# yhhshb/biolib

Measured on AMD Instinct MI355X. Metric: Gbp/s minimizer-scanned (k=31,w=11), higher is better.
Workload: dtype u64

## Files before the change

### biolib_amd/csrc/bl_capi.hip

```cpp
#include <hip/hip_runtime.h>
#include <algorithm>
#include <cstdio>
#include <cstdlib>
#include <cstring>
#include <deque>
#include <new>
#include <string>
#include <utility>
#include <vector>

#include "../../include/biolib_amd.h"
#include "bl_launch.hpp"
#include "bl_lookup_launch.hpp"
#include "bl_read_counts_launch.hpp"
#include "bl_scan128_launch.hpp"

namespace {

thread_local std::string g_err;

int fail(int code, const std::string& msg)
{
    g_err = msg;
    return code;
}

}

int bl_set_error(int code, const char* msg) { return fail(code, msg ? msg : ""); }
struct bl_ctx;
hipStream_t bl_ctx_stream(bl_ctx* ctx);
int bl_ctx_device(bl_ctx* ctx);

namespace {

#define BL_HIP(call)                                                                                       \
    do {                                                                                                   \
        hipError_t e_ = (call);                                                                            \
        if (e_ != hipSuccess)                                                                              \
            return fail(e_ == hipErrorOutOfMemory ? BL_ERR_OOM : BL_ERR_HIP,                               \
                        std::string(#call) + ": " + hipGetErrorString(e_));                                \
    } while (0)

constexpr int RESULT_WORDS = 16;
constexpr int RING = 256;
constexpr size_t HDR_BYTES = 256;
constexpr size_t SHARD_BYTES = (size_t)bl::NSHARD * 8 * sizeof(unsigned long long);

struct Pending {
    bl_result* user;
    int slot;
    uint64_t capacity;
    bool has_capacity;
};

}

struct Lane {
    hipStream_t own = nullptr;
    unsigned char* ws = nullptr;
    size_t ws_bytes = 0;
    unsigned char* tile_buf = nullptr;
    size_t tile_buf_bytes = 0;
    uint16_t* slot_buf = nullptr;
    size_t slot_buf_bytes = 0;
    hipEvent_t ev_start = nullptr, ev_stop = nullptr;
    hipEvent_t ev_count_done = nullptr;
    bool count_recorded = false;
    bool scan_recorded = false;

    unsigned long long* shards() const { return reinterpret_cast<unsigned long long*>(ws + HDR_BYTES); }
    unsigned long long* result() const { return reinterpret_cast<unsigned long long*>(ws + HDR_BYTES + SHARD_BYTES); }
};

struct bl_ctx {
    int device = 0;
    Lane lanes[2];
    Lane* cur = nullptr;
    int next_lane = 0;
    int n_lanes = 1;
    uint32_t emit_lds_per_wg = 0;
    hipStream_t user_stream = nullptr;
    bool borrowed = false;
    hipStream_t stream = nullptr;
    unsigned long long* pinned = nullptr;
    hipEvent_t slot_ev[RING] = {};
    int next_slot = 0;
    std::deque<Pending> pending;
    bool timed = false;
    bool exact_windows = false;
    bool position_tiled = false;
    int jaccard128_path = 0;
    bool count128_tables = true;
    int table_prefix_bits = -1;
    bool ktiming = false;
    bl::LaunchLog last_kernels{};
    std::vector<hipEvent_t> ev_pool;
    std::vector<std::pair<hipEvent_t, hipEvent_t>> ev_open;
    double kernel_ms = 0.0;
    uint64_t kernel_launches = 0;
    std::vector<std::pair<hipEvent_t, hipEvent_t>> marks;
    std::vector<bl_batch*> batches;
    void* scratch[8] = {};
    size_t scratch_bytes[8] = {};
    std::vector<std::pair<void*, size_t>> pool_idle;
    std::vector<std::pair<void*, size_t>> pool_live;

    unsigned long long* shards() const { return cur->shards(); }
    unsigned long long* result() const { return cur->result(); }
    static size_t fixed_bytes() { return HDR_BYTES + SHARD_BYTES + RESULT_WORDS * sizeof(unsigned long long); }
};

struct bl_batch {
    bl_ctx* ctx = nullptr;
    uint8_t* bases = nullptr;
    bool owns_bases = false;
    uint32_t* start_bits = nullptr;
    uint64_t n_bases = 0;
    uint64_t n_seqs = 0;
    uint64_t read_len = 0;
    uint64_t origin = 0;
};

namespace {

int grow(bl_ctx* c, void** buf, size_t* have, size_t need)
{
    if (need <= *have) return BL_OK;
    BL_HIP(hipStreamSynchronize(c->stream));
    if (*buf) BL_HIP(hipFree(*buf));
    *buf = nullptr;
    *have = 0;
    const size_t bytes = need + need / 8;
    hipError_t e = hipMalloc(buf, bytes);
    if (e != hipSuccess) return fail(BL_ERR_OOM, std::string("hipMalloc(scan scratch): ") + hipGetErrorString(e));
    *have = bytes;
    return BL_OK;
}

int ensure_workspace(bl_ctx* c)
{
    return grow(c, reinterpret_cast<void**>(&c->cur->ws), &c->cur->ws_bytes, bl_ctx::fixed_bytes());
}

void select_lane(bl_ctx* c)
{
    if (c->borrowed) {
        c->cur = &c->lanes[0];
        c->stream = c->user_stream;
    } else {
        c->cur = &c->lanes[c->next_lane];
        if (c->n_lanes == 2) c->next_lane ^= 1;
        c->stream = c->cur->own;
    }
}

void deliver(bl_ctx* c, const Pending& p)
{
    const unsigned long long* r = c->pinned + (size_t)p.slot * RESULT_WORDS;
    bl_result out;
    std::memset(&out, 0, sizeof(out));
    out.count = r[0];
    out.xor_value = r[1];
    out.xor_hash = r[2];
    out.xor_pos = r[3];
    out.aux = r[4];
    out.redone = (int32_t)(r[5] > 0x7fffffffull ? 0x7fffffffull : r[5]);
    out.status = BL_OK;
    if (p.has_capacity && r[0] > p.capacity) out.status = BL_ERR_CAPACITY;
    if (p.user) *p.user = out;
}

int flush_pending(bl_ctx* c)
{
    for (const Pending& p : c->pending) deliver(c, p);
    c->pending.clear();
    return BL_OK;
}

int flush_kernel_events(bl_ctx* c)
{
    for (auto& pr : c->ev_open) {
        float ms = 0.f;
        BL_HIP(hipEventElapsedTime(&ms, pr.first, pr.second));
        c->kernel_ms += ms;
        c->kernel_launches += 1;
        c->ev_pool.push_back(pr.first);
        c->ev_pool.push_back(pr.second);
    }
    c->ev_open.clear();
    return BL_OK;
}

int sync_ctx(bl_ctx* c)
{
    for (Lane& l : c->lanes) BL_HIP(hipStreamSynchronize(l.own));
    if (c->borrowed) BL_HIP(hipStreamSynchronize(c->user_stream));
    int rc = flush_kernel_events(c);
    if (rc != BL_OK) return rc;
    return flush_pending(c);
}

int kernel_event(bl_ctx* c, bool start)
{
    if (!c->ktiming) return BL_OK;
    if (start) {
        hipEvent_t ev[2];
        for (int i = 0; i < 2; ++i) {
            if (!c->ev_pool.empty()) { ev[i] = c->ev_pool.back(); c->ev_pool.pop_back(); }
            else BL_HIP(hipEventCreate(&ev[i]));
        }
        c->ev_open.emplace_back(ev[0], ev[1]);
        BL_HIP(hipEventRecord(ev[0], c->stream));
    } else {
        BL_HIP(hipEventRecord(c->ev_open.back().second, c->stream));
    }
    return BL_OK;
}

int begin_scan(bl_ctx* c)
{
    BL_HIP(hipSetDevice(c->device));
    select_lane(c);
    int rc = ensure_workspace(c);
    if (rc != BL_OK) return rc;
    BL_HIP(hipEventRecord(c->cur->ev_start, c->stream));
    BL_HIP(hipMemsetAsync(c->cur->ws, 0, bl_ctx::fixed_bytes(), c->stream));
    return BL_OK;
}

int end_scan(bl_ctx* c, uint32_t add_mask, bl_result* user, bool has_capacity, uint64_t capacity, uint32_t flags,
             bool already_folded = false)
{
    if (!already_folded) {
        hipError_t e = bl::launch_reduce_shards(c->shards(), c->result(), add_mask, reinterpret_cast<unsigned long long*>(c->cur->ws) + 1, c->stream);
        if (e != hipSuccess) return fail(BL_ERR_HIP, std::string("reduce_shards: ") + hipGetErrorString(e));
    }
    if ((int)c->pending.size() >= RING) {
        const Pending old = c->pending.front();
        BL_HIP(hipEventSynchronize(c->slot_ev[old.slot]));
        deliver(c, old);
        c->pending.pop_front();
    }
    const int slot = c->next_slot;
    c->next_slot = (c->next_slot + 1) % RING;
    BL_HIP(hipMemcpyAsync(c->pinned + (size_t)slot * RESULT_WORDS, c->result(), RESULT_WORDS * sizeof(unsigned long long),
                          hipMemcpyDeviceToHost, c->stream));
    BL_HIP(hipEventRecord(c->slot_ev[slot], c->stream));
    BL_HIP(hipEventRecord(c->cur->ev_stop, c->stream));
    c->cur->scan_recorded = true;
    c->timed = true;
    c->pending.push_back(Pending{user, slot, capacity, has_capacity});
    if (flags & BL_FLAG_SYNC) {
        int rc = sync_ctx(c);
        if (rc != BL_OK) return rc;
        if (user && user->status != BL_OK)
            return fail(user->status, "output capacity too small for the records found");
    }
    return BL_OK;
}

int zero_result(bl_ctx* c, bl_result* user, uint32_t flags)
{
    if (user) std::memset(user, 0, sizeof(*user));
    (void)c;
    (void)flags;
    return BL_OK;
}

int check_range(const bl_batch* b, uint64_t first, uint64_t n, uint64_t& end)
{
    if (first > b->n_bases) return fail(BL_ERR_INVALID, "range starts beyond the batch");
    end = (n == 0 || n > b->n_bases - first) ? b->n_bases : first + n;
    if (end - first > (1ull << 31)) return fail(BL_ERR_INVALID, "a scan range may hold at most 2^31 positions; split it");
    return BL_OK;
}

int make_start_bits(bl_ctx* c, bl_batch* b, const uint64_t* offsets, uint64_t n_seqs, uint64_t read_len)
{
    const uint64_t n_words = (b->n_bases + 31) / 32 + 4;
    if (!offsets && (read_len == 0 || read_len >= b->n_bases)) {
        b->start_bits = nullptr;
        b->n_seqs = b->n_bases ? 1 : 0;
        return BL_OK;
    }
    BL_HIP(hipMalloc(&b->start_bits, n_words * sizeof(uint32_t)));
    BL_HIP(hipMemsetAsync(b->start_bits, 0, n_words * sizeof(uint32_t), c->stream));
    if (offsets) {
        for (uint64_t q = 0; q < n_seqs; ++q)
            if (offsets[q] > offsets[q + 1]) return fail(BL_ERR_INVALID, "offsets must be non-decreasing");
        if (offsets[0] != 0 || offsets[n_seqs] != b->n_bases) return fail(BL_ERR_INVALID, "offsets must span [0, n_bases]");
        uint64_t* d_off = nullptr;
        BL_HIP(hipMalloc(&d_off, (n_seqs + 1) * sizeof(uint64_t)));
        hipError_t e = hipMemcpyAsync(d_off, offsets, (n_seqs + 1) * sizeof(uint64_t), hipMemcpyHostToDevice, c->stream);
        if (e == hipSuccess) e = bl::launch_start_bits_offsets(b->start_bits, d_off, n_seqs, b->n_bases, c->stream);
        if (e == hipSuccess) e = hipStreamSynchronize(c->stream);
        (void)hipFree(d_off);
        if (e != hipSuccess) return fail(BL_ERR_HIP, std::string("start_bits_offsets: ") + hipGetErrorString(e));
        b->n_seqs = n_seqs;
    } else {
        hipError_t e = bl::launch_start_bits_fixed(b->start_bits, n_words, b->n_bases, read_len, c->stream);
        if (e != hipSuccess) return fail(BL_ERR_HIP, std::string("start_bits_fixed: ") + hipGetErrorString(e));
        b->n_seqs = (b->n_bases + read_len - 1) / read_len;
        BL_HIP(hipStreamSynchronize(c->stream));
    }
    return BL_OK;
}

int ensure_start_bits(bl_ctx* c, const bl_batch* cb)
{
    bl_batch* b = const_cast<bl_batch*>(cb);
    if (b->start_bits || b->read_len == 0 || b->read_len >= b->n_bases) return BL_OK;
    int rc = sync_ctx(c);
    if (rc != BL_OK) return rc;
    return make_start_bits(c, b, nullptr, 0, b->read_len);
}

}

hipStream_t bl_ctx_stream(bl_ctx* c)
{
    if (c->borrowed) return c->user_stream;
    if (c->n_lanes == 2 && c->lanes[1].scan_recorded) (void)hipStreamWaitEvent(c->lanes[0].own, c->lanes[1].ev_stop, 0);
    return c->lanes[0].own;
}
int bl_batch_adopt_device(bl_ctx* ctx, void* d_bases, uint64_t n_bases, uint64_t* d_offsets, uint64_t n_seqs, uint64_t fixed_len, bl_batch** out);
int bl_ctx_device(bl_ctx* c) { return c->device; }
int bl_ctx_count128_tables(bl_ctx* c) { return c->count128_tables ? 1 : 0; }
int bl_ctx_jaccard128_path(bl_ctx* c) { return c->jaccard128_path; }
int bl_ctx_table_prefix_bits(bl_ctx* c) { return c->table_prefix_bits; }
int bl_batch_describe(const bl_batch* b, bl_ctx** ctx, uint64_t* n_bases, uint64_t* n_seqs, uint64_t* read_len)
{
    *ctx = b->ctx;
    *n_bases = b->n_bases;
    *n_seqs = b->n_seqs;
    *read_len = b->read_len;
    return BL_OK;
}

int bl_batch_scan_view(bl_ctx* c, const bl_batch* b, int ensure, const uint32_t** start_bits)
{
    if (ensure) {
        int rc = ensure_start_bits(c, b);
        if (rc != BL_OK) return rc;
    }
    *start_bits = b->start_bits;
    return BL_OK;
}

void* bl_ctx_scratch(bl_ctx* c, int slot, size_t bytes)
{
    if (!c || slot < 0 || slot >= 8) return nullptr;
    if (bytes <= c->scratch_bytes[slot]) return c->scratch[slot];
    (void)hipSetDevice(c->device);
    if (c->scratch[slot]) {
        (void)hipDeviceSynchronize();
        (void)hipFree(c->scratch[slot]);
        c->scratch[slot] = nullptr;
        c->scratch_bytes[slot] = 0;
    }
    const size_t want = bytes + bytes / 8;
    if (hipMalloc(&c->scratch[slot], want) != hipSuccess) {
        c->scratch[slot] = nullptr;
        return nullptr;
    }
    c->scratch_bytes[slot] = want;
    return c->scratch[slot];
}

void* bl_ctx_pool_alloc(bl_ctx* c, size_t bytes)
{
    if (!c) return nullptr;
    if (bytes < 256) bytes = 256;
    size_t best = c->pool_idle.size();
    for (size_t i = 0; i < c->pool_idle.size(); ++i) {
        const size_t have = c->pool_idle[i].second;
        if (have >= bytes && have <= 2 * bytes + 65536 && (best == c->pool_idle.size() || have < c->pool_idle[best].second)) best = i;
    }
    if (best < c->pool_idle.size()) {
        const auto entry = c->pool_idle[best];
        c->pool_idle[best] = c->pool_idle.back();
        c->pool_idle.pop_back();
        c->pool_live.push_back(entry);
        return entry.first;
    }
    void* p = nullptr;
    const size_t want = bytes + bytes / 8;
    if (hipMalloc(&p, want) != hipSuccess) return nullptr;
    c->pool_live.emplace_back(p, want);
    return p;
}

void bl_ctx_pool_free(bl_ctx* c, void* p)
{
    if (!p) return;
    if (c)
        for (size_t i = 0; i < c->pool_live.size(); ++i)
            if (c->pool_live[i].first == p) {
                const auto entry = c->pool_live[i];
                c->pool_live[i] = c->pool_live.back();
                c->pool_live.pop_back();
                size_t total = 0;
                for (const auto& e : c->pool_idle) total += e.second;
                if (c->pool_idle.size() < 16 && entry.second <= ((size_t)1 << 30) && total + entry.second <= ((size_t)4 << 30)) c->pool_idle.push_back(entry);
                else (void)hipFree(p);
                return;
            }
    (void)hipFree(p);
}

extern "C" {

const char* bl_last_error(void) { return g_err.c_str(); }
int bl_version(void) { return BL_VERSION; }

int bl_device_count(int* n)
{
    if (!n) return fail(BL_ERR_INVALID, "n is NULL");
    int c = 0;
    hipError_t e = hipGetDeviceCount(&c);
    if (e != hipSuccess) { *n = 0; return fail(BL_ERR_NO_DEVICE, std::string("hipGetDeviceCount: ") + hipGetErrorString(e)); }
    *n = c;
    return BL_OK;
}

int bl_ctx_create(int device, bl_ctx** out)
{
    if (!out) return fail(BL_ERR_INVALID, "out is NULL");
    *out = nullptr;
    int n = 0;
    if (hipGetDeviceCount(&n) != hipSuccess || n == 0) return fail(BL_ERR_NO_DEVICE, "no HIP device visible: this library has no CPU fallback");
    if (device < 0 || device >= n) return fail(BL_ERR_INVALID, "device index out of range");
    hipDeviceProp_t prop;
    BL_HIP(hipGetDeviceProperties(&prop, device));
    if (std::strncmp(prop.gcnArchName, "gfx950", 6) != 0)
        return fail(BL_ERR_NO_DEVICE, std::string("device is ") + prop.gcnArchName + ", kernels are built for gfx950 (MI355X) only");
    BL_HIP(hipSetDevice(device));
    bl_ctx* c = new (std::nothrow) bl_ctx();
    if (!c) return fail(BL_ERR_OOM, "host allocation failed");
    c->device = device;
    hipError_t e = hipSuccess;
    for (Lane& l : c->lanes) {
        if (e == hipSuccess) e = hipStreamCreateWithFlags(&l.own, hipStreamNonBlocking);
        if (e == hipSuccess) e = hipEventCreate(&l.ev_start);
        if (e == hipSuccess) e = hipEventCreateWithFlags(&l.ev_count_done, hipEventDisableTiming);
        if (e == hipSuccess) e = hipEventCreate(&l.ev_stop);
    }
    if (e == hipSuccess) e = hipHostMalloc(reinterpret_cast<void**>(&c->pinned), (size_t)RING * RESULT_WORDS * sizeof(unsigned long long), hipHostMallocDefault);
    for (int i = 0; i < RING && e == hipSuccess; ++i) e = hipEventCreateWithFlags(&c->slot_ev[i], hipEventDisableTiming);
    if (e != hipSuccess) {
        bl_ctx_destroy(c);
        return fail(BL_ERR_HIP, std::string("context setup: ") + hipGetErrorString(e));
    }
    for (int i = 0; i < 2; ++i) {
        c->cur = &c->lanes[i];
        c->stream = c->cur->own;
        int rc = ensure_workspace(c);
        if (rc != BL_OK) { bl_ctx_destroy(c); return rc; }
    }
    c->cur = &c->lanes[0];
    c->stream = c->lanes[0].own;
    *out = c;
    return BL_OK;
}

int bl_ctx_set_lanes(bl_ctx* c, int n)
{
    if (!c || (n != 1 && n != 2)) return fail(BL_ERR_INVALID, "bl_ctx_set_lanes: need a context and n = 1 or 2");
    int rc = sync_ctx(c);
    if (rc != BL_OK) return rc;
    c->n_lanes = n;
    c->next_lane = 0;
    c->lanes[0].count_recorded = c->lanes[1].count_recorded = false;
    return BL_OK;
}

int bl_ctx_destroy(bl_ctx* c)
{
    if (!c) return BL_OK;
    (void)hipSetDevice(c->device);
    for (Lane& l : c->lanes)
        if (l.own) (void)hipStreamSynchronize(l.own);
    if (c->borrowed) (void)hipStreamSynchronize(c->user_stream);
    while (!c->batches.empty()) bl_batch_destroy(c->batches.back());
    for (Lane& l : c->lanes) {
        if (l.ws) (void)hipFree(l.ws);
        if (l.tile_buf) (void)hipFree(l.tile_buf);
        if (l.slot_buf) (void)hipFree(l.slot_buf);
        if (l.ev_start) (void)hipEventDestroy(l.ev_start);
        if (l.ev_count_done) (void)hipEventDestroy(l.ev_count_done);
        if (l.ev_stop) (void)hipEventDestroy(l.ev_stop);
        if (l.own) (void)hipStreamDestroy(l.own);
    }
    for (void* p : c->scratch)
        if (p) (void)hipFree(p);
    for (const auto& e : c->pool_idle) (void)hipFree(e.first);
    for (const auto& e : c->pool_live) (void)hipFree(e.first);
    if (c->pinned) (void)hipHostFree(c->pinned);
    for (hipEvent_t ev : c->slot_ev)
        if (ev) (void)hipEventDestroy(ev);
    for (auto& pr : c->ev_open) { (void)hipEventDestroy(pr.first); (void)hipEventDestroy(pr.second); }
    for (hipEvent_t ev : c->ev_pool) (void)hipEventDestroy(ev);
    for (auto& pr : c->marks) { (void)hipEventDestroy(pr.first); if (pr.second) (void)hipEventDestroy(pr.second); }
    delete c;
    return BL_OK;
}

int bl_ctx_set_stream(bl_ctx* c, void* hip_stream)
{
    if (!c) return fail(BL_ERR_INVALID, "ctx is NULL");
    int rc = sync_ctx(c);
    if (rc != BL_OK) return rc;
    c->borrowed = true;
    c->user_stream = static_cast<hipStream_t>(hip_stream);
    c->cur = &c->lanes[0];
    c->stream = c->user_stream;
    return BL_OK;
}

int bl_ctx_use_own_streams(bl_ctx* c)
{
    if (!c) return fail(BL_ERR_INVALID, "ctx is NULL");
    int rc = sync_ctx(c);
    if (rc != BL_OK) return rc;
    c->borrowed = false;
    c->user_stream = nullptr;
    c->cur = &c->lanes[0];
    c->stream = c->lanes[0].own;
    return BL_OK;
}

int bl_ctx_sync(bl_ctx* c)
{
    if (!c) return fail(BL_ERR_INVALID, "ctx is NULL");
    return sync_ctx(c);
}

int bl_ctx_last_scan_ms(bl_ctx* c, float* ms)
{
    if (!c || !ms) return fail(BL_ERR_INVALID, "NULL argument");
    if (!c->timed) return fail(BL_ERR_INVALID, "no scan has been issued on this context");
    BL_HIP(hipEventSynchronize(c->cur->ev_stop));
    BL_HIP(hipEventElapsedTime(ms, c->cur->ev_start, c->cur->ev_stop));
    return BL_OK;
}

int bl_ctx_set_exact_windows(bl_ctx* c, int on)
{
    if (!c) return fail(BL_ERR_INVALID, "ctx is NULL");
    c->exact_windows = on != 0;
    return BL_OK;
}

int bl_ctx_set_option(bl_ctx* c, const char* name, int64_t value)
{
    if (!c || !name) return fail(BL_ERR_INVALID, "bl_ctx_set_option: NULL argument");
    const std::string n(name);
    if (n == "exact_windows" && (value == 0 || value == 1)) return bl_ctx_set_exact_windows(c, (int)value);
    if (n == "lanes") return bl_ctx_set_lanes(c, (int)value);
    if (n == "position_tiled" && (value == 0 || value == 1)) {
        c->position_tiled = value != 0;
        return BL_OK;
    }
    if (n == "count128_tables" && (value == 0 || value == 1)) {
        c->count128_tables = value != 0;
        return BL_OK;
    }
    if (n == "jaccard128_path" && value >= 0 && value <= 2) {
        c->jaccard128_path = (int)value;
        return BL_OK;
    }
    if (n == "table_prefix_bits" && value >= -1 && value <= bllk::MAX_PREFIX_BITS) {
        c->table_prefix_bits = (int)value;
        return BL_OK;
    }
    if (n == "emit_lds_bytes" && value >= 0 && value <= 160 * 1024) {
        c->emit_lds_per_wg = (uint32_t)value;
        return BL_OK;
    }
    return fail(BL_ERR_INVALID, "bl_ctx_set_option: unknown name or value out of range: " + n);
}

int bl_ctx_kernel_timing(bl_ctx* c, int enable)
{
    if (!c) return fail(BL_ERR_INVALID, "ctx is NULL");
    int rc = sync_ctx(c);
    if (rc != BL_OK) return rc;
    c->ktiming = enable != 0;
    c->kernel_ms = 0.0;
    c->kernel_launches = 0;
    return BL_OK;
}

int bl_ctx_kernel_time(bl_ctx* c, double* total_ms, uint64_t* launches)
{
    if (!c || !total_ms || !launches) return fail(BL_ERR_INVALID, "NULL argument");
    int rc = sync_ctx(c);
    if (rc != BL_OK) return rc;
    *total_ms = c->kernel_ms;
    *launches = c->kernel_launches;
    return BL_OK;
}

static constexpr size_t MAX_MARKS = 4096;

int bl_ctx_mark(bl_ctx* c)
{
    if (!c) return fail(BL_ERR_INVALID, "ctx is NULL");
    if (c->marks.size() >= MAX_MARKS) return fail(BL_ERR_CAPACITY, "bl_ctx_mark: 4096 markers outstanding: collect them with bl_ctx_mark_times");
    BL_HIP(hipSetDevice(c->device));
    std::pair<hipEvent_t, hipEvent_t> m{nullptr, nullptr};
    const bool two = !c->borrowed && c->n_lanes == 2 && c->lanes[1].own;
    hipError_t e = hipEventCreate(&m.first);
    if (e == hipSuccess && two) e = hipEventCreate(&m.second);
    if (e == hipSuccess) e = hipEventRecord(m.first, c->borrowed ? c->user_stream : c->lanes[0].own);
    if (e == hipSuccess && two) e = hipEventRecord(m.second, c->lanes[1].own);
    if (e != hipSuccess) {
        if (m.first) (void)hipEventDestroy(m.first);
        if (m.second) (void)hipEventDestroy(m.second);
        return fail(BL_ERR_HIP, std::string("bl_ctx_mark: ") + hipGetErrorString(e));
    }
    c->marks.push_back(m);
    return BL_OK;
}

int bl_ctx_mark_times(bl_ctx* c, double* ms, uint32_t capacity, uint32_t* n)
{
    if (!c || !n || (!ms && capacity)) return fail(BL_ERR_INVALID, "NULL argument");
    int rc = sync_ctx(c);
    if (rc != BL_OK) return rc;
    *n = (uint32_t)c->marks.size();
    if (capacity < c->marks.size()) {
        if (capacity == 0) return BL_OK;
        return fail(BL_ERR_CAPACITY, "bl_ctx_mark_times: more markers than the buffer holds (*n says how many)");
    }
    hipError_t e = hipSuccess;
    for (size_t i = 0; i < c->marks.size(); ++i) {
        float a = 0.f, b = 0.f;
        if (e == hipSuccess) e = hipEventSynchronize(c->marks[i].first);
        if (e == hipSuccess) e = hipEventElapsedTime(&a, c->marks[0].first, c->marks[i].first);
        if (e == hipSuccess && c->marks[i].second) {
            e = hipEventSynchronize(c->marks[i].second);
            if (e == hipSuccess) e = hipEventElapsedTime(&b, c->marks[0].first, c->marks[i].second);
        }
        if (i < capacity) ms[i] = a > b ? a : b;
    }
    for (auto& pr : c->marks) { (void)hipEventDestroy(pr.first); if (pr.second) (void)hipEventDestroy(pr.second); }
    c->marks.clear();
    if (e != hipSuccess) return fail(BL_ERR_HIP, std::string("bl_ctx_mark_times: ") + hipGetErrorString(e));
    return BL_OK;
}


static int new_batch(bl_ctx* c, uint64_t n_bases, bl_batch** out, bl_batch*& b)
{
    if (!c || !out) return fail(BL_ERR_INVALID, "NULL argument");
    *out = nullptr;
    BL_HIP(hipSetDevice(c->device));
    b = new (std::nothrow) bl_batch();
    if (!b) return fail(BL_ERR_OOM, "host allocation failed");
    b->ctx = c;
    b->n_bases = n_bases;
    c->batches.push_back(b);
    return BL_OK;
}

static int upload_batch(bl_ctx* c, const char* bases, uint64_t n_bases, const uint64_t* offsets, uint64_t n_seqs, uint64_t read_len, bl_batch** out)
{
    bl_batch* b = nullptr;
    int rc = new_batch(c, n_bases, out, b);
    if (rc != BL_OK) return rc;
    if (n_bases && !bases) { bl_batch_destroy(b); return fail(BL_ERR_INVALID, "bases is NULL"); }
    b->bases = static_cast<uint8_t*>(bl_ctx_pool_alloc(c, n_bases + 64));
    if (!b->bases) { bl_batch_destroy(b); return fail(BL_ERR_OOM, "device allocation of the batch's bases failed"); }
    b->owns_bases = true;
    hipError_t e = hipMemsetAsync(b->bases + (n_bases & ~15ull), 0, 64 + (n_bases & 15ull), c->stream);
    if (e == hipSuccess && n_bases) e = hipMemcpyAsync(b->bases, bases, n_bases, hipMemcpyHostToDevice, c->stream);
    if (e != hipSuccess) { bl_batch_destroy(b); return fail(BL_ERR_HIP, std::string("upload: ") + hipGetErrorString(e)); }
    uint64_t fixed = 0;
    if (read_len) {
        if (read_len < n_bases) {
            fixed = read_len;
            n_seqs = (n_bases + read_len - 1) / read_len;
        } else {
            offsets = nullptr;
            n_seqs = 0;
        }
    } else if (offsets && n_seqs > 1 && offsets[0] == 0 && offsets[n_seqs] == n_bases && offsets[1] > 0 && offsets[1] < n_bases) {
        fixed = offsets[1];
        for (uint64_t q = 1; q < n_seqs && fixed; ++q)
            if (offsets[q] != q * fixed) fixed = 0;
        if (fixed && (n_bases - offsets[n_seqs - 1] > fixed || n_bases == offsets[n_seqs - 1])) fixed = 0;
    }
    if (fixed) {
        b->read_len = fixed;
        b->n_seqs = n_seqs;
    } else {
        rc = make_start_bits(c, b, offsets, n_seqs, 0);
    }
    if (rc == BL_OK) {
        e = hipStreamSynchronize(c->stream);
        if (e != hipSuccess) rc = fail(BL_ERR_HIP, std::string("upload sync: ") + hipGetErrorString(e));
    }
    if (rc != BL_OK) { bl_batch_destroy(b); return rc; }
    *out = b;
    return BL_OK;
}

int bl_batch_upload(bl_ctx* c, const char* bases, uint64_t n_bases, const uint64_t* offsets, uint64_t n_seqs, bl_batch** out)
{
    return upload_batch(c, bases, n_bases, offsets, n_seqs, 0, out);
}

int bl_batch_upload_reads(bl_ctx* c, const char* bases, uint64_t n_bases, uint64_t read_len, bl_batch** out)
{
    if (read_len == 0) return fail(BL_ERR_INVALID, "read_len must not be 0");
    return upload_batch(c, bases, n_bases, nullptr, 0, read_len, out);
}

int bl_batch_from_device(bl_ctx* c, const void* d_bases, uint64_t n_bases, const uint64_t* offsets, uint64_t n_seqs, uint64_t read_len,
                         bl_batch** out)
{
    bl_batch* b = nullptr;
    int rc = new_batch(c, n_bases, out, b);
    if (rc != BL_OK) return rc;
    if ((n_bases && !d_bases) || (reinterpret_cast<uintptr_t>(d_bases) & 15)) {
        bl_batch_destroy(b);
        return fail(BL_ERR_INVALID, "d_bases must be a non-NULL, 16-byte aligned device pointer");
    }
    b->bases = const_cast<uint8_t*>(static_cast<const uint8_t*>(d_bases));
    b->owns_bases = false;
    if (!offsets && read_len > 0 && read_len < n_bases) {
        b->read_len = read_len;
        b->n_seqs = (n_bases + read_len - 1) / read_len;
    } else {
        rc = make_start_bits(c, b, offsets, n_seqs, read_len);
        if (rc != BL_OK) { bl_batch_destroy(b); return rc; }
    }
    *out = b;
    return BL_OK;
}

int bl_batch_set_origin(bl_batch* b, uint64_t origin)
{
    if (!b) return fail(BL_ERR_INVALID, "batch is NULL");
    b->origin = origin;
    return BL_OK;
}

uint64_t bl_batch_origin(const bl_batch* b) { return b ? b->origin : 0; }

int bl_batch_synth(bl_ctx* c, uint64_t seed, uint64_t n_bases, uint64_t read_len, bl_batch** out)
{
    bl_batch* b = nullptr;
    int rc = new_batch(c, n_bases, out, b);
    if (rc != BL_OK) return rc;
    hipError_t e = hipMalloc(&b->bases, n_bases + 64);
    if (e != hipSuccess) { bl_batch_destroy(b); return fail(BL_ERR_OOM, std::string("hipMalloc(bases): ") + hipGetErrorString(e)); }
    b->owns_bases = true;
    e = hipMemsetAsync(b->bases + (n_bases & ~15ull), 0, 64 + (n_bases & 15ull), c->stream);
    if (e == hipSuccess) e = bl::launch_synth(b->bases, 0, n_bases, seed, c->stream);
    if (e != hipSuccess) { bl_batch_destroy(b); return fail(BL_ERR_HIP, std::string("synth: ") + hipGetErrorString(e)); }
    if (read_len > 0 && read_len < n_bases) {
        b->read_len = read_len;
        b->n_seqs = (n_bases + read_len - 1) / read_len;
    } else {
        rc = make_start_bits(c, b, nullptr, 0, read_len);
    }
    if (rc == BL_OK && hipStreamSynchronize(c->stream) != hipSuccess) rc = fail(BL_ERR_HIP, "synth sync failed");
    if (rc != BL_OK) { bl_batch_destroy(b); return rc; }
    *out = b;
    return BL_OK;
}

}

int bl_batch_adopt_device(bl_ctx* c, void* d_bases, uint64_t n_bases, uint64_t* d_offsets, uint64_t n_seqs, uint64_t fixed_len, bl_batch** out)
{
    bl_batch* b = nullptr;
    int rc = new_batch(c, n_bases, out, b);
    if (rc != BL_OK) { bl_ctx_pool_free(c, d_bases); bl_ctx_pool_free(c, d_offsets); return rc; }
    b->bases = static_cast<uint8_t*>(d_bases);
    b->owns_bases = true;
    b->n_seqs = n_seqs;
    if (fixed_len && n_seqs > 1 && fixed_len < n_bases) {
        b->read_len = fixed_len;
        bl_ctx_pool_free(c, d_offsets);
        *out = b;
        return BL_OK;
    }
    hipStream_t s = bl_ctx_stream(c);
    const uint64_t n_words = (n_bases + 31) / 32 + 4;
    b->start_bits = static_cast<uint32_t*>(bl_ctx_pool_alloc(c, n_words * sizeof(uint32_t)));
    hipError_t e = b->start_bits ? hipSuccess : hipErrorOutOfMemory;
    if (e == hipSuccess) e = hipMemsetAsync(b->start_bits, 0, n_words * sizeof(uint32_t), s);
    if (e == hipSuccess) e = bl::launch_start_bits_offsets(b->start_bits, d_offsets, n_seqs, n_bases, s);
    if (e == hipSuccess) e = hipStreamSynchronize(s);
    bl_ctx_pool_free(c, d_offsets);
    if (e != hipSuccess) { bl_batch_destroy(b); return fail(BL_ERR_HIP, std::string("adopt: ") + hipGetErrorString(e)); }
    *out = b;
    return BL_OK;
}

int bl_batch_adopt_like(bl_ctx* c, const bl_batch* like, void* d_bases, uint32_t* d_start_bits, bl_batch** out)
{
    bl_batch* b = nullptr;
    int rc = new_batch(c, like->n_bases, out, b);
    if (rc != BL_OK) { bl_ctx_pool_free(c, d_bases); bl_ctx_pool_free(c, d_start_bits); return rc; }
    b->bases = static_cast<uint8_t*>(d_bases);
    b->owns_bases = true;
    b->start_bits = d_start_bits;
    b->n_seqs = like->n_seqs;
    b->read_len = like->read_len;
    b->origin = like->origin;
    *out = b;
    return BL_OK;
}

extern "C" {

int bl_batch_destroy(bl_batch* b)
{
    if (!b) return BL_OK;
    if (b->ctx) {
        (void)hipSetDevice(b->ctx->device);
        for (Lane& l : b->ctx->lanes)
            if (l.own) (void)hipStreamSynchronize(l.own);
        if (b->ctx->borrowed) (void)hipStreamSynchronize(b->ctx->user_stream);
        auto& v = b->ctx->batches;
        for (size_t i = 0; i < v.size(); ++i)
            if (v[i] == b) { v[i] = v.back(); v.pop_back(); break; }
    }
    if (b->owns_bases && b->bases) bl_ctx_pool_free(b->ctx, b->bases);
    if (b->start_bits) bl_ctx_pool_free(b->ctx, b->start_bits);
    delete b;
    return BL_OK;
}

uint64_t bl_batch_n_bases(const bl_batch* b) { return b ? b->n_bases : 0; }
uint64_t bl_batch_n_seqs(const bl_batch* b) { return b ? b->n_seqs : 0; }
const void* bl_batch_device_bases(const bl_batch* b) { return b ? b->bases : nullptr; }

int bl_batch_download(bl_batch* b, uint64_t first, uint64_t n, char* out)
{
    if (!b || (!out && n)) return fail(BL_ERR_INVALID, "NULL argument");
    if (first > b->n_bases || n > b->n_bases - first) return fail(BL_ERR_INVALID, "range beyond the batch");
    BL_HIP(hipSetDevice(b->ctx->device));
    int rc = sync_ctx(b->ctx);
    if (rc != BL_OK) return rc;
    if (n) BL_HIP(hipMemcpy(out, b->bases + first, n, hipMemcpyDeviceToHost));
    return BL_OK;
}


int bl_scan_kmers(bl_ctx* c, const bl_batch* b, uint64_t first, uint64_t n, uint32_t k, uint64_t seed, uint32_t flags,
                  uint64_t* d_values, uint64_t* d_hashes, uint8_t* d_valid, bl_result* result)
{
    if (!c || !b || b->ctx != c) return fail(BL_ERR_INVALID, "ctx/batch is NULL or the batch belongs to another context");
    if (k < 1 || k > bl::MAX_UNIT) return fail(BL_ERR_INVALID, "k must be in [1, 32] (KmerType = uint64_t)");
    uint64_t end;
    int rc = check_range(b, first, n, end);
    if (rc != BL_OK) return rc;
    if (end <= first) return zero_result(c, result, flags);
    rc = ensure_start_bits(c, b);
    if (rc != BL_OK) return rc;
    bl::KmerParams p{};
    p.bases = b->bases;
    p.n_bases = (int64_t)b->n_bases;
    p.start_bits = b->start_bits;
    p.first = (int64_t)first;
    p.end = (int64_t)end;
    p.origin = bl::align_down16((int64_t)first);
    p.n_tiles = (int32_t)(((int64_t)end - 1 - p.origin) / bl::H + 1);
    p.unit = (int32_t)k;
    p.seed = (uint32_t)seed;
    p.canonical = (flags & BL_FLAG_CANONICAL) ? 1 : 0;
    p.drop_last = (flags & BL_FLAG_DROP_LAST) ? 1 : 0;
    p.out_value = d_values;
    p.out_hash = d_hashes;
    p.out_valid = d_valid;
    rc = begin_scan(c);
    if (rc != BL_OK) return rc;
    p.shards = c->shards();
    const int n_blocks = p.n_tiles < 256 * 8 ? p.n_tiles : 256 * 8;
    rc = kernel_event(c, true);
    if (rc != BL_OK) return rc;
    hipError_t e = bl::launch_kmers(p, n_blocks, c->stream);
    if (e != hipSuccess) return fail(BL_ERR_HIP, std::string("kmer_kernel: ") + hipGetErrorString(e));
    rc = kernel_event(c, false);
    if (rc != BL_OK) return rc;
    return end_scan(c,  (1u << 0) | (1u << 3), result, false, 0, flags);
}


static int prepare_kmers128(bl_ctx* c, const bl_batch* b, uint64_t first, uint64_t n, uint32_t k, uint64_t seed, uint32_t flags, const uint64_t* d_values,
                            bl::Kmer128Params& p, bl_result* result, bool& empty)
{
    empty = false;
    if (!c || !b || b->ctx != c) return fail(BL_ERR_INVALID, "ctx/batch is NULL or the batch belongs to another context");
    if (k < 1 || k > bl::MAX_UNIT128) return fail(BL_ERR_INVALID, "k must be in [1, 64] (KmerType = __uint128_t)");
    if (reinterpret_cast<uintptr_t>(d_values) % 16 != 0) return fail(BL_ERR_INVALID, "d_values must be 16-byte aligned (one __uint128_t per record)");
    uint64_t end;
    int rc = check_range(b, first, n, end);
    if (rc != BL_OK) return rc;
    if (end <= first) {
        empty = true;
        return zero_result(c, result, flags);
    }
    rc = ensure_start_bits(c, b);
    if (rc != BL_OK) return rc;
    p.bases = b->bases;
    p.n_bases = (int64_t)b->n_bases;
    p.start_bits = b->start_bits;
    p.pos_base = (int64_t)b->origin;
    bl::plan_kmers128((int64_t)first, (int64_t)end, p);
    p.unit = (int32_t)k;
    p.seed = (uint32_t)seed;
    p.canonical = (flags & BL_FLAG_CANONICAL) ? 1 : 0;
    p.drop_last = (flags & BL_FLAG_DROP_LAST) ? 1 : 0;
    return BL_OK;
}

extern "C++" {
template <typename P>
static int scan_two_pass128(bl_ctx* c, P& p, bl::Kmer128Params& km, size_t lane_bytes, uint32_t** lane_rest, bool wants, uint64_t capacity, uint32_t flags,
                            bl_result* result, hipError_t (*count)(const P&, hipStream_t), hipError_t (*emit)(const P&, hipStream_t), const char* family)
{
    km.capacity = wants ? capacity : 0;
    int rc = begin_scan(c);
    if (rc != BL_OK) return rc;
    const size_t nt = (size_t)km.n_tiles, nb = (nt + bl::SCAN_BLK - 1) / bl::SCAN_BLK;
    rc = grow(c, reinterpret_cast<void**>(&c->cur->tile_buf), &c->cur->tile_buf_bytes, (2 * nt + 2 * nb + 8) * sizeof(unsigned long long));
    if (rc != BL_OK) return rc;
    unsigned long long* tb = reinterpret_cast<unsigned long long*>(c->cur->tile_buf);
    km.tile_counts = tb;
    km.tile_base = tb + nt;
    unsigned long long* block_tot = tb + 2 * nt;
    km.block_base = block_tot + nb;
    if (lane_bytes) {
        rc = grow(c, reinterpret_cast<void**>(&c->cur->slot_buf), &c->cur->slot_buf_bytes, nt * bl::TPB * lane_bytes);
        if (rc != BL_OK) return rc;
        km.lane_masks = c->cur->slot_buf;
        if (lane_rest) *lane_rest = reinterpret_cast<uint32_t*>(c->cur->slot_buf + nt * bl::TPB);
    }
    km.shards = c->shards();
    rc = kernel_event(c, true);
    if (rc != BL_OK) return rc;
    hipError_t e = count(p, c->stream);
    if (e != hipSuccess) return fail(BL_ERR_HIP, std::string(family) + "_count_kernel: " + hipGetErrorString(e));
    rc = kernel_event(c, false);
    if (rc != BL_OK) return rc;
    bl::ScanParams sp{};
    sp.tile_counts = km.tile_counts;
    sp.tile_base = km.tile_base;
    sp.block_base = km.block_base;
    sp.shards = km.shards;
    unsigned long long* carry = reinterpret_cast<unsigned long long*>(c->cur->ws);
    e = bl::launch_tile_scan(sp, bl::GroupRange{0, (uint32_t)km.n_tiles}, block_tot, carry, c->stream);
    if (e != hipSuccess) return fail(BL_ERR_HIP, std::string("tile_scan: ") + hipGetErrorString(e));
    if (wants) {
        e = emit(p, c->stream);
        if (e != hipSuccess) return fail(BL_ERR_HIP, std::string(family) + "_emit_kernel: " + hipGetErrorString(e));
    }
    return end_scan(c, 1u << 0, result, wants, capacity, flags);
}
}

int bl_scan_kmers128(bl_ctx* c, const bl_batch* b, uint64_t first, uint64_t n, uint32_t k, uint64_t seed, uint32_t flags,
                     uint64_t* d_values, uint64_t* d_hashes, uint8_t* d_valid, bl_result* result)
{
    bl::Kmer128Params p{};
    bool empty;
    int rc = prepare_kmers128(c, b, first, n, k, seed, flags, d_values, p, result, empty);
    if (rc != BL_OK || empty) return rc;
    p.out_value = d_values;
    p.out_hash = d_hashes;
    p.out_valid = d_valid;
    rc = begin_scan(c);
    if (rc != BL_OK) return rc;
    p.shards = c->shards();
    rc = kernel_event(c, true);
    if (rc != BL_OK) return rc;
    hipError_t e = bl::launch_kmers128(p, c->stream);
    if (e != hipSuccess) return fail(BL_ERR_HIP, std::string("kmer128_kernel: ") + hipGetErrorString(e));
    rc = kernel_event(c, false);
    if (rc != BL_OK) return rc;
    return end_scan(c,  (1u << 0) | (1u << 3), result, false, 0, flags);
}

int bl_scan_kmer_counts(bl_ctx* c, const bl_batch* b, uint64_t first, uint64_t n, uint32_t k, uint32_t flags, const bl_table* table, uint32_t* d_counts,
                        uint8_t* d_valid, bl_result* result)
{
    if (!table) return fail(BL_ERR_INVALID, "table is NULL");
    if (c && table->ctx != c) return fail(BL_ERR_INVALID, "the table belongs to another context");
    if (table->view.key_words == 1 && k > 32) return fail(BL_ERR_INVALID, "a table of one-word keys takes k <= 32");
    if (k >= 1 && 2 * k > table->view.key_bits)
        return fail(BL_ERR_INVALID, "2k = " + std::to_string(2 * k) + " exceeds the table's key_bits = " + std::to_string(table->view.key_bits));
    bllk::ScanCountParams p{};
    bool empty;
    int rc = prepare_kmers128(c, b, first, n, k, 0, flags, nullptr, p.km, result, empty);
    if (rc != BL_OK || empty) return rc;
    p.table = table->view;
    p.out_counts = d_counts;
    p.out_valid = d_valid;
    rc = begin_scan(c);
    if (rc != BL_OK) return rc;
    p.km.shards = c->shards();
    rc = kernel_event(c, true);
    if (rc != BL_OK) return rc;
    hipError_t e = bllk::launch_scan_counts(p, c->stream);
    if (e != hipSuccess) return fail(BL_ERR_HIP, std::string("scan_counts_kernel: ") + hipGetErrorString(e));
    rc = kernel_event(c, false);
    if (rc != BL_OK) return rc;
    return end_scan(c,  (1u << 0) | (1u << 2) | (1u << 3), result, false, 0, flags);
}

int bl_scan_read_counts(bl_ctx* c, const bl_batch* b, uint64_t first, uint64_t n, uint32_t k, uint32_t flags, const bl_table* table, uint32_t min_count,
                        const uint64_t* d_offsets, uint32_t mode, bl_read_counts* d_records, bl_result* result)
{
    static_assert(sizeof(bl_read_counts) == sizeof(blrc::Record) && alignof(blrc::Record) == 16, "the kernel's record is the header's");
    if (!table) return fail(BL_ERR_INVALID, "table is NULL");
    if (c && table->ctx != c) return fail(BL_ERR_INVALID, "the table belongs to another context");
    if (table->view.key_words == 1 && k > 32) return fail(BL_ERR_INVALID, "a table of one-word keys takes k <= 32");
    if (k >= 1 && 2 * k > table->view.key_bits)
        return fail(BL_ERR_INVALID, "2k = " + std::to_string(2 * k) + " exceeds the table's key_bits = " + std::to_string(table->view.key_bits));
    if (min_count == 0) return fail(BL_ERR_INVALID, "min_count must be at least 1");
    if (mode != BL_READ_COUNTS_INIT && mode != BL_READ_COUNTS_ACCUMULATE) return fail(BL_ERR_INVALID, "mode is BL_READ_COUNTS_INIT or BL_READ_COUNTS_ACCUMULATE");
    if (!d_records) return fail(BL_ERR_INVALID, "d_records is NULL");
    if (reinterpret_cast<uintptr_t>(d_records) % 16 != 0) return fail(BL_ERR_INVALID, "d_records must be 16-byte aligned");
    if (b && !d_offsets && b->n_seqs > 1 && b->read_len == 0)
        return fail(BL_ERR_INVALID, "d_offsets is NULL: only a single-sequence or a fixed-read-length batch finds its sequences without the offsets");
    blrc::ReadCountParams p{};
    bool empty;
    int rc = prepare_kmers128(c, b, first, n, k, 0, flags, nullptr, p.km, result, empty);
    if (rc != BL_OK || empty) return rc;
    p.table = table->view;
    p.min_count = min_count;
    p.offsets = d_offsets;
    p.n_seqs = b->n_seqs;
    p.read_len = d_offsets ? 0 : b->read_len;
    p.records = reinterpret_cast<blrc::Record*>(d_records);
    rc = begin_scan(c);
    if (rc != BL_OK) return rc;
    p.km.shards = c->shards();
    rc = kernel_event(c, true);
    if (rc != BL_OK) return rc;
    hipError_t e = mode == BL_READ_COUNTS_INIT ? blrc::launch_read_counts_init(p, c->stream) : hipSuccess;
    if (e != hipSuccess) return fail(BL_ERR_HIP, std::string("read_counts_init_kernel: ") + hipGetErrorString(e));
    e = blrc::launch_read_counts(p, c->stream);
    if (e != hipSuccess) return fail(BL_ERR_HIP, std::string("read_counts_kernel: ") + hipGetErrorString(e));
    rc = kernel_event(c, false);
    if (rc != BL_OK) return rc;
    return end_scan(c,  (1u << 0) | (1u << 2) | (1u << 3), result, false, 0, flags);
}

int bl_scan_hash_sample128(bl_ctx* c, const bl_batch* b, uint64_t first, uint64_t n, uint32_t k, uint64_t seed, uint64_t threshold, uint32_t flags,
                           uint64_t* d_values, uint64_t* d_positions, uint64_t* d_hashes, uint64_t capacity, bl_result* result)
{
    bl::Kmer128Params p{};
    bool empty;
    int rc = prepare_kmers128(c, b, first, n, k, seed, flags, d_values, p, result, empty);
    if (rc != BL_OK || empty) return rc;
    p.hash_below = threshold;
    p.rec_value = d_values;
    p.rec_pos = d_positions;
    p.rec_hash = d_hashes;
    return scan_two_pass128(c, p, p, sizeof(uint16_t), nullptr, d_values || d_positions || d_hashes, capacity, flags, result, bl::launch_kmers128_count,
                            bl::launch_kmers128_emit, "kmer128");
}


int bl_scan_syncmers128(bl_ctx* c, const bl_batch* b, uint64_t first, uint64_t n, uint32_t k, uint32_t s, uint32_t start_offset,
                        uint32_t end_offset, uint64_t seed, uint32_t flags, uint64_t* d_positions, uint64_t capacity, bl_result* result)
{
    if (!c || !b || b->ctx != c) return fail(BL_ERR_INVALID, "ctx/batch is NULL or the batch belongs to another context");
    if (s < 1 || s > bl::MAX_SMER128 || k < s || k > bl::MAX_UNIT128)
        return fail(BL_ERR_INVALID, "need 1 <= s <= 32 and s <= k <= 64 (KmerType = __uint128_t, 16-byte s-mer keys)");
    bl::Sync128Params p{};
    bool empty;
    int rc = prepare_kmers128(c, b, first, n, k, seed, flags, nullptr, p.km, result, empty);
    if (rc != BL_OK || empty) return rc;
    bl::plan_syncmers128((int)k, (int)s, start_offset, end_offset, p);
    p.km.rec_pos = d_positions;
    return scan_two_pass128(c, p, p.km, sizeof(uint16_t), nullptr, d_positions != nullptr, capacity, flags, result, bl::launch_syncmers128_count,
                            bl::launch_syncmers128_emit, "sync128");
}


int bl_scan_minimizers128(bl_ctx* c, const bl_batch* b, uint64_t first, uint64_t n, uint32_t unit, uint32_t w, uint64_t seed, uint32_t flags,
                          uint64_t* d_values, uint64_t* d_positions, uint64_t* d_hashes, uint64_t capacity, bl_result* result)
{
    if (!c || !b || b->ctx != c) return fail(BL_ERR_INVALID, "ctx/batch is NULL or the batch belongs to another context");
    if (unit < 1 || unit > bl::MAX_UNIT128 || w < 1 || w > bl::MAX_W)
        return fail(BL_ERR_INVALID, "need 1 <= unit <= 64 and 1 <= w <= 64 (KmerType = __uint128_t, 16-byte unit keys)");
    bl::Min128Params p{};
    bool empty;
    int rc = prepare_kmers128(c, b, first, n, unit, seed, flags, d_values, p.km, result, empty);
    if (rc != BL_OK || empty) return rc;
    const bool wants = d_values || d_positions || d_hashes;
    p.w = (int32_t)w;
    p.km.rec_value = d_values;
    p.km.rec_pos = d_positions;
    p.km.rec_hash = d_hashes;
    return scan_two_pass128(c, p, p.km, wants ? sizeof(uint16_t) + 3 * sizeof(uint32_t) : 0, &p.lane_offs, wants, capacity, flags, result,
                            bl::launch_minimizers128_count, bl::launch_minimizers128_emit, "min128");
}

uint64_t bl_hash64_u128(uint64_t lo, uint64_t hi, uint64_t seed) { return bl::murmur64_u128(lo, hi, (uint32_t)seed); }

static int scan_windows(int mode, bl_ctx* c, const bl_batch* b, uint64_t first, uint64_t n, uint32_t unit, uint32_t w, uint64_t seed,
                        uint32_t flags, bl::ScanParams& p, uint64_t capacity, bl_result* result)
{
    if (!c || !b || b->ctx != c) return fail(BL_ERR_INVALID, "ctx/batch is NULL or the batch belongs to another context");
    c->last_kernels.n = 0;
    if (unit < 1 || unit > bl::MAX_UNIT) return fail(BL_ERR_INVALID, "hashed unit length must be in [1, 32]");
    if (w < 1 || w > bl::MAX_W) return fail(BL_ERR_INVALID, "window must be in [1, 64]");
    uint64_t end;
    int rc = check_range(b, first, n, end);
    if (rc != BL_OK) return rc;
    if (end <= first) return zero_result(c, result, flags);
    p.bases = b->bases;
    p.n_bases = (int64_t)b->n_bases;
    p.pos_base = (int64_t)b->origin;
    p.exact_windows = c->exact_windows ? 1 : 0;
    bl::plan_scan(mode, (int64_t)first, (int64_t)end, (int)w, p);
    if (b->read_len && !c->position_tiled && !p.use_threshold && bl::frl_width_built(mode, (int)w)) {
        bl::plan_scan_frl_for(mode, (int64_t)first, (int64_t)end, (int64_t)b->n_bases, (int64_t)b->read_len, (int)unit, (int)w, (flags & BL_FLAG_CANONICAL) != 0, p);
    }
    if (!p.frl) {
        rc = ensure_start_bits(c, b);
        if (rc != BL_OK) return rc;
    }
    p.start_bits = b->start_bits;
    p.unit = (int32_t)unit;
    p.w = (int32_t)w;
    p.seed = (uint32_t)seed;
    p.canonical = (flags & BL_FLAG_CANONICAL) ? 1 : 0;
    p.drop_last = (flags & BL_FLAG_DROP_LAST) ? 1 : 0;
    p.capacity = capacity;
    rc = begin_scan(c);
    if (rc != BL_OK) return rc;
    const size_t nt = (size_t)p.n_tiles, nb = (nt + bl::SCAN_BLK - 1) / bl::SCAN_BLK;
    rc = grow(c, reinterpret_cast<void**>(&c->cur->tile_buf), &c->cur->tile_buf_bytes, (2 * nt + 2 * nb + 8) * sizeof(unsigned long long) + nt * sizeof(uint32_t));
    if (rc != BL_OK) return rc;
    const size_t n_lists = mode == bl::MODE_SUPERKMER ? 3 : 1;
    const size_t slot_entries = nt * (size_t)p.stride;
    const size_t list_bytes = n_lists * slot_entries * sizeof(uint16_t);
    rc = grow(c, reinterpret_cast<void**>(&c->cur->slot_buf), &c->cur->slot_buf_bytes, list_bytes + nt * (size_t)p.slot_chunks * sizeof(uint32_t));
    if (rc != BL_OK) return rc;
    unsigned long long* tb = reinterpret_cast<unsigned long long*>(c->cur->tile_buf);
    p.tile_counts = tb;
    p.tile_base = tb + nt;
    unsigned long long* block_tot = tb + 2 * nt;
    p.block_base = block_tot + nb;
    p.redo_list = reinterpret_cast<uint32_t*>(tb + 2 * nt + 2 * nb + 8);
    p.redo_count = reinterpret_cast<unsigned long long*>(c->cur->ws) + 1;
    p.slots_a = c->cur->slot_buf;
    p.slots_j = mode == bl::MODE_SUPERKMER ? c->cur->slot_buf + slot_entries : nullptr;
    p.slots_e = mode == bl::MODE_SUPERKMER ? c->cur->slot_buf + 2 * slot_entries : nullptr;
    p.slots_c = reinterpret_cast<uint32_t*>(reinterpret_cast<unsigned char*>(c->cur->slot_buf) + list_bytes);
    p.shards = c->shards();
    const bl::GroupRange all{0, (uint32_t)p.n_tiles};
    unsigned long long* carry = reinterpret_cast<unsigned long long*>(c->cur->ws);
    const bool staggered = c->n_lanes == 2 && !c->borrowed;
    if (staggered) {
        Lane* other = c->cur == &c->lanes[0] ? &c->lanes[1] : &c->lanes[0];
        if (other->count_recorded) BL_HIP(hipStreamWaitEvent(c->stream, other->ev_count_done, 0));
    }
    rc = kernel_event(c, true);
    if (rc != BL_OK) return rc;
    hipError_t e = bl::launch_scan_count(mode, p, all, c->stream, &c->last_kernels);
    if (e != hipSuccess) return fail(BL_ERR_HIP, std::string("scan_count_kernel: ") + hipGetErrorString(e));
    if (staggered) {
        BL_HIP(hipEventRecord(c->cur->ev_count_done, c->stream));
        c->cur->count_recorded = true;
    }
    rc = kernel_event(c, false);
    if (rc != BL_OK) return rc;
    e = bl::launch_tile_scan(p, all, block_tot, carry, c->stream);
    if (e != hipSuccess) return fail(BL_ERR_HIP, std::string("tile_scan: ") + hipGetErrorString(e));
    const uint32_t emit_lds_default = mode == bl::MODE_SUPERKMER ? 8192u : 28672u;
    e = bl::launch_scan_emit(mode, p, all, c->stream, staggered ? (c->emit_lds_per_wg ? c->emit_lds_per_wg : emit_lds_default) : 0, &c->last_kernels);
    if (e != hipSuccess) return fail(BL_ERR_HIP, std::string("scan_emit_kernel: ") + hipGetErrorString(e));
    return BL_OK;
}

int bl_scan_minimizers(bl_ctx* c, const bl_batch* b, uint64_t first, uint64_t n, uint32_t unit, uint32_t w, uint64_t seed, uint32_t flags,
                       uint64_t* d_values, uint64_t* d_positions, uint64_t* d_hashes, uint64_t capacity, bl_result* result)
{
    bl::ScanParams p{};
    p.out_value = d_values;
    p.out_pos = d_positions;
    p.out_hash = d_hashes;
    const bool wants = d_values || d_positions || d_hashes;
    int rc = scan_windows(bl::MODE_MINIMIZER, c, b, first, n, unit, w, seed, flags, p, wants ? capacity : 0, result);
    if (rc != BL_OK || p.n_tiles == 0) return rc;
    return end_scan(c, 1u << 0, result, wants, capacity, flags);
}

int bl_scan_hash_sample(bl_ctx* c, const bl_batch* b, uint64_t first, uint64_t n, uint32_t k, uint64_t seed, uint64_t threshold, uint32_t flags,
                        uint64_t* d_values, uint64_t* d_positions, uint64_t* d_hashes, uint64_t capacity, bl_result* result)
{
    bl::ScanParams p{};
    p.out_value = d_values;
    p.out_pos = d_positions;
    p.out_hash = d_hashes;
    p.use_threshold = 1;
    p.hash_below = threshold;
    const bool wants = d_values || d_positions || d_hashes;
    int rc = scan_windows(bl::MODE_MINIMIZER, c, b, first, n, k, 1, seed, flags, p, wants ? capacity : 0, result);
    if (rc != BL_OK || p.n_tiles == 0) return rc;
    return end_scan(c, 1u << 0, result, wants, capacity, flags);
}

int bl_scan_super_kmers(bl_ctx* c, const bl_batch* b, uint64_t first, uint64_t n, uint32_t k, uint32_t m, uint64_t seed, uint32_t flags,
                        uint64_t* d_minimizers, uint64_t* d_first_pos, uint8_t* d_mm_pos, uint8_t* d_sizes, uint64_t* d_hashes,
                        uint64_t capacity, bl_result* result)
{
    if (m < 1 || k < m) return fail(BL_ERR_INVALID, "need 1 <= m <= k");
    if (!c) return fail(BL_ERR_INVALID, "ctx is NULL");
    bl::ScanParams p{};
    p.out_value = d_minimizers;
    p.out_first = d_first_pos;
    p.out_mmpos = d_mm_pos;
    p.out_hash = d_hashes;
    const bool wants = d_minimizers || d_first_pos || d_mm_pos || d_sizes || d_hashes;
    p.out_size = d_sizes;
    int rc = scan_windows(bl::MODE_SUPERKMER, c, b, first, n, m, k - m + 1, seed, flags, p, wants ? capacity : 0, result);
    if (rc != BL_OK || p.n_tiles == 0) return rc;
    return end_scan(c, (1u << 0) | (1u << 4), result, wants, capacity, flags);
}

int bl_scan_super_kmer_records(bl_ctx* c, const bl_batch* b, uint64_t first, uint64_t n, uint32_t k, uint32_t m, uint64_t seed, uint32_t flags,
                               uint64_t* d_records, uint64_t* d_hashes, uint64_t capacity, bl_result* result)
{
    if (m < 1 || k < m || k > 32 || 2 * k - m > 59) return fail(BL_ERR_INVALID, "need 1 <= m <= k <= 32 and 2k - m <= 59 (bases per packed record)");
    if (!c) return fail(BL_ERR_INVALID, "ctx is NULL");
    bl::ScanParams p{};
    p.out_records = d_records;
    p.out_hash = d_hashes;
    const bool wants = d_records || d_hashes;
    int rc = scan_windows(bl::MODE_SUPERKMER, c, b, first, n, m, k - m + 1, seed, flags, p, wants ? capacity : 0, result);
    if (rc != BL_OK || p.n_tiles == 0) return rc;
    return end_scan(c, (1u << 0) | (1u << 4), result, wants, capacity, flags);
}

int bl_scan_super_kmer_records128(bl_ctx* c, const bl_batch* b, uint64_t first, uint64_t n, uint32_t k, uint32_t m, uint64_t seed, uint32_t flags,
                                  uint64_t* d_records, uint64_t* d_hashes, uint64_t capacity, bl_result* result)
{
    if (m < 1 || m > 32 || k < m || k > 64 || k - m + 1 > 64 || 2 * k - m > 122)
        return fail(BL_ERR_INVALID, "need 1 <= m <= 32, m <= k <= 64, k - m + 1 <= 64 and 2k - m <= 122 (bases per 32-byte record)");
    if ((uintptr_t)d_records & 31u) return fail(BL_ERR_INVALID, "d_records must be 32-byte aligned");
    if (!c) return fail(BL_ERR_INVALID, "ctx is NULL");
    bl::ScanParams p{};
    p.out_records = d_records;
    p.out_hash = d_hashes;
    p.records128 = 1;
    const bool wants = d_records || d_hashes;
    int rc = scan_windows(bl::MODE_SUPERKMER, c, b, first, n, m, k - m + 1, seed, flags, p, wants ? capacity : 0, result);
    if (rc != BL_OK || p.n_tiles == 0) return rc;
    return end_scan(c, (1u << 0) | (1u << 4), result, wants, capacity, flags);
}

int bl_scan_syncmers(bl_ctx* c, const bl_batch* b, uint64_t first, uint64_t n, uint32_t k, uint32_t s, uint32_t start_offset,
                     uint32_t end_offset, uint64_t seed, uint32_t flags, uint64_t* d_positions, uint64_t capacity, bl_result* result)
{
    if (s < 1 || k < s || k > bl::MAX_UNIT) return fail(BL_ERR_INVALID, "need 1 <= s <= k <= 32");
    bl::ScanParams p{};
    p.out_pos = d_positions;
    p.soff = (int32_t)start_offset;
    p.eoff = (int32_t)end_offset;
    int rc = scan_windows(bl::MODE_SYNCMER, c, b, first, n, s, k - s + 1, seed, flags, p, d_positions ? capacity : 0, result);
    if (rc != BL_OK || p.n_tiles == 0) return rc;
    return end_scan(c, 1u << 0, result, d_positions != nullptr, capacity, flags);
}

static int copy_names(const char* const* names, int n, char* buf, uint64_t capacity, uint64_t* needed)
{
    uint64_t bytes = 1;
    for (int i = 0; i < n; ++i) bytes += std::strlen(names[i]) + 1;
    if (needed) *needed = bytes;
    if (!buf || capacity < bytes) return fail(BL_ERR_CAPACITY, "the buffer is too small for the kernel names");
    char* o = buf;
    for (int i = 0; i < n; ++i) {
        const size_t len = std::strlen(names[i]);
        std::memcpy(o, names[i], len);
        o[len] = '\n';
        o += len + 1;
    }
    *o = 0;
    return BL_OK;
}

int bl_ctx_last_scan_kernels(bl_ctx* c, char* buf, uint64_t capacity, uint64_t* needed)
{
    if (!c) return fail(BL_ERR_INVALID, "ctx is NULL");
    return copy_names(c->last_kernels.names, c->last_kernels.n, buf, capacity, needed);
}

int bl_scan_kernel_names(char* buf, uint64_t capacity, uint64_t* needed)
{
    int n = 0;
    const char* const* names = bl::scan_kernel_names(&n);
    return copy_names(names, n, buf, capacity, needed);
}


int bl_device_alloc(bl_ctx* c, uint64_t bytes, void** d_ptr)
{
    if (!c || !d_ptr) return fail(BL_ERR_INVALID, "NULL argument");
    BL_HIP(hipSetDevice(c->device));
    *d_ptr = nullptr;
    hipError_t e = hipMalloc(d_ptr, bytes ? bytes : 16);
    if (e != hipSuccess) return fail(BL_ERR_OOM, std::string("hipMalloc: ") + hipGetErrorString(e));
    return BL_OK;
}

int bl_device_free(bl_ctx* c, void* d_ptr)
{
    if (!c) return fail(BL_ERR_INVALID, "ctx is NULL");
    BL_HIP(hipSetDevice(c->device));
    int rc = sync_ctx(c);
    if (rc != BL_OK) return rc;
    if (d_ptr) BL_HIP(hipFree(d_ptr));
    return BL_OK;
}

int bl_host_alloc(bl_ctx* c, uint64_t bytes, void** ptr)
{
    if (!c || !ptr) return fail(BL_ERR_INVALID, "NULL argument");
    BL_HIP(hipSetDevice(c->device));
    *ptr = nullptr;
    hipError_t e = hipHostMalloc(ptr, bytes ? bytes : 16, hipHostMallocPortable);
    if (e != hipSuccess) return fail(BL_ERR_OOM, std::string("hipHostMalloc: ") + hipGetErrorString(e));
    return BL_OK;
}

int bl_host_free(bl_ctx* c, void* ptr)
{
    if (!c) return fail(BL_ERR_INVALID, "ctx is NULL");
    BL_HIP(hipSetDevice(c->device));
    int rc = sync_ctx(c);
    if (rc != BL_OK) return rc;
    if (ptr) BL_HIP(hipHostFree(ptr));
    return BL_OK;
}

int bl_copy_to_host(bl_ctx* c, void* dst, const void* d_src, uint64_t bytes)
{
    if (!c || (bytes && (!dst || !d_src))) return fail(BL_ERR_INVALID, "NULL argument");
    BL_HIP(hipSetDevice(c->device));
    int rc = sync_ctx(c);
    if (rc != BL_OK) return rc;
    if (bytes) BL_HIP(hipMemcpy(dst, d_src, bytes, hipMemcpyDeviceToHost));
    return BL_OK;
}

int bl_copy_to_device(bl_ctx* c, void* d_dst, const void* src, uint64_t bytes)
{
    if (!c || (bytes && (!d_dst || !src))) return fail(BL_ERR_INVALID, "NULL argument");
    BL_HIP(hipSetDevice(c->device));
    int rc = sync_ctx(c);
    if (rc != BL_OK) return rc;
    if (bytes) BL_HIP(hipMemcpy(d_dst, src, bytes, hipMemcpyHostToDevice));
    return BL_OK;
}

uint64_t bl_hash64_u64(uint64_t value, uint64_t seed) { return bl::murmur64(value, (uint32_t)seed); }

}
```

### biolib_amd/csrc/bl_kernels.hip

```cpp
#include <hip/hip_runtime.h>
#include <cstdlib>
#include "bl_scan_frl.hpp"
#include "bl_launch.hpp"

#ifndef BL_SY0_WAVES
#define BL_SY0_WAVES 2
#endif
#ifndef BL_SY2_WAVES
#define BL_SY2_WAVES 3
#endif
#ifndef BL_CS_WAVES
#define BL_CS_WAVES 3
#endif
#ifndef BL_POSAX_WAVES
#define BL_POSAX_WAVES 4
#endif
#ifndef BL_SKAX_WAVES
#define BL_SKAX_WAVES 4
#endif
#ifndef BL_C4_WAVES
#define BL_C4_WAVES 5
#endif
#ifndef BL_CSRT_WAVES
#define BL_CSRT_WAVES 3
#endif

namespace bl {


__device__ __forceinline__ uint32_t wave_incl_scan_u32(uint32_t v, int lane)
{
    (void)lane;
#ifndef BL_SCAN_BUILTIN_DPP
    asm("s_nop 1\n\t"
        "v_add_u32_dpp %0, %0, %0 row_shr:1 row_mask:0xf bank_mask:0xf bound_ctrl:0\n\t"
        "s_nop 1\n\t"
        "v_add_u32_dpp %0, %0, %0 row_shr:2 row_mask:0xf bank_mask:0xf bound_ctrl:0\n\t"
        "s_nop 1\n\t"
        "v_add_u32_dpp %0, %0, %0 row_shr:4 row_mask:0xf bank_mask:0xf bound_ctrl:0\n\t"
        "s_nop 1\n\t"
        "v_add_u32_dpp %0, %0, %0 row_shr:8 row_mask:0xf bank_mask:0xf bound_ctrl:0\n\t"
        "s_nop 1\n\t"
        "v_add_u32_dpp %0, %0, %0 row_bcast:15 row_mask:0xa bank_mask:0xf\n\t"
        "s_nop 1\n\t"
        "v_add_u32_dpp %0, %0, %0 row_bcast:31 row_mask:0xc bank_mask:0xf"
        : "+v"(v));
    return v;
#else
    v += (uint32_t)__builtin_amdgcn_update_dpp(0, (int)v, 0x111, 0xf, 0xf, false);
    v += (uint32_t)__builtin_amdgcn_update_dpp(0, (int)v, 0x112, 0xf, 0xf, false);
    v += (uint32_t)__builtin_amdgcn_update_dpp(0, (int)v, 0x114, 0xf, 0xf, false);
    v += (uint32_t)__builtin_amdgcn_update_dpp(0, (int)v, 0x118, 0xf, 0xf, false);
    v += (uint32_t)__builtin_amdgcn_update_dpp(0, (int)v, 0x142, 0xa, 0xf, false);
    v += (uint32_t)__builtin_amdgcn_update_dpp(0, (int)v, 0x143, 0xc, 0xf, false);
    return v;
#endif
}

__device__ __forceinline__ uint32_t wave_xor_to_last_u32(uint32_t v)
{
    v ^= (uint32_t)__builtin_amdgcn_update_dpp(0, (int)v, 0x111, 0xf, 0xf, false);
    v ^= (uint32_t)__builtin_amdgcn_update_dpp(0, (int)v, 0x112, 0xf, 0xf, false);
    v ^= (uint32_t)__builtin_amdgcn_update_dpp(0, (int)v, 0x114, 0xf, 0xf, false);
    v ^= (uint32_t)__builtin_amdgcn_update_dpp(0, (int)v, 0x118, 0xf, 0xf, false);
    v ^= (uint32_t)__builtin_amdgcn_update_dpp(0, (int)v, 0x142, 0xa, 0xf, false);
    v ^= (uint32_t)__builtin_amdgcn_update_dpp(0, (int)v, 0x143, 0xc, 0xf, false);
    return v;
}

__device__ __forceinline__ unsigned long long wave_xor_to_last_u64(unsigned long long v)
{
    return ((unsigned long long)wave_xor_to_last_u32((uint32_t)(v >> 32)) << 32) | wave_xor_to_last_u32((uint32_t)v);
}

__device__ __forceinline__ unsigned long long wave_xor_u64(unsigned long long v)
{
#pragma unroll
    for (int d = 32; d >= 1; d >>= 1) v ^= __shfl_xor(v, d, 64);
    return v;
}

__device__ __forceinline__ unsigned long long wave_sum_u64(unsigned long long v)
{
#pragma unroll
    for (int d = 32; d >= 1; d >>= 1) v += __shfl_xor(v, d, 64);
    return v;
}

__device__ __forceinline__ unsigned long long uniform64(unsigned long long v)
{
    const uint32_t lo = __builtin_amdgcn_readfirstlane((uint32_t)v), hi = __builtin_amdgcn_readfirstlane((uint32_t)(v >> 32));
    return ((unsigned long long)hi << 32) | lo;
}

__device__ __forceinline__ uint32_t block_excl_scan(uint32_t v, uint32_t* wave_tot, int tid, uint32_t& total)
{
    const int lane = tid & 63, wv = wave_index(tid);
    const uint32_t incl = wave_incl_scan_u32(v, lane);
    if (lane == 63) wave_tot[wv] = incl;
    __syncthreads();
    uint32_t before = 0, all = 0;
#pragma unroll
    for (int i = 0; i < TPB / 64; ++i) {
        const uint32_t t = wave_tot[i];
        if (i < wv) before += t;
        all += t;
    }
    total = all;
    return before + incl - v;
}

__device__ __forceinline__ void spill_list(uint16_t* dst, const uint16_t* src, uint32_t n, int tid)
{
    uint32_t* d32 = reinterpret_cast<uint32_t*>(dst);
    const uint32_t* s32 = reinterpret_cast<const uint32_t*>(src);
    const uint32_t nd = (n + 1) / 2;
    if ((uint32_t)tid < nd) d32[tid] = s32[tid];
#pragma unroll 1
    for (uint32_t i = TPB + tid; i < nd; i += TPB) d32[i] = s32[i];
}

__device__ __forceinline__ void fill_list(uint16_t* dst, const uint16_t* src, uint32_t n, int tid)
{
    uint32_t* d32 = reinterpret_cast<uint32_t*>(dst);
    const uint32_t* s32 = reinterpret_cast<const uint32_t*>(src);
#pragma unroll 1
    for (uint32_t i = tid; i < (n + 1) / 2; i += TPB) d32[i] = s32[i];
}

template <int MODE, int W, int SY = 0, int U = 0>
__device__ __forceinline__ void count_tile(const ScanParams& p, TileShared<MODE, W>& sh, uint32_t tile, int tid)
{
    const int64_t q0 = p.origin + (int64_t)tile * p.stride;
    phase_load<MODE, W>(p, sh, tid, q0);
    constexpr bool CS = SY == 1;
    if (SY != 0 && tid == 0) sh.redo = 0;
    if (MODE != MODE_SYNCMER) {
        const int needed = staged_chunks(p);
        uint32_t* sc = p.slots_c + (size_t)tile * p.slot_chunks;
        if (tid < needed) sc[tid] = sh.codes[tid];
        if (TPB + tid < needed) sc[TPB + tid] = sh.codes[TPB + tid];
    }
    __syncthreads();

    ThreadState st;
    constexpr bool DIRECT = MODE == MODE_SYNCMER && SY != 0 && U >= 1 && U <= 16 && U + W - 1 >= 16 && U + W - 1 <= 32;
    bool tie = false;
#ifdef BL_CLOSED_ON_HASHES
    constexpr bool AP = false;
#else
    constexpr bool AP = DIRECT && CS;
#endif
    constexpr bool MAX = MODE != MODE_SYNCMER && SY == 2;
    if (DIRECT) phase_hash_closed<MODE, W, (DIRECT ? U : 1), SY == 2, AP>(p, sh, tid, st, &tie);
    else phase_hash<MODE, W, (MODE != MODE_SYNCMER && U >= 1 && U <= 16 ? U : 0), U == 0, MAX>(p, sh, tid, st);

    uint32_t packed;
    if constexpr (MODE == MODE_SYNCMER && CS && W < 0) {
        packed = phase_sync_closed_rt<MODE, (W == -16 ? -16 : -8)>(p, reinterpret_cast<TileShared<MODE, (W == -16 ? -16 : -8)>&>(sh), tid, q0, st, nullptr);
    } else if (MODE == MODE_SYNCMER && CS) {
        bool undecided;
        packed = phase_sync_closed<MODE, (W > 1 ? W : 2), (DIRECT ? U : 0), AP>(p, reinterpret_cast<TileShared<MODE, (W > 1 ? W : 2)>&>(sh), tid, q0, st, nullptr, undecided);
        if (BL_COLD(wave_any(undecided)) && (tid & 63) == 0) sh.redo = 1;
    } else if (MODE == MODE_SYNCMER && SY == 2 && W > 1) {
        uint32_t af[S + 1];
        phase_sync_fwd<MODE, W, true>(p, sh, tid, st, nullptr, af, &tie);
        packed = phase_sync_rev<MODE, W, true>(p, sh, tid, q0, st, nullptr, af, &tie);
        if (BL_COLD(wave_any(tie)) && (tid & 63) == 0) sh.redo = 1;
    } else if (MODE == MODE_SYNCMER) {
        uint32_t af[S + 1];
        phase_sync_fwd<MODE, W>(p, sh, tid, st, nullptr, af);
        packed = phase_sync_rev<MODE, W>(p, sh, tid, q0, st, nullptr, af);
    } else if (MAX) {
        packed = phase_window<MODE, W, MAX>(p, sh, tid, q0, st, nullptr, &tie);
        if (BL_COLD(wave_any(tie)) && (tid & 63) == 0) sh.redo = 1;
    } else {
        packed = phase_window<MODE, W>(p, sh, tid, q0, st, nullptr);
    }

    uint32_t total;
    const uint32_t excl = block_excl_scan(packed, sh.wave_tot, tid, total);
    const uint32_t n_s = total & 0xffffu, n_e = total >> 16;
    phase_list<MODE, W>(sh, tid, st, excl & 0xffffu, excl >> 16);
    if (tid == 0) p.tile_counts[tile] = (unsigned long long)n_s | ((unsigned long long)n_e << 32);
    __syncthreads();
    if (SY != 0 && tid == 0 && BL_COLD(sh.redo != 0)) p.redo_list[atomicAdd(p.redo_count, 1ull)] = tile;

    const size_t slot = (size_t)tile * p.stride;
    spill_list(p.slots_a + slot, sh.list_a, n_s, tid);
    if (MODE == MODE_SUPERKMER) {
        spill_list(p.slots_j + slot, sh.list_j, n_s, tid);
        spill_list(p.slots_e + slot, sh.list_e, n_e, tid);
    }
}

template <int MODE, int W, int NS, int LIM_LAST, bool GENERIC, bool APPROX = false, int U = 0>
__device__ __forceinline__ void count_tile_frl(const ScanParams& p, TileShared<MODE, W>& sh, uint32_t tile, int tid)
{
    const int64_t q0 = tile_q0(p, tile);
    phase_load_frl<MODE, W>(p, sh, tid, q0);
    if (APPROX && tid == 0) sh.redo = 0;
    {
        uint32_t* sc = p.slots_c + (size_t)tile * p.slot_chunks;
        for (int c = tid; c < p.slot_chunks; c += TPB) sc[c] = sh.codes[c];
    }
    __syncthreads();

    ThreadState st;
    bool tie = false;
    phase_hash_frl<MODE, W, NS, GENERIC, APPROX, U>(p, sh, tid, q0, tile, st);
    phase_window_frl_a<MODE, W, NS, LIM_LAST, APPROX>(p, sh, tid, st, nullptr, &tie);
    if (APPROX && BL_COLD(wave_any(tie)) && (tid & 63) == 0) sh.redo = 1;
    const uint32_t packed = phase_window_frl_b<MODE, W, NS>(p, tid, st, nullptr);

    uint32_t total;
    const uint32_t excl = block_excl_scan(packed, sh.wave_tot, tid, total);
    const uint32_t n_s = total & 0xffffu, n_e = total >> 16;
    phase_list_frl<MODE, W, NS>(sh, st, excl & 0xffffu, excl >> 16);
    if (tid == 0) p.tile_counts[tile] = (unsigned long long)n_s | ((unsigned long long)n_e << 32);
    __syncthreads();
    if (APPROX && tid == 0 && BL_COLD(sh.redo != 0)) p.redo_list[atomicAdd(p.redo_count, 1ull)] = tile;
    const size_t slot = (size_t)tile * p.stride;
    spill_list(p.slots_a + slot, sh.list_a, n_s, tid);
    if (MODE == MODE_SUPERKMER) {
        spill_list(p.slots_j + slot, sh.list_j, n_s, tid);
        spill_list(p.slots_e + slot, sh.list_e, n_e, tid);
    }
}

constexpr int C3_RC = NCHUNK + 4;
template <int MODE, bool LOOPED = false, bool C3 = false, bool WIDE = false>
__device__ __forceinline__ void emit_tile(const ScanParams& p, uint32_t* codes, uint32_t tile, int tid, Digest& dg)
{
    const int64_t q0 = tile_q0(p, tile);
    const size_t slot = (size_t)tile * p.stride;
    const unsigned long long cnt = uniform64(p.tile_counts[tile]);
    const unsigned long long base = uniform64(p.tile_base[tile] + p.block_base[tile / SCAN_BLK]);
    const int needed = staged_chunks(p);
    const uint32_t* sc = p.slots_c + (size_t)tile * p.slot_chunks;
    const uint32_t c0 = (MODE != MODE_SYNCMER && tid < needed) ? sc[tid] : 0;
    const uint32_t c1 = (MODE != MODE_SYNCMER && TPB + tid < needed) ? sc[TPB + tid] : 0;
    const uint16_t* la = p.slots_a + slot;
    const uint16_t* lj = MODE == MODE_SUPERKMER ? p.slots_j + slot : nullptr;
    const bool in0 = tid < p.stride, in1 = TPB + tid < p.stride;
    const uint32_t a0 = in0 ? la[tid] : 0, a1 = in1 ? la[TPB + tid] : 0;
    uint32_t j0 = 0, j1 = 0;
    if (MODE == MODE_SUPERKMER) {
        j0 = in0 ? lj[tid] : 0;
        j1 = in1 ? lj[TPB + tid] : 0;
    }
    const uint32_t n_s = (uint32_t)cnt, n_e = (uint32_t)(cnt >> 32);
    if (n_s == 0 && n_e == 0) {
        if (LOOPED && MODE != MODE_SYNCMER) __syncthreads();
        return;
    }
    const uint64_t base_s = base & 0xffffffffull, base_e = base >> 32;
    if (C3) {
        if (tid < needed) {
            codes[1 + tid] = c0;
            codes[C3_RC + needed - tid] = revcomp16(c0);
        }
        if (TPB + tid < needed) {
            codes[1 + TPB + tid] = c1;
            codes[C3_RC + needed - TPB - tid] = revcomp16(c1);
        }
        __syncthreads();
    } else if (MODE != MODE_SYNCMER) {
        if (tid < needed) codes[tid] = c0;
        if (TPB + tid < needed) codes[TPB + tid] = c1;
        __syncthreads();
    }
    const bool fits = !BL_COLD(base_s + n_s > p.capacity);
    TileLists L{codes, la, lj, MODE == MODE_SUPERKMER ? p.slots_e + slot : nullptr, MODE == MODE_SUPERKMER ? p.slots_e + slot + p.stride : nullptr};
    const uint32_t d = (uint32_t)(base_s - base_e);
    auto one = [&](uint32_t r, uint32_t ent, uint32_t ent_j) {
        const Record rec = C3 ? emit_prepare_c3<LOOPED>(p, codes + 1, codes + C3_RC + 1, needed, q0, ent, dg) : emit_prepare<MODE, LOOPED>(p, codes, q0, ent, ent_j, dg);
        if (fits) emit_store<MODE, false>(p, rec, base_s + r);
        else emit_store<MODE, true>(p, rec, base_s + r);
        if (MODE == MODE_SUPERKMER && (p.out_size || p.out_records) && (fits || base_s + r < p.capacity)) {
            const int size = (int)(end_position(p, L, tile, q0, r + d, n_e) - (int64_t)rec.first + 1);
            if (p.out_size) p.out_size[base_s + r] = (uint8_t)size;
            if (WIDE) {
                if (p.out_records) emit_record128(p, codes, needed - 1, q0, rec, size, base_s + r);
            } else if (p.out_records) {
                emit_record(p, codes, needed - 1, q0, rec, size, base_s + r);
            }
        }
    };
    if ((uint32_t)tid < n_s) one(tid, a0, j0);
    if (LOOPED) BL_SCHED_FENCE();
    if ((uint32_t)(TPB + tid) < n_s) one(TPB + tid, a1, j1);
    if (LOOPED) BL_SCHED_FENCE();
#pragma unroll 1
    for (uint32_t r = 2 * TPB + tid; r < n_s; r += TPB) one(r, la[r], MODE == MODE_SUPERKMER ? lj[r] : 0u);
}

template <int MODE, int W, int U, int C, int SY = 0>
__global__ __launch_bounds__(TPB, (MODE == MODE_MINIMIZER && SY == 2 ? BL_POSAX_WAVES : MODE == MODE_SUPERKMER && SY == 2 ? BL_SKAX_WAVES : SY == 1 && W < 0 ? BL_CSRT_WAVES : SY == 1 ? BL_CS_WAVES : SY == 2 ? BL_SY2_WAVES : (MODE == MODE_SYNCMER && W > 0 ? BL_SY0_WAVES : MODE == MODE_SYNCMER || (MODE == MODE_SUPERKMER && W == -32) ? 2 : (W == -32 || (W < 0 && MODE == MODE_SUPERKMER) ? 3 : (W == -16 ? 5 : (W < 0 ? 4 : (W <= 11 ? 5 : (MODE == MODE_SUPERKMER && W == 17 && U == 15 ? BL_C4_WAVES : 4)))))))) void scan_count_kernel(const ScanParams pin, GroupRange g)
{
    __shared__ TileShared<MODE, W> sh;
    ScanParams p = pin;
    if (U != 0) p.unit = U;
    if (W > 0) {
        p.w = W;
        p.stride = NWAVE * (64 * S - 16 * ((W + 15) / 16));
    }
    if (C >= 0) p.canonical = C;
    if (blockIdx.x < g.count) count_tile<MODE, W, SY, U>(p, sh, g.first + blockIdx.x, threadIdx.x);
}

template <int MODE, int W, int U, int C>
__global__ __launch_bounds__(TPB, 2) void scan_redo_kernel(const ScanParams pin)
{
    __shared__ TileShared<MODE, W> sh;
    ScanParams p = pin;
    if (U != 0) p.unit = U;
    if (W > 0) {
        p.w = W;
        p.stride = NWAVE * (64 * S - 16 * ((W + 15) / 16));
    }
    if (C >= 0) p.canonical = C;
    const unsigned long long n = *p.redo_count;
    for (unsigned long long i = blockIdx.x; i < n; i += gridDim.x) {
        count_tile<MODE, W>(p, sh, p.redo_list[i], threadIdx.x);
        __syncthreads();
    }
}

template <int MODE, int W, int NS, int U, int L, int C>
__device__ __forceinline__ ScanParams frl_params(const ScanParams& pin)
{
    ScanParams p = pin;
    p.w = W;
    p.ns = NS;
    if (U != 0) p.unit = U;
    if (C >= 0) p.canonical = C;
    if (L != 0) {
        constexpr int nu = L - U + 1, lpr = (nu + S - 1) / S, rpw = 64 / (lpr > 0 ? lpr : 1);
        p.read_len = L;
        p.lpr = lpr;
        p.rpw = rpw;
        p.nwin = nu - W + 1;
        p.lpr_inv = (65536u + lpr - 1) / lpr;
        p.stride = NWAVE * rpw * L;
        p.slot_chunks = (15 + NWAVE * rpw * L + 15) / 16 + 3;
    }
    return p;
}
template <int W, int NS, int U, int L>
constexpr int frl_lim_last() { return L != 0 ? (L - U + 1 - W + 1) - ((L - U + 1 + S - 1) / S - 1) * NS : 0; }

#ifndef BL_FRL_WAVES
#define BL_FRL_WAVES 5
#endif
template <int MODE, int W, int NS, int U, int L, int C, bool APPROX = false>
__global__ __launch_bounds__(TPB, (W <= 11 ? BL_FRL_WAVES : 4)) void scan_count_frl_kernel(const ScanParams pin, GroupRange g)
{
    __shared__ TileShared<MODE, W> sh;
    const ScanParams p = frl_params<MODE, W, NS, U, L, C>(pin);
    constexpr int LIM_LAST = frl_lim_last<W, NS, U, L>();
    static_assert(L == 0 || (LIM_LAST >= 1 && LIM_LAST <= NS), "read-tiled geometry: the last lane of a read must own 1..NS windows");
    if (blockIdx.x < g.count) count_tile_frl<MODE, W, NS, LIM_LAST, U == 0, APPROX, U>(p, sh, g.first + blockIdx.x, threadIdx.x);
}

template <int MODE, int W, int NS, int U, int L, int C>
__global__ __launch_bounds__(TPB, (W <= 11 ? 5 : 4)) void scan_redo_frl_kernel(const ScanParams pin)
{
    __shared__ TileShared<MODE, W> sh;
    const ScanParams p = frl_params<MODE, W, NS, U, L, C>(pin);
    const unsigned long long n = *p.redo_count;
    for (unsigned long long i = blockIdx.x; i < n; i += gridDim.x) {
        count_tile_frl<MODE, W, NS, frl_lim_last<W, NS, U, L>(), U == 0, false, U>(p, sh, p.redo_list[i], threadIdx.x);
        __syncthreads();
    }
}

#ifndef BL_EMIT_TILES
#define BL_EMIT_TILES 4
#endif
template <int MODE>
constexpr int emit_tiles() { return MODE == MODE_MINIMIZER ? BL_EMIT_TILES : 1; }

template <int MODE, int U, int C, int FRL>
constexpr bool emit_c3() { return MODE == MODE_MINIMIZER && U == 31 && C == 1 && FRL == 1; }
template <int MODE, int U = 0, int C = -1, int FRL = -1, bool WIDE = false>
__global__ __launch_bounds__(TPB) void scan_emit_kernel(const ScanParams pin, GroupRange g)
{
    static_assert(!WIDE || (MODE == MODE_SUPERKMER && U == 0), "32-byte records are super-k-mer groups; the unit length comes from the arguments");
    constexpr int K = emit_tiles<MODE>();
    constexpr bool C3 = emit_c3<MODE, U, C, FRL>();
    __shared__ uint32_t codes[K > 1 ? 2 : 1][C3 ? 2 * C3_RC : NCHUNK];
    const int tid = threadIdx.x;
    ScanParams p = pin;
    if (U != 0) p.unit = U;
    if (C >= 0) p.canonical = C;
    if (FRL >= 0) p.frl = FRL;
    Digest dg{0, 0, 0};
    if constexpr (K > 1) {
        __shared__ uint32_t acc[6][TPB];
#pragma unroll
        for (int i = 0; i < 6; ++i) acc[i][tid] = 0;
        const uint32_t t0 = blockIdx.x * K;
#pragma unroll 1
        for (uint32_t k = 0; k < (uint32_t)K && t0 + k < g.count; ++k) {
            Digest d1{0, 0, 0};
            emit_tile<MODE, true, C3>(p, codes[k & 1], g.first + t0 + k, tid, d1);
            acc[0][tid] ^= (uint32_t)d1.xv; acc[1][tid] ^= (uint32_t)(d1.xv >> 32);
            acc[2][tid] ^= (uint32_t)d1.xh; acc[3][tid] ^= (uint32_t)(d1.xh >> 32);
            acc[4][tid] ^= (uint32_t)d1.xp; acc[5][tid] ^= (uint32_t)(d1.xp >> 32);
        }
        dg.xv = ((unsigned long long)acc[1][tid] << 32) | acc[0][tid];
        dg.xh = ((unsigned long long)acc[3][tid] << 32) | acc[2][tid];
        dg.xp = ((unsigned long long)acc[5][tid] << 32) | acc[4][tid];
    } else {
        if (blockIdx.x >= g.count) return;
        emit_tile<MODE, false, C3, WIDE>(p, codes[0], g.first + blockIdx.x, tid, dg);
    }

    const unsigned long long xv = MODE == MODE_SYNCMER ? 0ull : wave_xor_to_last_u64(dg.xv), xh = MODE == MODE_SYNCMER ? 0ull : wave_xor_to_last_u64(dg.xh);
    const unsigned long long xp = wave_xor_to_last_u64(dg.xp);
    if ((tid & 63) == 63 && (xv | xh | xp)) {
        unsigned long long* shard = p.shards + 8 * ((blockIdx.x * NWAVE + (tid >> 6)) % NSHARD);
        if (MODE != MODE_SYNCMER) {
            atomicXor(&shard[1], xv);
            atomicXor(&shard[2], xh);
        }
        atomicXor(&shard[3], xp);
    }
}

__global__ __launch_bounds__(512) void tile_scan_local_kernel(const unsigned long long* counts, unsigned long long* tile_base,
                                                              unsigned long long* block_tot, uint32_t first_tile, uint32_t n_group)
{
    __shared__ unsigned long long wtot[8];
    const int tid = threadIdx.x, lane = tid & 63, wv = tid >> 6;
    const uint32_t rel = blockIdx.x * SCAN_BLK + tid * 4;
    unsigned long long c[4], run = 0;
#pragma unroll
    for (int i = 0; i < 4; ++i) {
        c[i] = rel + i < n_group ? counts[first_tile + rel + i] : 0;
        run += c[i];
    }
    unsigned long long incl = run;
#pragma unroll
    for (int d = 1; d < 64; d <<= 1) {
        const unsigned long long o = __shfl_up(incl, d, 64);
        if (lane >= d) incl += o;
    }
    if (lane == 63) wtot[wv] = incl;
    __syncthreads();
    unsigned long long before = 0, all = 0;
#pragma unroll
    for (int i = 0; i < 8; ++i) {
        if (i < wv) before += wtot[i];
        all += wtot[i];
    }
    unsigned long long ex = before + incl - run;
#pragma unroll
    for (int i = 0; i < 4; ++i) {
        if (rel + i < n_group) tile_base[first_tile + rel + i] = ex;
        ex += c[i];
    }
    if (tid == 0) block_tot[first_tile / SCAN_BLK + blockIdx.x] = all;
}

__global__ void tile_scan_top_kernel(const unsigned long long* block_tot, unsigned long long* block_base, uint32_t first_block,
                                     uint32_t n_blocks, unsigned long long* carry, unsigned long long* shards)
{
    if (blockIdx.x != 0 || threadIdx.x >= 64) return;
    const uint32_t lane = threadIdx.x, per = (n_blocks + 63) / 64;
    const uint32_t lo = lane * per, hi = lo + per < n_blocks ? lo + per : n_blocks;
    unsigned long long sum = 0;
    for (uint32_t i = lo; i < hi; ++i) sum += block_tot[first_block + i];
    unsigned long long incl = sum;
#pragma unroll
    for (int d = 1; d < 64; d <<= 1) {
        const unsigned long long o = __shfl_up(incl, d, 64);
        if ((int)lane >= d) incl += o;
    }
    const unsigned long long before = *carry;
    unsigned long long run = before + incl - sum;
    for (uint32_t i = lo; i < hi; ++i) {
        block_base[first_block + i] = run;
        run += block_tot[first_block + i];
    }
    const unsigned long long total = __shfl(incl, 63, 64);
    if (lane == 0) {
        *carry = before + total;
        shards[0] += total & 0xffffffffull;
        shards[4] += total >> 32;
    }
}

struct KmerShared {
    uint32_t codes[NCHUNK_POS];
    uint32_t flags[NCHUNK_POS];
    unsigned long long dig[4];
};

__global__ __launch_bounds__(TPB) void kmer_kernel(const KmerParams p)
{
    __shared__ KmerShared sh;
    const int tid = threadIdx.x;
    KmerAcc acc{0, 0, 0, 0};
    if (tid < 4) sh.dig[tid] = 0;
    ScanParams lp{};
    lp.bases = p.bases;
    lp.n_bases = p.n_bases;
    lp.start_bits = p.start_bits;
    for (int tile = blockIdx.x; tile < p.n_tiles; tile += gridDim.x) {
        const int64_t q0 = p.origin + (int64_t)tile * H;
        __syncthreads();
        stage_chunk(lp, sh.codes, sh.flags, tid, q0);
        if (tid < NCHUNK_POS - TPB) stage_chunk(lp, sh.codes, sh.flags, TPB + tid, q0);
        __syncthreads();
        kmer_thread(p, sh.codes, sh.flags, tid, q0, acc);
    }
    __syncthreads();
    const unsigned long long c = wave_sum_u64(acc.cnt), xv = wave_xor_u64(acc.xv), xh = wave_xor_u64(acc.xh), s = wave_sum_u64(acc.sh);
    if ((tid & 63) == 0) {
        atomicAdd(&sh.dig[0], c);
        atomicXor(&sh.dig[1], xv);
        atomicXor(&sh.dig[2], xh);
        atomicAdd(&sh.dig[3], s);
    }
    __syncthreads();
    if (tid < 4) {
        unsigned long long* shard = p.shards + 8 * (blockIdx.x % NSHARD);
        if (tid == 0 || tid == 3) atomicAdd(&shard[tid], sh.dig[tid]);
        else atomicXor(&shard[tid], sh.dig[tid]);
    }
}


__global__ void reduce_shards_kernel(const unsigned long long* shards, unsigned long long* result, uint32_t add_mask, const unsigned long long* redone)
{
    const int slot = threadIdx.x;
    if (slot == 8) result[8] = 0;
    if (slot == 9) result[5] = *redone;
    if (slot >= 8) return;
    if (slot == 5) return;
    unsigned long long acc = 0;
    for (int i = 0; i < NSHARD; ++i) {
        const unsigned long long v = shards[8 * i + slot];
        if ((add_mask >> slot) & 1) acc += v;
        else acc ^= v;
    }
    result[slot] = acc;
}

__global__ void synth_kernel(uint8_t* bases, uint64_t first, uint64_t n, uint64_t seed)
{
    const uint64_t wordi = (uint64_t)blockIdx.x * blockDim.x + threadIdx.x;
    const uint64_t i0 = wordi * 32;
    if (i0 >= n) return;
    uint64_t x = seed + ((first + i0) >> 5);
    x += 0x9E3779B97F4A7C15ULL;
    x = (x ^ (x >> 30)) * 0xBF58476D1CE4E5B9ULL;
    x = (x ^ (x >> 27)) * 0x94D049BB133111EBULL;
    x ^= x >> 31;
    const uint32_t lut = 0x54474341u;
    uint32_t out[8];
#pragma unroll
    for (int q = 0; q < 8; ++q) {
        const uint32_t c4 = (uint32_t)(x >> (8 * q)) & 0xffu;
        const uint32_t sel = (c4 & 3u) | (((c4 >> 2) & 3u) << 8) | (((c4 >> 4) & 3u) << 16) | (((c4 >> 6) & 3u) << 24);
        out[q] = __builtin_amdgcn_perm(lut, lut, sel);
    }
    if (i0 + 32 <= n) {
        uint4* dst = reinterpret_cast<uint4*>(bases + i0);
        dst[0] = make_uint4(out[0], out[1], out[2], out[3]);
        dst[1] = make_uint4(out[4], out[5], out[6], out[7]);
    } else {
        for (uint64_t b = 0; i0 + b < n; ++b) bases[i0 + b] = (uint8_t)(out[b >> 2] >> (8 * (b & 3)));
    }
}

__global__ void start_bits_fixed_kernel(uint32_t* bits, uint64_t n_words, uint64_t n_bases, uint64_t read_len)
{
    const uint64_t wi = (uint64_t)blockIdx.x * blockDim.x + threadIdx.x;
    if (wi >= n_words) return;
    const uint64_t p0 = wi * 32;
    uint64_t r = p0 % read_len;
    uint64_t nxt = r == 0 ? p0 : p0 + (read_len - r);
    uint32_t w = 0;
    while (nxt < p0 + 32 && nxt < n_bases) {
        w |= 1u << (nxt - p0);
        nxt += read_len;
    }
    bits[wi] = w;
}

__global__ void start_bits_offsets_kernel(uint32_t* bits, const uint64_t* offsets, uint64_t n_seqs, uint64_t n_bases)
{
    const uint64_t q = (uint64_t)blockIdx.x * blockDim.x + threadIdx.x;
    if (q >= n_seqs) return;
    const uint64_t p = offsets[q];
    if (p < n_bases && offsets[q + 1] > p) atomicOr(&bits[p >> 5], 1u << (p & 31));
}


#define BL_LAUNCH(NAME, KERNEL, GRID, BLOCK, LDS, ...)                          \
    do {                                                                       \
        if (log) log->add(NAME);                                               \
        hipLaunchKernelGGL(KERNEL, GRID, BLOCK, LDS, stream, __VA_ARGS__);     \
    } while (0)
#define BL_MODE_NAME(HEAD, TAIL) (MODE == MODE_MINIMIZER ? HEAD "MM" TAIL : MODE == MODE_SUPERKMER ? HEAD "SK" TAIL : HEAD "SY" TAIL)

#define BL_W_ALL(X)                                                                                                                      \
    X(2) X(3) X(4) X(5) X(6) X(7) X(8) X(9) X(10) X(11) X(12) X(13) X(14) X(15) X(16) X(17) X(18) X(19) X(20) X(21) X(22) X(23) X(24)    \
    X(25) X(26) X(27) X(28) X(29) X(30) X(31) X(32)

static const char* const SCAN_KERNEL_NAMES[] = {
    "frl<MM,W=11,NS=15,U=31,L=150,approx>", "frl_redo<MM,W=11,NS=15,U=31,L=150>", "frl<MM,W=11,NS=15,U=31,L=150>",
    "frl<MM,W=11,NS=14,U=31,approx>", "frl_redo<MM,W=11,NS=14,U=31>", "frl<MM,W=11,NS=14,U=31>",
    "frl<MM,W=11,NS=15,U=31,approx>", "frl_redo<MM,W=11,NS=15,U=31>", "frl<MM,W=11,NS=15,U=31>",
    "frl<MM,W=11,NS=16,U=31,approx>", "frl_redo<MM,W=11,NS=16,U=31>", "frl<MM,W=11,NS=16,U=31>",
    "frl<MM,W=5>", "frl<MM,W=10>", "frl<MM,W=11>", "frl<MM,W=19>", "frl<SK,W=17>",
#ifndef BL_NO_POSAX
    "count<MM,W=11,U=31,C=1,approx>", "redo<MM,W=11,U=31,C=1>",
#endif
    "count<MM,W=11,U=31,C=1>",
#ifdef BL_SKAX
    "count<SK,W=17,U=15,C=1,approx>", "redo<SK,W=17,U=15,C=1>",
#endif
    "count<SK,W=17,U=15,C=1>",
    "count<SY,W=21,U=11,C=1,closed>", "redo<SY,W=21,U=11,C=1>",
#ifndef BL_NO_SY2
    "count<SY,W=21,U=11,C=1,deferred>",
#else
    "count<SY,W=21,U=11,C=1>",
#endif
    "count<SY,closed,W<=17>", "count<SY,closed,W<=32>",
#define BL_W(WV) "count<MM,W=" #WV ">", "count<SK,W=" #WV ">",
    BL_W_ALL(BL_W)
#undef BL_W
    "count<MM,W=1>", "count<SK,W=1>", "count<SY,W=1>", "count<SY,W=11>", "count<SY,W=17>", "count<SY,W=21>",
    "count<SY,W<=16>", "count<SY,W<=32>", "count<MM,W>32>", "count<SK,W>32>",
    "emit<MM>", "emit<SK>", "emit<SY>", "emit<MM,C3>", "emit<SK,wide>",
};

const char* const* scan_kernel_names(int* count)
{
    *count = (int)(sizeof(SCAN_KERNEL_NAMES) / sizeof(SCAN_KERNEL_NAMES[0]));
    return SCAN_KERNEL_NAMES;
}

static hipError_t launch_count_frl(int mode, const ScanParams& p, GroupRange g, hipStream_t stream, LaunchLog* log)
{
    const dim3 grid(g.count), block(TPB);
    if (mode == MODE_MINIMIZER && p.w == 11 && p.unit == 31 && p.canonical && p.read_len == 150 && p.ns == 15 && p.rpw == 8) {
        if (p.redo_list && g.first == 0 && !p.exact_windows) {
            BL_LAUNCH("frl<MM,W=11,NS=15,U=31,L=150,approx>", (scan_count_frl_kernel<MODE_MINIMIZER, 11, 15, 31, 150, 1, true>), grid, block, 0, p, g);
            BL_LAUNCH("frl_redo<MM,W=11,NS=15,U=31,L=150>", (scan_redo_frl_kernel<MODE_MINIMIZER, 11, 15, 31, 150, 1>), dim3(g.count < 512u ? g.count : 512u), block, 0, p);
        } else {
            BL_LAUNCH("frl<MM,W=11,NS=15,U=31,L=150>", (scan_count_frl_kernel<MODE_MINIMIZER, 11, 15, 31, 150, 1>), grid, block, 0, p, g);
        }
        return hipGetLastError();
    }
    if (mode == MODE_MINIMIZER && p.w == 11 && p.unit == 31 && p.canonical && p.ns >= 14 && p.ns <= 16) {
        const bool approx = p.redo_list && g.first == 0 && !p.exact_windows;
        const dim3 redo_grid(g.count < 512u ? g.count : 512u);
#define BL_FRL_SHAPE(NSV)                                                                                                                                    \
    if (approx) {                                                                                                                                            \
        BL_LAUNCH("frl<MM,W=11,NS=" #NSV ",U=31,approx>", (scan_count_frl_kernel<MODE_MINIMIZER, 11, NSV, 31, 0, 1, true>), grid, block, 0, p, g);            \
        BL_LAUNCH("frl_redo<MM,W=11,NS=" #NSV ",U=31>", (scan_redo_frl_kernel<MODE_MINIMIZER, 11, NSV, 31, 0, 1>), redo_grid, block, 0, p);                   \
    } else {                                                                                                                                                 \
        BL_LAUNCH("frl<MM,W=11,NS=" #NSV ",U=31>", (scan_count_frl_kernel<MODE_MINIMIZER, 11, NSV, 31, 0, 1>), grid, block, 0, p, g);                         \
    }
        if (p.ns == 14) { BL_FRL_SHAPE(14) } else if (p.ns == 15) { BL_FRL_SHAPE(15) } else { BL_FRL_SHAPE(16) }
#undef BL_FRL_SHAPE
        return hipGetLastError();
    }
    if (p.ns != S) return hipErrorInvalidValue;
    if (mode == MODE_MINIMIZER) {
        switch (p.w) {
            case 5: BL_LAUNCH("frl<MM,W=5>", (scan_count_frl_kernel<MODE_MINIMIZER, 5, S, 0, 0, -1>), grid, block, 0, p, g); break;
            case 10: BL_LAUNCH("frl<MM,W=10>", (scan_count_frl_kernel<MODE_MINIMIZER, 10, S, 0, 0, -1>), grid, block, 0, p, g); break;
            case 11: BL_LAUNCH("frl<MM,W=11>", (scan_count_frl_kernel<MODE_MINIMIZER, 11, S, 0, 0, -1>), grid, block, 0, p, g); break;
            case 19: BL_LAUNCH("frl<MM,W=19>", (scan_count_frl_kernel<MODE_MINIMIZER, 19, S, 0, 0, -1>), grid, block, 0, p, g); break;
            default: return hipErrorInvalidValue;
        }
    } else if (mode == MODE_SUPERKMER && p.w == 17) {
        BL_LAUNCH("frl<SK,W=17>", (scan_count_frl_kernel<MODE_SUPERKMER, 17, S, 0, 0, -1>), grid, block, 0, p, g);
    } else {
        return hipErrorInvalidValue;
    }
    return hipGetLastError();
}

template <int MODE>
static hipError_t launch_count_mode(const ScanParams& p, GroupRange g, hipStream_t stream, LaunchLog* log)
{
    const dim3 grid(g.count), block(TPB);
    if (MODE == MODE_MINIMIZER && p.w == 11 && p.unit == 31 && p.canonical) {
#ifndef BL_NO_POSAX
        if (p.redo_list && g.first == 0 && !p.exact_windows) {
            BL_LAUNCH("count<MM,W=11,U=31,C=1,approx>", (scan_count_kernel<MODE_MINIMIZER, 11, 31, 1, 2>), grid, block, 0, p, g);
            BL_LAUNCH("redo<MM,W=11,U=31,C=1>", (scan_redo_kernel<MODE_MINIMIZER, 11, 31, 1>), dim3(g.count < 512u ? g.count : 512u), block, 0, p);
            return hipGetLastError();
        }
#endif
        BL_LAUNCH("count<MM,W=11,U=31,C=1>", (scan_count_kernel<MODE, 11, 31, 1>), grid, block, 0, p, g);
        return hipGetLastError();
    }
    if (MODE == MODE_SUPERKMER && p.w == 17 && p.unit == 15 && p.canonical) {
#ifdef BL_SKAX
        if (p.redo_list && g.first == 0 && !p.exact_windows) {
            BL_LAUNCH("count<SK,W=17,U=15,C=1,approx>", (scan_count_kernel<MODE_SUPERKMER, 17, 15, 1, 2>), grid, block, 0, p, g);
            BL_LAUNCH("redo<SK,W=17,U=15,C=1>", (scan_redo_kernel<MODE_SUPERKMER, 17, 15, 1>), dim3(g.count < 512u ? g.count : 512u), block, 0, p);
            return hipGetLastError();
        }
#endif
        BL_LAUNCH("count<SK,W=17,U=15,C=1>", (scan_count_kernel<MODE, 17, 15, 1>), grid, block, 0, p, g);
        return hipGetLastError();
    }
    if (MODE == MODE_SYNCMER && p.w == 21 && p.unit == 11 && p.canonical) {
        const bool closed = (p.soff == 0 && p.eoff == 20) || (p.soff == 20 && p.eoff == 0);
        const unsigned redo_grid = g.count < 512u ? g.count : 512u;
        if (closed && !p.exact_windows && p.redo_list && g.first == 0) {
            BL_LAUNCH("count<SY,W=21,U=11,C=1,closed>", (scan_count_kernel<MODE_SYNCMER, 21, 11, 1, 1>), grid, block, 0, p, g);
            BL_LAUNCH("redo<SY,W=21,U=11,C=1>", (scan_redo_kernel<MODE_SYNCMER, 21, 11, 1>), dim3(redo_grid), block, 0, p);
#ifndef BL_NO_SY2
        } else if (p.redo_list && g.first == 0) {
            BL_LAUNCH("count<SY,W=21,U=11,C=1,deferred>", (scan_count_kernel<MODE_SYNCMER, 21, 11, 1, 2>), grid, block, 0, p, g);
            BL_LAUNCH("redo<SY,W=21,U=11,C=1>", (scan_redo_kernel<MODE_SYNCMER, 21, 11, 1>), dim3(redo_grid), block, 0, p);
#endif
        } else {
            BL_LAUNCH("count<SY,W=21,U=11,C=1>", (scan_count_kernel<MODE, 21, 11, 1>), grid, block, 0, p, g);
        }
        return hipGetLastError();
    }
    if (MODE == MODE_SYNCMER && p.w <= 32 && !p.exact_windows && ((p.soff == 0 && p.eoff == p.w - 1) || (p.soff == p.w - 1 && p.eoff == 0))) {
        if (p.w <= 17) BL_LAUNCH("count<SY,closed,W<=17>", (scan_count_kernel<MODE_SYNCMER, -8, 0, -1, 1>), grid, block, 0, p, g);
        else BL_LAUNCH("count<SY,closed,W<=32>", (scan_count_kernel<MODE_SYNCMER, -16, 0, -1, 1>), grid, block, 0, p, g);
        return hipGetLastError();
    }
    if (MODE != MODE_SYNCMER && p.w >= 2 && p.w <= 32) {
        constexpr int MM = MODE == MODE_SYNCMER ? MODE_MINIMIZER : MODE;
        switch (p.w) {
#define BL_W(WV) case WV: BL_LAUNCH(BL_MODE_NAME("count<", ",W=" #WV ">"), (scan_count_kernel<MM, WV, 0, -1>), grid, block, 0, p, g); return hipGetLastError();
            BL_W_ALL(BL_W)
#undef BL_W
        }
    }
    switch (p.w) {
        case 1: BL_LAUNCH(BL_MODE_NAME("count<", ",W=1>"), (scan_count_kernel<MODE, 1, 0, -1>), grid, block, 0, p, g); break;
        case 11: BL_LAUNCH(BL_MODE_NAME("count<", ",W=11>"), (scan_count_kernel<MODE, 11, 0, -1>), grid, block, 0, p, g); break;
        case 17: BL_LAUNCH(BL_MODE_NAME("count<", ",W=17>"), (scan_count_kernel<MODE, 17, 0, -1>), grid, block, 0, p, g); break;
        case 21: BL_LAUNCH(BL_MODE_NAME("count<", ",W=21>"), (scan_count_kernel<MODE, 21, 0, -1>), grid, block, 0, p, g); break;
        default:
            if constexpr (MODE == MODE_SYNCMER) {
                if (p.w <= 16) { BL_LAUNCH("count<SY,W<=16>", (scan_count_kernel<MODE, -8, 0, -1>), grid, block, 0, p, g); break; }
                if (p.w <= 32) { BL_LAUNCH("count<SY,W<=32>", (scan_count_kernel<MODE, -16, 0, -1>), grid, block, 0, p, g); break; }
            }
            BL_LAUNCH(BL_MODE_NAME("count<", ",W>32>"), (scan_count_kernel<MODE, -32, 0, -1>), grid, block, 0, p, g);
            break;
    }
    return hipGetLastError();
}

hipError_t launch_scan_count(int mode, const ScanParams& p, GroupRange g, hipStream_t stream, LaunchLog* log)
{
    if (g.count == 0) return hipSuccess;
    if (p.frl) return launch_count_frl(mode, p, g, stream, log);
    switch (mode) {
        case MODE_MINIMIZER: return launch_count_mode<MODE_MINIMIZER>(p, g, stream, log);
        case MODE_SUPERKMER: return launch_count_mode<MODE_SUPERKMER>(p, g, stream, log);
        case MODE_SYNCMER: return launch_count_mode<MODE_SYNCMER>(p, g, stream, log);
    }
    return hipErrorInvalidValue;
}

template <int MODE>
static void launch_emit_mode(const ScanParams& p, GroupRange g, hipStream_t stream, uint32_t lds_per_wg, LaunchLog* log)
{
    constexpr int K = emit_tiles<MODE>();
    const uint32_t have = (uint32_t)(((K > 1 ? 2 : 1) * NCHUNK + (K > 1 ? 6 * TPB : 0)) * sizeof(uint32_t));
    const uint32_t pad = lds_per_wg > have ? lds_per_wg - have : 0;
    const dim3 grid((g.count + K - 1) / K), block(TPB);
    if (MODE == MODE_MINIMIZER && p.frl && p.unit == 31 && p.canonical) {
        const uint32_t have_c3 = (uint32_t)(((K > 1 ? 2 : 1) * 2 * C3_RC + (K > 1 ? 6 * TPB : 0)) * sizeof(uint32_t));
        BL_LAUNCH("emit<MM,C3>", (scan_emit_kernel<MODE_MINIMIZER, 31, 1, 1>), grid, block, lds_per_wg > have_c3 ? lds_per_wg - have_c3 : 0, p, g);
        return;
    }
    if (MODE == MODE_SUPERKMER && p.records128) {
        BL_LAUNCH("emit<SK,wide>", (scan_emit_kernel<MODE_SUPERKMER, 0, -1, -1, true>), grid, block, pad, p, g);
        return;
    }
    BL_LAUNCH(BL_MODE_NAME("emit<", ">"), (scan_emit_kernel<MODE>), grid, block, pad, p, g);
}

hipError_t launch_scan_emit(int mode, const ScanParams& p, GroupRange g, hipStream_t stream, uint32_t lds_per_wg, LaunchLog* log)
{
    if (g.count == 0) return hipSuccess;
    switch (mode) {
        case MODE_MINIMIZER: launch_emit_mode<MODE_MINIMIZER>(p, g, stream, lds_per_wg, log); break;
        case MODE_SUPERKMER: launch_emit_mode<MODE_SUPERKMER>(p, g, stream, lds_per_wg, log); break;
        case MODE_SYNCMER: launch_emit_mode<MODE_SYNCMER>(p, g, stream, lds_per_wg, log); break;
        default: return hipErrorInvalidValue;
    }
    return hipGetLastError();
}
#undef BL_LAUNCH
#undef BL_MODE_NAME
#undef BL_W_ALL

hipError_t launch_tile_scan(const ScanParams& p, GroupRange g, unsigned long long* block_tot, unsigned long long* carry, hipStream_t stream)
{
    if (g.count == 0) return hipSuccess;
    const uint32_t n_blocks = (g.count + SCAN_BLK - 1) / SCAN_BLK;
    hipLaunchKernelGGL(tile_scan_local_kernel, dim3(n_blocks), dim3(512), 0, stream, p.tile_counts, p.tile_base, block_tot, g.first, g.count);
    hipLaunchKernelGGL(tile_scan_top_kernel, dim3(1), dim3(64), 0, stream, block_tot, p.block_base, g.first / SCAN_BLK, n_blocks, carry,
                       p.shards);
    return hipGetLastError();
}

hipError_t launch_kmers(const KmerParams& p, int n_blocks, hipStream_t stream)
{
    if (p.n_tiles <= 0) return hipSuccess;
    hipLaunchKernelGGL(kmer_kernel, dim3(n_blocks), dim3(TPB), 0, stream, p);
    return hipGetLastError();
}

hipError_t launch_reduce_shards(const unsigned long long* shards, unsigned long long* result, uint32_t add_mask, const unsigned long long* redone, hipStream_t stream)
{
    hipLaunchKernelGGL(reduce_shards_kernel, dim3(1), dim3(64), 0, stream, shards, result, add_mask, redone);
    return hipGetLastError();
}

hipError_t launch_synth(uint8_t* bases, uint64_t first, uint64_t n, uint64_t seed, hipStream_t stream)
{
    if (n == 0) return hipSuccess;
    const uint64_t words = (n + 31) / 32;
    hipLaunchKernelGGL(synth_kernel, dim3((unsigned)((words + 255) / 256)), dim3(256), 0, stream, bases, first, n, seed);
    return hipGetLastError();
}

hipError_t launch_start_bits_fixed(uint32_t* bits, uint64_t n_words, uint64_t n_bases, uint64_t read_len, hipStream_t stream)
{
    if (n_words == 0) return hipSuccess;
    hipLaunchKernelGGL(start_bits_fixed_kernel, dim3((unsigned)((n_words + 255) / 256)), dim3(256), 0, stream, bits, n_words, n_bases, read_len);
    return hipGetLastError();
}

hipError_t launch_start_bits_offsets(uint32_t* bits, const uint64_t* offsets, uint64_t n_seqs, uint64_t n_bases, hipStream_t stream)
{
    if (n_seqs == 0) return hipSuccess;
    hipLaunchKernelGGL(start_bits_offsets_kernel, dim3((unsigned)((n_seqs + 255) / 256)), dim3(256), 0, stream, bits, offsets, n_seqs, n_bases);
    return hipGetLastError();
}

}

#ifdef BL_EXPERIMENT_COUNT_FALLBACK
extern "C" unsigned long long bl_dbg_read_fallbacks()
{
    unsigned long long v = 0;
    (void)hipDeviceSynchronize();
    (void)hipMemcpyFromSymbol(&v, HIP_SYMBOL(bl::bl_dbg_fallbacks), sizeof(v));
    return v;
}
#endif
```

### biolib_amd/csrc/bl_launch.hpp

```cpp
#pragma once
#include <hip/hip_runtime.h>
#include "bl_scan_phases.hpp"

namespace bl {
struct LaunchLog {
    static constexpr int MAX = 8;
    const char* names[MAX];
    int n;
    void add(const char* name) { if (n < MAX) names[n++] = name; }
};
const char* const* scan_kernel_names(int* count);
hipError_t launch_scan_count(int mode, const ScanParams& p, GroupRange g, hipStream_t stream, LaunchLog* log);
hipError_t launch_scan_emit(int mode, const ScanParams& p, GroupRange g, hipStream_t stream, uint32_t lds_per_wg, LaunchLog* log);
hipError_t launch_tile_scan(const ScanParams& p, GroupRange g, unsigned long long* block_tot, unsigned long long* carry, hipStream_t stream);
hipError_t launch_kmers(const KmerParams& p, int n_blocks, hipStream_t stream);
hipError_t launch_reduce_shards(const unsigned long long* shards, unsigned long long* result, uint32_t add_mask, const unsigned long long* redone, hipStream_t stream);
hipError_t launch_synth(uint8_t* bases, uint64_t first, uint64_t n, uint64_t seed, hipStream_t stream);
hipError_t launch_start_bits_fixed(uint32_t* bits, uint64_t n_words, uint64_t n_bases, uint64_t read_len, hipStream_t stream);
hipError_t launch_start_bits_offsets(uint32_t* bits, const uint64_t* offsets, uint64_t n_seqs, uint64_t n_bases, hipStream_t stream);
}
```

### biolib_amd/csrc/bl_scan_core.hpp

```cpp
#pragma once
#include <stdint.h>

#if defined(__HIPCC__) && !defined(BL_CPU_EMU)
#define BL_DEV __host__ __device__ __forceinline__
#define BL_UNROLL _Pragma("unroll")
#else
#define BL_DEV static inline
#define BL_UNROLL
#endif

#ifdef BL_CENSUS_HOT
#define BL_COLD(c) (false)
#else
#define BL_COLD(c) (c)
#endif

#if defined(__HIP_DEVICE_COMPILE__) && !defined(BL_CPU_EMU) && !defined(BL_NO_SCHED_FENCE)
#define BL_SCHED_FENCE() __builtin_amdgcn_sched_barrier(0)
#else
#define BL_SCHED_FENCE() do {} while (0)
#endif

namespace bl {

constexpr int TPB = 256;
constexpr int S = 16;
constexpr int H = TPB * S;
constexpr int NCHUNK = 512;
constexpr int NCHUNK_POS = H / 16 + 8;
constexpr int MAX_UNIT = 32;
constexpr int MAX_W = 64;
constexpr int NSHARD = 256;
constexpr int SCAN_BLK = 2048;
constexpr int NWAVE_CORE = TPB / 64;

enum ScanMode { MODE_MINIMIZER = 0, MODE_SUPERKMER = 1, MODE_SYNCMER = 2 };

struct ScanParams {
    const uint8_t* bases;
    int64_t n_bases;
    const uint32_t* start_bits;
    int64_t win_first, win_end;
    int64_t origin;
    int64_t pos_base;
    int32_t n_tiles;
    int32_t stride;
    int32_t unit, w;
    uint32_t seed;
    int32_t canonical;
    int32_t soff, eoff;
    int32_t drop_last;
    int32_t use_threshold;
    uint64_t hash_below;
    uint64_t* out_value;
    uint64_t* out_pos;
    uint64_t* out_hash;
    uint64_t* out_first;
    uint8_t* out_mmpos;
    uint8_t* out_size;
    uint64_t* out_records;
    uint64_t capacity;
    unsigned long long* tile_counts;
    unsigned long long* tile_base;
    unsigned long long* block_base;
    uint16_t* slots_a;
    uint16_t* slots_j;
    uint16_t* slots_e;
    uint32_t* slots_c;
    int32_t slot_chunks;
    unsigned long long* shards;
    int32_t exact_windows;
    uint32_t* redo_list;
    unsigned long long* redo_count;
    int32_t frl;
    int32_t read_len;
    int32_t lpr, rpw, ns;
    int32_t nwin;
    uint32_t lpr_inv;
    int64_t n_reads;
    int32_t records128;
};

BL_DEV bool frl_width_built(int mode, int w)
{
    return (mode == MODE_MINIMIZER && (w == 11 || w == 5 || w == 10 || w == 19)) || (mode == MODE_SUPERKMER && w == 17);
}

BL_DEV bool plan_scan_frl(int64_t first, int64_t end, int64_t n_bases, int64_t read_len, int unit, int w, int ns_fixed, ScanParams& p)
{
    if (read_len <= 0 || read_len > 4096 || first % read_len != 0) return false;
    if (end % read_len != 0 || end > n_bases || end <= first) return false;
    const int L = (int)read_len;
    const int nu = L - unit + 1, nwin = nu - w + 1;
    if (nwin < 1 || w < 2) return false;
    const int lpr = (nu + S - 1) / S;
    if (lpr > 64) return false;
    const int ns = ns_fixed ? ns_fixed : (nu + lpr - 1) / lpr;
    if (ns * lpr < nu || ns > S || w - 1 > 3 * ns) return false;
    int rpw = 64 / lpr;
    const int cap = (NCHUNK * 16 - 64 - 32) / NWAVE_CORE / L;
    if (rpw > cap) rpw = cap;
    if (rpw < 1) return false;
    const double frl_eff = (double)(rpw * nwin) / (64.0 * ns);
    const double pos_eff = (double)nwin / L * (double)(64 * S - 16 * ((w + 15) / 16)) / (64.0 * S);
    if (frl_eff <= pos_eff) return false;
    p.frl = 1;
    p.read_len = L;
    p.lpr = lpr;
    p.rpw = rpw;
    p.ns = ns;
    p.nwin = nwin;
    p.lpr_inv = (65536u + (uint32_t)lpr - 1) / (uint32_t)lpr;
    p.n_reads = (end - first) / L;
    p.win_first = first;
    p.win_end = end;
    p.origin = first;
    p.stride = NWAVE_CORE * rpw * L;
    p.n_tiles = (int32_t)((p.n_reads + NWAVE_CORE * rpw - 1) / (NWAVE_CORE * rpw));
    p.slot_chunks = (15 + p.stride + 15) / 16 + 3;
    return true;
}

BL_DEV bool plan_scan_frl_for(int mode, int64_t first, int64_t end, int64_t n_bases, int64_t read_len, int unit, int w, bool canonical, ScanParams& p)
{
    if (mode == MODE_MINIMIZER && w == 11 && unit == 31 && canonical) {
        ScanParams q = p;
        if (plan_scan_frl(first, end, n_bases, read_len, unit, w, 0, q) && q.ns >= 14 && q.ns <= 16) {
            p = q;
            return true;
        }
    }
    return plan_scan_frl(first, end, n_bases, read_len, unit, w, S, p);
}

struct GroupRange {
    uint32_t first, count;
};

BL_DEV int64_t align_down16(int64_t x) { return x >= 0 ? (x & ~15LL) : -(((-x) + 15) & ~15LL); }

BL_DEV void plan_scan(int mode, int64_t first, int64_t end, int w, ScanParams& p)
{
    p.win_first = first;
    p.win_end = end;
    p.stride = (TPB / 64) * (64 * S - 16 * ((w + 15) / 16));
    p.origin = align_down16(mode == MODE_SYNCMER ? first : first - 1);
    p.n_tiles = end > first ? (int32_t)((end - 1 - p.origin) / p.stride + 1) : 0;
    p.frl = 0;
    p.slot_chunks = NCHUNK_POS;
}

BL_DEV uint64_t rotl64(uint64_t x, int r) { return (x << r) | (x >> (64 - r)); }

BL_DEV uint64_t rotl64_31(uint64_t x)
{
#if defined(__HIP_DEVICE_COMPILE__) && !defined(BL_CPU_EMU)
    const uint32_t lo = (uint32_t)x, hi = (uint32_t)(x >> 32);
    const uint32_t nh = __builtin_amdgcn_alignbit(hi, lo, 1), nl = __builtin_amdgcn_alignbit(lo, hi, 1);
    return ((uint64_t)nh << 32) | nl;
#else
    return rotl64(x, 31);
#endif
}

template <bool SPELLED = false>
BL_DEV uint64_t mul64c_as(uint64_t a, uint64_t c)
{
    const uint32_t alo = (uint32_t)a, ahi = (uint32_t)(a >> 32);
    const uint32_t clo = (uint32_t)c, chi = (uint32_t)(c >> 32);
    uint32_t cross = alo * chi + ahi * clo;
#if defined(__HIP_DEVICE_COMPILE__) && !defined(BL_CPU_EMU)
    asm("" : "+v"(cross));
    if (SPELLED) {
        uint64_t d, carry;
        asm("v_mad_u64_u32 %0, %1, %2, %3, %4" : "=v"(d), "=s"(carry) : "v"(alo), "s"(clo), "v"((uint64_t)cross << 32));
        return d;
    }
#endif
    return (uint64_t)alo * clo + ((uint64_t)cross << 32);
}
BL_DEV uint64_t mul64c(uint64_t a, uint64_t c) { return mul64c_as<false>(a, c); }

BL_DEV uint64_t fmix64(uint64_t k)
{
    k ^= k >> 33;
    k = mul64c(k, 0xff51afd7ed558ccdULL);
    k ^= k >> 33;
    k = mul64c(k, 0xc4ceb9fe1a85ec53ULL);
    k ^= k >> 33;
    return k;
}

BL_DEV uint64_t murmur64(uint64_t key, uint32_t seed)
{
    uint64_t k1 = mul64c(key, 0x87c37b91114253d5ULL);
    k1 = rotl64_31(k1);
    k1 = mul64c(k1, 0x4cf5ad432745937fULL);
    uint64_t h1 = (uint64_t)seed ^ k1;
    uint64_t h2 = (uint64_t)seed;
    h1 ^= 8; h2 ^= 8;
    h1 += h2; h2 += h1;
    h1 = fmix64(h1); h2 = fmix64(h2);
    return h1 + h2;
}

BL_DEV uint64_t mad_lo(uint32_t a, uint32_t b, uint64_t c)
{
#if defined(__HIP_DEVICE_COMPILE__) && !defined(BL_CPU_EMU)
    uint64_t d, carry;
    asm("v_mad_u64_u32 %0, %1, %2, %3, %4" : "=v"(d), "=s"(carry) : "v"(a), "s"(b), "v"(c));
    return d;
#else
    return (uint64_t)(uint32_t)(a * b + (uint32_t)c);
#endif
}
template <bool PLUS_ONE = false>
BL_DEV uint64_t mad_lo0(uint32_t a, uint32_t b)
{
#if defined(__HIP_DEVICE_COMPILE__) && !defined(BL_CPU_EMU)
    uint64_t d, carry;
    if (PLUS_ONE) asm("v_mad_u64_u32 %0, %1, %2, %3, 1" : "=v"(d), "=s"(carry) : "v"(a), "s"(b));
    else asm("v_mad_u64_u32 %0, %1, %2, %3, 0" : "=v"(d), "=s"(carry) : "v"(a), "s"(b));
    return d;
#else
    return (uint64_t)(uint32_t)(a * b + (PLUS_ONE ? 1u : 0u));
#endif
}
template <bool PLUS_ONE = false>
BL_DEV uint32_t murmur64_top(uint64_t key, uint32_t seed)
{
    uint64_t k1 = mul64c(key, 0x87c37b91114253d5ULL);
    k1 = rotl64_31(k1);
    k1 = mul64c(k1, 0x4cf5ad432745937fULL);
    uint64_t h1 = (uint64_t)seed ^ k1;
    uint64_t h2 = (uint64_t)seed;
    h1 ^= 8; h2 ^= 8;
    h1 += h2; h2 += h1;
    h1 ^= h1 >> 33;
    h1 = mul64c_as<true>(h1, 0xff51afd7ed558ccdULL);
    h1 ^= h1 >> 33;
    h2 ^= h2 >> 33;
    h2 = mul64c_as<true>(h2, 0xff51afd7ed558ccdULL);
    h2 ^= h2 >> 33;
    const uint32_t clo = 0x1a85ec53u, chi = 0xc4ceb9feu;
    const uint32_t a1 = (uint32_t)h1, b1 = (uint32_t)(h1 >> 32), a2 = (uint32_t)h2, b2 = (uint32_t)(h2 >> 32);
    const uint32_t cross = (uint32_t)mad_lo(b1 + b2, clo, mad_lo0<PLUS_ONE>(a1 + a2, chi));
#if defined(__HIP_DEVICE_COMPILE__) && !defined(BL_CPU_EMU)
    uint32_t top;
    asm("v_add3_u32 %0, %1, %2, %3" : "=v"(top) : "v"(__umulhi(a1, clo)), "v"(__umulhi(a2, clo)), "v"(cross));
    return top;
#else
    return (uint32_t)(((uint64_t)a1 * clo) >> 32) + (uint32_t)(((uint64_t)a2 * clo) >> 32) + cross;
#endif
}

BL_DEV uint64_t fmix64_plain(uint64_t k)
{
    k ^= k >> 33;
    k *= 0xff51afd7ed558ccdULL;
    k ^= k >> 33;
    k *= 0xc4ceb9fe1a85ec53ULL;
    k ^= k >> 33;
    return k;
}
BL_DEV uint64_t murmur64_plain(uint64_t key, uint32_t seed)
{
    uint64_t k1 = key * 0x87c37b91114253d5ULL;
    k1 = rotl64_31(k1);
    k1 *= 0x4cf5ad432745937fULL;
    uint64_t h1 = (uint64_t)seed ^ k1;
    uint64_t h2 = (uint64_t)seed;
    h1 ^= 8; h2 ^= 8;
    h1 += h2; h2 += h1;
    h1 = fmix64_plain(h1); h2 = fmix64_plain(h2);
    return h1 + h2;
}

BL_DEV uint32_t byte_perm(uint32_t hi, uint32_t lo, uint32_t sel)
{
#if defined(__HIP_DEVICE_COMPILE__) && !defined(BL_CPU_EMU)
    return __builtin_amdgcn_perm(hi, lo, sel);
#else
    uint64_t both = ((uint64_t)hi << 32) | lo;
    uint32_t r = 0;
    for (int i = 0; i < 4; ++i) {
        uint32_t s = (sel >> (8 * i)) & 0xff;
        uint32_t byte = s < 8 ? (uint32_t)((both >> (8 * s)) & 0xff) : 0;
        r |= byte << (8 * i);
    }
    return r;
#endif
}

BL_DEV bool wave_any(bool pred)
{
#if defined(__HIP_DEVICE_COMPILE__) && !defined(BL_CPU_EMU)
    return __builtin_amdgcn_ballot_w64(pred) != 0;
#else
    return pred;
#endif
}

BL_DEV void encode4(uint32_t d, uint32_t& code8, uint32_t& diff)
{
    uint32_t x = (d >> 1) & 0x03030303u;
    x ^= (x >> 1) & 0x01010101u;
    const uint32_t lut = 0x74676361u;
    const uint32_t expect = byte_perm(lut, lut, x);
    diff = ((d | 0x20202020u) ^ expect) & ~((x & (x >> 1)) & 0x01010101u);
    code8 = (x * 0x40100401u) >> 24;
}

BL_DEV uint32_t bad_bits4(uint32_t diff)
{
    const uint32_t nz = (((diff & 0x7f7f7f7fu) + 0x7f7f7f7fu) | diff) & 0x80808080u;
    return ((nz >> 7) * 0x00204081u >> 21) & 0xfu;
}

BL_DEV void encode16(const uint32_t d[4], uint32_t& code, uint32_t& bad)
{
    uint32_t c0, c1, c2, c3, f0, f1, f2, f3;
    encode4(d[0], c0, f0);
    encode4(d[1], c1, f1);
    encode4(d[2], c2, f2);
    encode4(d[3], c3, f3);
    code = (c0 << 24) | (c1 << 16) | (c2 << 8) | c3;
    bad = 0;
    if (BL_COLD(wave_any((f0 | f1 | f2 | f3) != 0))) bad = bad_bits4(f0) | (bad_bits4(f1) << 4) | (bad_bits4(f2) << 8) | (bad_bits4(f3) << 12);
}

BL_DEV uint64_t pairrev64(uint64_t x)
{
    uint64_t r = __builtin_bitreverse64(x);
    return ((r >> 1) & 0x5555555555555555ULL) | ((r & 0x5555555555555555ULL) << 1);
}

struct Roller {
    uint32_t flo, fhi;
    uint32_t rlo, rhi;
    uint32_t next16;
    int unit;
};
BL_DEV uint64_t roller_fwd(const Roller& r) { return ((uint64_t)r.fhi << 32) | r.flo; }
BL_DEV uint64_t roller_rc(const Roller& r) { return ((uint64_t)r.rhi << 32) | r.rlo; }

BL_DEV uint32_t funnel_shr(uint32_t hi, uint32_t lo, int n)
{
#if defined(__HIP_DEVICE_COMPILE__) && !defined(BL_CPU_EMU)
    return __builtin_amdgcn_alignbit(hi, lo, n);
#else
    return (uint32_t)((((uint64_t)hi << 32) | lo) >> n);
#endif
}

BL_DEV void roller_start(Roller& r, uint32_t c0, uint32_t c1, uint32_t c2, int unit)
{
    const uint64_t A = ((uint64_t)c0 << 32) | c1;
    const uint64_t B = ((uint64_t)c1 << 32) | c2;
    const int pre = unit - 1;
    uint64_t fwd = 0, rc = 0;
    if (pre != 0) {
        fwd = A >> (64 - 2 * pre);
        uint64_t little = pairrev64(fwd) >> (64 - 2 * pre);
        little ^= (pre == 32) ? ~0ULL : ((1ULL << (2 * pre)) - 1);
        rc = little << 2;
    }
    r.flo = (uint32_t)fwd;
    r.fhi = (uint32_t)(fwd >> 32);
    r.rlo = (uint32_t)rc;
    r.rhi = (uint32_t)(rc >> 32);
    r.next16 = pre < 16 ? (uint32_t)((A << (2 * pre)) >> 32) : (uint32_t)((B << (2 * (pre - 16))) >> 32);
    r.unit = unit;
}

BL_DEV void roller_step(Roller& r, int s)
{
    const int at = 30 - 2 * s;
    const uint32_t c = (r.next16 >> at) & 3u;
    const int top = 2 * (r.unit - 1);
    if (r.unit > 16) {
        const uint32_t nhi = funnel_shr(r.fhi, r.flo, 30);
        r.flo = (r.flo << 2) | c;
        r.fhi = r.unit == 32 ? nhi : (nhi & ((1u << (2 * r.unit - 32)) - 1u));
        r.rlo = funnel_shr(r.rhi, r.rlo, 2);
// ... 291 lines not shown
```

### biolib_amd/csrc/bl_scan_frl.hpp

```cpp
#pragma once
#include "bl_scan_phases.hpp"

namespace bl {

BL_DEV int64_t tile_q0(const ScanParams& p, uint32_t tile)
{
    const int64_t g = p.origin + (int64_t)tile * p.stride;
    return p.frl ? (g & ~15LL) : g;
}

BL_DEV bool stage_chunk_frl(const ScanParams& p, uint32_t* codes, uint32_t* flags, int c, int64_t q0)
{
    const int64_t g = q0 + 16 * (int64_t)c;
    uint32_t d[4] = {0, 0, 0, 0};
    if (g + 16 <= p.n_bases) {
        const Vec16 v = *reinterpret_cast<const Vec16*>(p.bases + g);
        d[0] = v.x; d[1] = v.y; d[2] = v.z; d[3] = v.w;
    } else if (BL_COLD(g < p.n_bases)) {
        for (int b = 0; b < 16; ++b) {
            const int64_t q = g + b;
            if (q < p.n_bases) d[b >> 2] |= (uint32_t)p.bases[q] << (8 * (b & 3));
        }
    }
    uint32_t code, bad;
    encode16(d, code, bad);
    codes[c] = code;
    flags[c] = ~bad & 0xffffu;
    return bad != 0;
}

template <int MODE, int W>
BL_DEV void phase_load_frl(const ScanParams& p, TileShared<MODE, W>& sh, int tid, int64_t q0)
{
    bool bad = false;
    for (int c = tid; c < p.slot_chunks; c += TPB) bad |= stage_chunk_frl(p, sh.codes, sh.flags, c, q0);
    const int wv = wave_index(tid);
#if defined(__HIP_DEVICE_COMPILE__) && !defined(BL_CPU_EMU)
    const bool any = wave_any(bad);
    if ((tid & 63) == 0) sh.wave_bad[wv] = any ? 1u : 0u;
#else
    if ((tid & 63) == 0) sh.wave_bad[wv] = 0;
    if (bad) sh.wave_bad[wv] = 1;
#endif
}


BL_DEV uint64_t bases_ending_at(uint32_t a0, uint32_t a1, uint32_t a2, int e)
{
    const int q = e >> 4, sh = 30 - 2 * (e & 15);
    const uint32_t w[3] = {a0, a1, a2};
    const uint32_t lo = sh == 0 ? w[q] : (q == 0 ? w[0] >> sh : funnel_shr(w[q - 1], w[q], sh));
    const uint32_t hi = q == 0 ? 0u : (sh == 0 ? w[q - 1] : (q == 1 ? w[0] >> sh : funnel_shr(w[q - 2], w[q - 1], sh)));
    return ((uint64_t)hi << 32) | lo;
}

template <int U>
BL_DEV void units_direct(uint32_t a0, uint32_t a1, uint32_t a2, uint32_t r0, uint32_t r1, uint32_t r2, int s, uint64_t& fw, uint64_t& rv)
{
    static_assert(U > 16 && U <= 32, "direct extraction: 16 < U <= 32");
    constexpr uint64_t M = U == 32 ? ~0ull : (1ull << (2 * U)) - 1;
    fw = bases_ending_at(a0, a1, a2, s + U - 1) & M;
    rv = bases_ending_at(r0, r1, r2, 47 - s) & M;
}

template <int MODE, int W, int NS, bool GENERIC = false, bool APPROX = false, int U = 0>
BL_DEV void phase_hash_frl(const ScanParams& p, TileShared<MODE, W>& sh, int tid, int64_t q0, uint32_t tile, ThreadState& st)
{
    const int wv = wave_index(tid), lane = tid & 63;
    const int r = (int)(((uint32_t)lane * p.lpr_inv) >> 16);
    const int j = lane - r * p.lpr;
    const int64_t read_idx = ((int64_t)tile * NWAVE + wv) * p.rpw + r;
    const bool active = r < p.rpw && read_idx < p.n_reads;
    const int off0 = (int)(p.origin + (int64_t)tile * p.stride - q0);
    const int base = active ? off0 + (wv * p.rpw + r) * p.read_len + j * NS : off0;
    st.lane_base = base;
    st.jlane = active ? j : -1;
    const uint32_t* cp = sh.codes + (base >> 4);
    const uint32_t c0 = cp[0], c1 = cp[1], c2 = cp[2], c3 = cp[3];
    const int sh2 = 2 * (base & 15);
    const uint32_t a0 = (uint32_t)(((((uint64_t)c0 << 32) | c1) << sh2) >> 32);
    const uint32_t a1 = (uint32_t)(((((uint64_t)c1 << 32) | c2) << sh2) >> 32);
    const uint32_t a2 = (uint32_t)(((((uint64_t)c2 << 32) | c3) << sh2) >> 32);
    constexpr bool DIRECT_OK = !GENERIC && (U == 0 || U == 31) && NS + 31 - 1 <= 47;
    if (DIRECT_OK && (U == 31 || p.unit == 31)) {
        const uint32_t r0 = revcomp16(a2), r1 = revcomp16(a1), r2 = revcomp16(a0);
        BL_UNROLL
        for (int s = 0; s < NS; ++s) {
            uint64_t fw, rv;
            units_direct<31>(a0, a1, a2, r0, r1, r2, s, fw, rv);
            const uint64_t v = (p.canonical && rv < fw) ? rv : fw;
            st.h[s] = APPROX ? (uint64_t)murmur64_top<true>(v, p.seed) << 32 : murmur64(v, p.seed);
        }
        return;
    }
    Roller rr;
    roller_start(rr, a0, a1, a2, p.unit);
    BL_UNROLL
    for (int s = 0; s < NS; ++s) {
        roller_step(rr, s);
        const uint64_t fw = roller_fwd(rr), rv = roller_rc(rr);
        const uint64_t v = (p.canonical && rv < fw) ? rv : fw;
        if (APPROX) st.h[s] = (uint64_t)murmur64_top<true>(v, p.seed) << 32;
        else st.h[s] = GENERIC ? murmur64_plain(v, p.seed) : murmur64(v, p.seed);
    }
}

#if defined(__HIP_DEVICE_COMPILE__) && !defined(BL_CPU_EMU)
BL_DEV uint32_t dpp_next32(uint32_t v) { return (uint32_t)__builtin_amdgcn_update_dpp(0, (int)v, 0x130, 0xf, 0xf, true); }
BL_DEV uint32_t dpp_next32_rot(uint32_t v) { return (uint32_t)__builtin_amdgcn_update_dpp(0, (int)v, 0x134, 0xf, 0xf, true); }
BL_DEV uint32_t dpp_prev32(uint32_t v) { return (uint32_t)__builtin_amdgcn_update_dpp(0, (int)v, 0x138, 0xf, 0xf, true); }
BL_DEV uint32_t dpp_next32_rot_add(uint32_t v, uint32_t k)
{
    uint32_t d;
    asm("s_nop 1\n\tv_add_u32_dpp %0, %1, %2 wave_rol:1 row_mask:0xf bank_mask:0xf" : "=v"(d) : "v"(v), "v"(k));
    return d;
}
#endif

template <int NS, int W, bool APPROX = false>
BL_DEV void lane_window_argmin_frl(const ThreadState* all, int tid, const ThreadState& st, bool owns, uint32_t* a, bool* tie = nullptr)
{
    constexpr int NE = W - 1, NK = NS + NE;
    uint32_t key[NK];
    BL_UNROLL
    for (int s = 0; s < NS; ++s) key[s] = packed_key((uint32_t)(st.h[s] >> 32), s, true);
#if defined(__HIP_DEVICE_COMPILE__) && !defined(BL_CPU_EMU)
    (void)all;
    (void)tid;
    if constexpr (APPROX && NE <= NS) {
        const uint32_t ns = (uint32_t)NS;
        BL_UNROLL
        for (int x = 0; x < NE; ++x) key[NS + x] = dpp_next32_rot_add(key[x], ns);
    } else {
        uint32_t cur[NS];
        BL_UNROLL
        for (int x = 0; x < NS; ++x) cur[x] = key[x];
        BL_UNROLL
        for (int hop = 0; hop * NS < NE; ++hop) {
            BL_UNROLL
            for (int x = 0; x < NS; ++x) {
                if (hop * NS + x < NE || (hop + 1) * NS + x < NE || (hop + 2) * NS + x < NE)
                    cur[x] = dpp_next32_rot(cur[x]) + (uint32_t)NS;
                if (hop * NS + x < NE) key[(hop + 1) * NS + x] = cur[x];
            }
        }
    }
#else
    {
        const int lane = tid & 63;
        for (int x = 0; x < NE; ++x) {
            const int nb = lane + 1 + x / NS;
            const uint32_t hi = nb < 64 ? (uint32_t)(all[tid + 1 + x / NS].h[x % NS] >> 32) : (0x03fffff0u - 4u * (uint32_t)x) << 6;
            key[NS + x] = packed_key(hi, NS + x, true);
        }
    }
#endif
    const uint32_t dmin = window_argmin_packed<NS, W, true, true, APPROX>(key, a);
    if (APPROX) {
        uint32_t amin = a[NS - 1];
        BL_UNROLL
        for (int s = 0; s < NS - 1; s += W) amin = a[s] < amin ? a[s] : amin;
        if (owns && (dmin < 128u || amin < 64u)) *tie = true;
        return;
    }
    if (BL_COLD(wave_any(owns && dmin < 64u))) {
        uint64_t e[NK];
        BL_UNROLL
        for (int s = 0; s < NS; ++s) e[s] = st.h[s];
#if defined(__HIP_DEVICE_COMPILE__) && !defined(BL_CPU_EMU)
        uint64_t cur[NS];
        BL_UNROLL
        for (int x = 0; x < NS; ++x) cur[x] = st.h[x];
        BL_UNROLL
        for (int hop = 0; hop * NS < NE; ++hop) {
            BL_UNROLL
            for (int x = 0; x < NS; ++x) {
                if (hop * NS + x < NE || (hop + 1) * NS + x < NE || (hop + 2) * NS + x < NE) cur[x] = lane_next(cur[x]);
                if (hop * NS + x < NE) e[(hop + 1) * NS + x] = cur[x];
            }
        }
#else
        const int lane = tid & 63;
        for (int x = 0; x < NE; ++x) {
            const int nb = lane + 1 + x / NS;
            e[NS + x] = nb < 64 ? all[tid + 1 + x / NS].h[x % NS] : 0xDEADBEEFDEADBEEFull;
        }
#endif
        window_argmin<NS, W, true>(e, a);
    }
}

template <int NS>
BL_DEV uint32_t frl_good_mask(const ScanParams& p, const uint32_t* flags, int base, int span)
{
    const int ch = base >> 4, off = base & 15;
    uint64_t g[3] = {0, 0, 0};
    for (int c = 0; c < 9; ++c) {
        int idx = ch + c;
        idx = idx < p.slot_chunks ? idx : p.slot_chunks - 1;
        g[c >> 2] |= (uint64_t)(flags[idx] & 0xffffu) << (16 * (c & 3));
    }
    Bits128 good;
    good.lo = off ? (g[0] >> off) | (g[1] << (64 - off)) : g[0];
    good.hi = off ? (g[1] >> off) | (g[2] << (64 - off)) : g[1];
    return (uint32_t)and_run(good, span).lo & ((1u << NS) - 1);
}

template <int MODE, int W, int NS>
constexpr bool frl_occ_form() { return MODE == MODE_MINIMIZER && W > 1 && W - 1 <= NS && NS + W - 1 <= 32; }

template <int MODE, int W, int NS, int LIM_LAST = 0, bool APPROX = false>
BL_DEV void phase_window_frl_a(const ScanParams& p, TileShared<MODE, W>& sh, int tid, ThreadState& st, const ThreadState* all, bool* tie = nullptr)
{
    uint32_t a[S];
    lane_window_argmin_frl<NS, (W > 1 ? W : 2), APPROX>(all, tid, st, st.jlane >= 0, a, tie);
    uint32_t vmask = 0;
    if (st.jlane >= 0) {
        int lim = p.nwin - st.jlane * NS;
        lim = lim < 0 ? 0 : (lim > NS ? NS : lim);
        vmask = (1u << lim) - 1u;
    }
    const uint32_t tile_bad = sh.wave_bad[0] | sh.wave_bad[1] | sh.wave_bad[2] | sh.wave_bad[3];
    if (BL_COLD(tile_bad)) vmask &= frl_good_mask<NS>(p, sh.flags, st.lane_base, p.unit + (W > 0 ? W : p.w) - 1);
    st.vmask = vmask;
    if (frl_occ_form<MODE, W, NS>()) {
        uint32_t occ = 0;
        if (LIM_LAST == 0 || BL_COLD(tile_bad)) {
            BL_UNROLL
            for (int s = 0; s < NS; ++s) occ |= ((vmask >> s) & 1u) << (a[s] & 31u);
        } else {
            BL_UNROLL
            for (int s = 0; s < NS; ++s) occ |= 1u << (a[s] & 31u);
            const uint32_t a_sel = st.jlane == p.lpr - 1 ? a[LIM_LAST > 0 ? LIM_LAST - 1 : 0] : a[NS - 1];
            occ &= (2u << (a_sel & 31u)) - 1u;
            if (st.jlane < 0) occ = 0;
        }
        st.occ = occ;
        return;
    }
    BL_UNROLL
    for (int s = NS; s < S; ++s) a[s] = 0;
    uint32_t apk[4];
    BL_UNROLL
    for (int q = 0; q < 4; ++q) {
        const uint32_t lo2 = byte_perm(a[4 * q + 1], a[4 * q], 0x0c0c0400u);
        const uint32_t hi2 = byte_perm(a[4 * q + 3], a[4 * q + 2], 0x04000c0cu);
        apk[q] = (lo2 | hi2) & 0x3f3f3f3fu;
    }
    st.apk0 = ((uint64_t)apk[1] << 32) | apk[0];
    st.apk1 = ((uint64_t)apk[3] << 32) | apk[2];
    st.a_first = a[0] & 63u;
    st.a_last = a[NS - 1] & 63u;
}

template <int MODE, int W, int NS>
BL_DEV uint32_t phase_window_frl_b(const ScanParams& p, int tid, ThreadState& st, const ThreadState* all)
{
    if (frl_occ_form<MODE, W, NS>()) {
#if defined(__HIP_DEVICE_COMPILE__) && !defined(BL_CPU_EMU)
        (void)all;
        (void)tid;
        const uint32_t prev = dpp_prev32(st.occ);
#else
        const uint32_t prev = (tid & 63) > 0 ? all[tid - 1].occ : 0u;
#endif
        st.endm = 0;
        st.emit = (st.occ | (prev >> NS)) & ((1u << NS) - 1u);
        return (uint32_t)__builtin_popcount(st.emit);
    }
#if defined(__HIP_DEVICE_COMPILE__) && !defined(BL_CPU_EMU)
    (void)all;
    (void)tid;
    const uint32_t prev_last = dpp_prev32(st.a_last), prev_vm = dpp_prev32(st.vmask);
    const uint32_t next_first = dpp_next32(st.a_first), next_vm = dpp_next32(st.vmask);
#else
    const int lane = tid & 63;
    const uint32_t prev_last = lane > 0 ? all[tid - 1].a_last : 0xAAu, prev_vm = lane > 0 ? all[tid - 1].vmask : 0xAAAAu;
    const uint32_t next_first = lane < 63 ? all[tid + 1].a_first : 0x55u, next_vm = lane < 63 ? all[tid + 1].vmask : 0x5555u;
#endif
    const int j = st.jlane;
    const uint32_t apk[4] = {(uint32_t)st.apk0, (uint32_t)(st.apk0 >> 32), (uint32_t)st.apk1, (uint32_t)(st.apk1 >> 32)};
    const uint32_t p0 = (prev_last - (uint32_t)NS) & 0x7fu;
    uint32_t differ = 0;
    BL_UNROLL
    for (int q = 0; q < 4; ++q) {
        const uint32_t prv = q ? funnel_shr(apk[q], apk[q - 1], 24) : ((apk[0] << 8) | p0);
        const uint32_t x = apk[q] ^ prv;
        const uint32_t nz = ((x + 0x7f7f7f7fu) >> 7) & 0x01010101u;
        differ |= ((nz * 0x01020408u) >> 24) << (4 * q);
    }
    const uint32_t vm = st.vmask;
    const uint32_t pv = (j > 0) ? ((prev_vm >> (NS - 1)) & 1u) : 0u;
    const uint32_t vprev = (vm << 1) | pv;
    st.emit = vm & (~vprev | differ);
    st.endm = 0;
    if (MODE == MODE_SUPERKMER) {
        const uint32_t nv = (j >= 0 && j < p.lpr - 1) ? (next_vm & 1u) : 0u;
        const uint32_t dn = ((next_first + (uint32_t)NS) != st.a_last) ? 1u : 0u;
        const uint32_t vnext = (vm >> 1) | (nv << (NS - 1));
        const uint32_t dnext = (differ >> 1) | (dn << (NS - 1));
        st.endm = vm & (~vnext | dnext);
    }
    return (uint32_t)__builtin_popcount(st.emit) | ((uint32_t)__builtin_popcount(st.endm) << 16);
}

template <int MODE, int W, int NS = 0>
BL_DEV void phase_list_frl(TileShared<MODE, W>& sh, const ThreadState& st, uint32_t excl_s, uint32_t excl_e)
{
    uint32_t m = st.emit;
    uint32_t r = excl_s;
    if (NS != 0 && frl_occ_form<MODE, W, (NS ? NS : 1)>()) {
        while (m) {
            const int s = __builtin_ctz(m);
            m &= m - 1;
            sh.list_a[r] = (uint16_t)(st.lane_base + s);
            ++r;
        }
        return;
    }
    while (m) {
        const int s = __builtin_ctz(m);
        m &= m - 1;
        const uint32_t arel = (uint32_t)((s < 8 ? st.apk0 : st.apk1) >> (8 * (s & 7))) & 0xffu;
        sh.list_a[r] = (uint16_t)((uint32_t)st.lane_base + arel);
        if (MODE == MODE_SUPERKMER) sh.list_j[r] = (uint16_t)(st.lane_base + s);
        ++r;
    }
    if (MODE == MODE_SUPERKMER) {
        m = st.endm;
        r = excl_e;
        while (m) {
            const int s = __builtin_ctz(m);
            m &= m - 1;
            sh.list_e[r] = (uint16_t)(st.lane_base + s);
            ++r;
        }
    }
}
// ... 3 lines not shown
```

### biolib_amd/csrc/bl_scan_phases.hpp

```cpp
#pragma once
#include <type_traits>

#include "bl_scan_core.hpp"

namespace bl {

constexpr int NWAVE = TPB / 64;
constexpr int WH = 64 * S;
constexpr int WCHUNK = 64 + 8;

template <int MODE, int W>
struct TileShared {
    uint32_t codes[NCHUNK];
    uint32_t flags[NCHUNK];
    typename std::conditional<(MODE == MODE_SYNCMER || W == -32), uint64_t, uint32_t>::type half[W < 0 ? S : 1][W < 0 ? TPB : 1];
    alignas(4) uint16_t list_a[H];
    alignas(4) uint16_t list_j[MODE == MODE_SUPERKMER ? H : 2];
    alignas(4) uint16_t list_e[MODE == MODE_SUPERKMER ? H : 2];
    uint32_t wave_tot[NWAVE];
    uint32_t redo;
    uint32_t wave_bad[NWAVE];
    unsigned long long dig[4];
};

struct ThreadState {
    uint64_t h[S];
    uint64_t h2[S];
    uint32_t emit;
    uint32_t endm;
    uint32_t strand;
    uint64_t apk0, apk1;
    int32_t lane_base;
    int32_t jlane;
    uint32_t a_first, a_last;
    uint32_t vmask;
    uint32_t cw[3], rw[3];
    uint32_t hmax;
    uint32_t hlow;
    uint32_t occ;
};

struct alignas(16) Vec16 {
    uint32_t x, y, z, w;
};

BL_DEV void stage_chunk(const ScanParams& p, uint32_t* codes, uint32_t* flags, int c, int64_t q0)
{
    const int64_t g = q0 + 16 * (int64_t)c;
    uint32_t d[4] = {0, 0, 0, 0};
    if (g >= 0 && g + 16 <= p.n_bases) {
        const Vec16 v = *reinterpret_cast<const Vec16*>(p.bases + g);
        d[0] = v.x; d[1] = v.y; d[2] = v.z; d[3] = v.w;
    } else if (BL_COLD(g + 16 > 0 && g < p.n_bases)) {
        for (int b = 0; b < 16; ++b) {
            const int64_t q = g + b;
            if (q >= 0 && q < p.n_bases) d[b >> 2] |= (uint32_t)p.bases[q] << (8 * (b & 3));
        }
    }
    uint32_t code, bad;
    encode16(d, code, bad);
    uint32_t start = 0;
    if (p.start_bits) {
        if (g >= 0 && g < p.n_bases) start = (p.start_bits[g >> 5] >> (g & 31)) & 0xffffu;
    } else if (g == 0) {
        start = 1;
    }
    codes[c] = code;
    flags[c] = (~bad & 0xffffu) | (start << 16);
}

BL_DEV Vec16 load_chunk(const ScanParams& p, int c, int64_t q0)
{
    const int64_t g = q0 + 16 * (int64_t)c;
    Vec16 v{0, 0, 0, 0};
    if (g >= 0 && g + 16 <= p.n_bases) {
        v = *reinterpret_cast<const Vec16*>(p.bases + g);
    } else if (g + 16 > 0 && g < p.n_bases) {
        uint32_t d[4] = {0, 0, 0, 0};
        for (int b = 0; b < 16; ++b) {
            const int64_t q = g + b;
            if (q >= 0 && q < p.n_bases) d[b >> 2] |= (uint32_t)p.bases[q] << (8 * (b & 3));
        }
        v = Vec16{d[0], d[1], d[2], d[3]};
    }
    return v;
}

BL_DEV uint32_t codes_of(const Vec16& v)
{
    const uint32_t d[4] = {v.x, v.y, v.z, v.w};
    uint32_t code = 0;
    BL_UNROLL
    for (int i = 0; i < 4; ++i) {
        uint32_t x = (d[i] >> 1) & 0x03030303u;
        x ^= (x >> 1) & 0x01010101u;
        code = (code << 8) | ((x * 0x40100401u) >> 24);
    }
    return code;
}

BL_DEV int wave_index(int tid)
{
#if defined(__HIP_DEVICE_COMPILE__) && !defined(BL_CPU_EMU)
    return __builtin_amdgcn_readfirstlane(tid >> 6);
#else
    return tid >> 6;
#endif
}

BL_DEV int64_t wave_origin(const ScanParams& p, int64_t q0, int wv) { return q0 + (int64_t)wv * (p.stride / NWAVE); }

BL_DEV int wave_chunk0(const ScanParams& p, int wv) { return wv * (p.stride / NWAVE / 16); }

BL_DEV int staged_chunks(const ScanParams& p)
{
    if (p.frl) return p.slot_chunks;
    const int wchunks = p.stride / NWAVE / 16;
    int per_wave = (wchunks - 1) + (S + p.unit + p.w) / 16 + 1;
    per_wave = per_wave < 66 ? 66 : (per_wave > WCHUNK ? WCHUNK : per_wave);
    if (p.records128) per_wave = WCHUNK;
    return wave_chunk0(p, NWAVE - 1) + per_wave;
}
static_assert(3 * 63 + WCHUNK <= NCHUNK_POS && NCHUNK_POS <= 2 * TPB && NCHUNK_POS <= NCHUNK, "a tile's staged chunks fit its slot, two staging rounds and the LDS array");

template <int MODE, int W>
BL_DEV void phase_load(const ScanParams& p, TileShared<MODE, W>& sh, int tid, int64_t q0)
{
    const int needed = staged_chunks(p);
    if (tid < needed) stage_chunk(p, sh.codes, sh.flags, tid, q0);
    if (TPB + tid < needed) stage_chunk(p, sh.codes, sh.flags, TPB + tid, q0);
}

BL_DEV void gather_flags(const uint32_t* flags, int lane, Bits128& good, Bits128& start)
{
    uint64_t g[2] = {0, 0}, s[2] = {0, 0};
    BL_UNROLL
    for (int c = 0; c < 8; ++c) {
        const uint32_t f = flags[lane + c];
        g[c >> 2] |= (uint64_t)(f & 0xffffu) << (16 * (c & 3));
        s[c >> 2] |= (uint64_t)(f >> 16) << (16 * (c & 3));
    }
    good = Bits128{g[0], g[1]};
    start = Bits128{s[0], s[1]};
}

BL_DEV uint32_t bases_at(uint32_t a0, uint32_t a1, uint32_t a2, int o, int n)
{
    const int q = o >> 4, r = o & 15;
    const uint32_t hi = q == 0 ? a0 : (q == 1 ? a1 : a2), lo = q == 0 ? a1 : (q == 1 ? a2 : 0u);
    if (r + n <= 16) return n == 16 ? hi : (hi >> (32 - 2 * (r + n))) & ((1u << (2 * n)) - 1u);
    const uint32_t w16 = funnel_shr(hi, lo, 32 - 2 * r);
    return n == 16 ? w16 : w16 >> (32 - 2 * n);
}

BL_DEV uint32_t revcomp16(uint32_t c)
{
    const uint32_t r = __builtin_bitreverse32(c);
    return ~(((r >> 1) & 0x55555555u) | ((r & 0x55555555u) << 1));
}

template <int MODE, int W, int U = 0, bool GENERIC = false, bool APPROX = false>
BL_DEV void phase_hash(const ScanParams& p, TileShared<MODE, W>& sh, int tid, ThreadState& st)
{
    const int wv = wave_index(tid), lane = tid & 63;
    const uint32_t* wcodes = sh.codes + wave_chunk0(p, wv);
    const uint32_t c0 = wcodes[lane], c1 = wcodes[lane + 1], c2 = wcodes[lane + 2];
    Roller r;
    roller_start(r, c0, c1, c2, p.unit);
    if (MODE == MODE_SYNCMER) {
        Roller rk;
        roller_start(rk, c0, c1, c2, p.unit + p.w - 1);
        uint32_t strand = 0;
        BL_UNROLL
        for (int s = 0; s < S; ++s) {
            roller_step(r, s);
            roller_step(rk, s);
            st.h[s] = murmur64_plain(roller_fwd(r), p.seed);
            st.h2[s] = murmur64_plain(roller_rc(r), p.seed);
            if (p.canonical && roller_rc(rk) < roller_fwd(rk)) strand |= 1u << s;
        }
        st.strand = strand;
    } else if (U >= 1 && U <= 16) {
        const uint32_t r0 = revcomp16(c2), r1 = revcomp16(c1), r2 = revcomp16(c0);
        uint32_t hmax = 0;
        BL_UNROLL
        for (int s = 0; s < S; ++s) {
            const uint32_t fw = bases_at(c0, c1, c2, s, U >= 1 && U <= 16 ? U : 1);
            uint32_t v = fw;
            if (p.canonical) {
                const uint32_t rv = bases_at(r0, r1, r2, 48 - (U >= 1 && U <= 16 ? U : 1) - s, U >= 1 && U <= 16 ? U : 1);
                v = rv < fw ? rv : fw;
            }
            if (APPROX) {
                const uint32_t top = murmur64_top(v, p.seed);
                hmax = top > hmax ? top : hmax;
                st.h[s] = (uint64_t)top << 32;
            } else {
                st.h[s] = murmur64(v, p.seed);
            }
        }
        st.hmax = hmax;
    } else {
        uint32_t hmax = 0;
        BL_UNROLL
        for (int s = 0; s < S; ++s) {
            roller_step(r, s);
            const uint64_t fw = roller_fwd(r), rv = roller_rc(r);
            const uint64_t v = (p.canonical && rv < fw) ? rv : fw;
            if (APPROX) {
                const uint32_t top = murmur64_top(v, p.seed);
                hmax = top > hmax ? top : hmax;
                st.h[s] = (uint64_t)top << 32;
            } else {
                st.h[s] = GENERIC ? murmur64_plain(v, p.seed) : murmur64(v, p.seed);
            }
        }
        st.hmax = hmax;
    }
    (void)sh;
}

#if defined(__HIP_DEVICE_COMPILE__) && !defined(BL_CPU_EMU)
BL_DEV uint64_t lane_next(uint64_t v)
{
    const uint32_t lo = (uint32_t)__builtin_amdgcn_update_dpp(0, (int)(uint32_t)v, 0x130, 0xf, 0xf, true);
    const uint32_t hi = (uint32_t)__builtin_amdgcn_update_dpp(0, (int)(uint32_t)(v >> 32), 0x130, 0xf, 0xf, true);
    return ((uint64_t)hi << 32) | lo;
}
#endif

template <int NE, bool SECOND>
BL_DEV void gather_halo(const ThreadState* all, int tid, const ThreadState& st, uint64_t* e)
{
#if defined(__HIP_DEVICE_COMPILE__) && !defined(BL_CPU_EMU)
    (void)all;
    (void)tid;
    uint64_t n1[S];
    BL_UNROLL
    for (int x = 0; x < S; ++x) {
        if (x < NE || x < NE - 16 || x < NE - 32 || x < NE - 48) n1[x] = lane_next(SECOND ? st.h2[x] : st.h[x]);
        if (x < NE) e[S + x] = n1[x];
    }
    if (NE > 16) {
        uint64_t n2[S];
        BL_UNROLL
        for (int x = 0; x < S; ++x) {
            if (x < NE - 16 || x < NE - 32 || x < NE - 48) n2[x] = lane_next(n1[x]);
            if (x < NE - 16) e[2 * S + x] = n2[x];
        }
        if (NE > 32) {
            uint64_t n3[S];
            BL_UNROLL
            for (int x = 0; x < S; ++x) {
                if (x < NE - 32 || x < NE - 48) n3[x] = lane_next(n2[x]);
                if (x < NE - 32) e[3 * S + x] = n3[x];
            }
            if (NE > 48) {
                BL_UNROLL
                for (int x = 0; x < S; ++x)
                    if (x < NE - 48) e[4 * S + x] = lane_next(n3[x]);
            }
        }
    }
#else
    const int lane = tid & 63;
    for (int x = 0; x < NE; ++x) {
        const int nb = lane + 1 + (x >> 4);
        e[S + x] = nb < 64 ? (SECOND ? all[tid + 1 + (x >> 4)].h2[x & 15] : all[tid + 1 + (x >> 4)].h[x & 15]) : 0xDEADBEEFDEADBEEFull;
    }
    (void)st;
#endif
}

template <int NE, bool LEFT>
BL_DEV void gather_halo_keys(uint32_t* key)
{
#if defined(__HIP_DEVICE_COMPILE__) && !defined(BL_CPU_EMU)
    uint32_t cur[S];
    BL_UNROLL
    for (int x = 0; x < S; ++x) cur[x] = key[x];
    BL_UNROLL
    for (int hop = 0; hop < (NE + S - 1) / S; ++hop) {
        BL_UNROLL
        for (int x = 0; x < S; ++x) {
            if (hop * S + x < NE || (hop + 1) * S + x < NE || (hop + 2) * S + x < NE || (hop + 3) * S + x < NE) {
                const uint32_t nb = (uint32_t)__builtin_amdgcn_update_dpp(0, (int)cur[x], 0x130, 0xf, 0xf, true);
                cur[x] = LEFT ? nb + 16u : nb - 16u;
            }
            if (hop * S + x < NE) key[(hop + 1) * S + x] = cur[x];
        }
    }
#else
    (void)key;
#endif
}

#ifdef BL_EXPERIMENT_COUNT_FALLBACK
__device__ unsigned long long bl_dbg_fallbacks;
#endif
template <int NW, int W, bool LEFT, bool SECOND, bool RAW = false, bool DEFER = false, bool APPROX = false>
BL_DEV void lane_window_argmin(const ThreadState* all, int tid, const ThreadState& st, bool owns, uint32_t* a, bool* tie = nullptr)
{
    uint32_t key[S + W];
    BL_UNROLL
    for (int s = 0; s < S; ++s) key[s] = packed_key((uint32_t)((SECOND ? st.h2[s] : st.h[s]) >> 32), s, LEFT);
#if defined(__HIP_DEVICE_COMPILE__) && !defined(BL_CPU_EMU)
    gather_halo_keys<W, LEFT>(key);
#else
    {
        const int lane = tid & 63;
        for (int x = 0; x < W; ++x) {
            const int nb = lane + 1 + (x >> 4);
            const uint32_t hi = nb < 64 ? (uint32_t)((SECOND ? all[tid + 1 + (x >> 4)].h2[x & 15] : all[tid + 1 + (x >> 4)].h[x & 15]) >> 32) : 0xDEADBEEFu;
            key[S + x] = packed_key(hi, S + x, LEFT);
        }
    }
#endif
    static_assert(!APPROX || DEFER, "keys from murmur64_top: no exact form in here");
    const uint32_t dmin = window_argmin_packed<NW, W, LEFT, RAW && LEFT, APPROX>(key, a);
    if (DEFER) {
        if ((owns && dmin < (APPROX ? 128u : 64u)) || (APPROX && st.hmax >= 0xffffffc0u)) *tie = true;
        return;
    }
    if (BL_COLD(wave_any(owns && dmin < 64u))) {
#ifdef BL_EXPERIMENT_COUNT_FALLBACK
        if ((tid & 63) == 0) atomicAdd(&bl_dbg_fallbacks, 1ull);
#endif
        uint64_t e[S + W];
        BL_UNROLL
        for (int s = 0; s < S; ++s) e[s] = SECOND ? st.h2[s] : st.h[s];
        gather_halo<W, SECOND>(all, tid, st, e);
        window_argmin<NW, W, LEFT>(e, a);
    }
}

BL_DEV uint32_t range_mask(int64_t lo, int64_t hi)
{
    const int l = lo < 0 ? 0 : (lo > S + 1 ? S + 1 : (int)lo);
    const int h = hi < 0 ? 0 : (hi > S + 1 ? S + 1 : (int)hi);
    return h > l ? (((1u << h) - 1) & ~((1u << l) - 1)) : 0u;
}

BL_DEV uint32_t owned_mask(const ScanParams& p, int lane)
{
    const int own = p.stride / NWAVE - 16 * lane;
    return own >= S ? 0xffffu : (own > 0 ? (1u << own) - 1 : 0u);
}

template <int MODE, int W, bool LEFT, bool SECOND, int NW>
BL_DEV void window_argmin_lds_exact(TileShared<MODE, W>& sh, const ThreadState* all, int tid, const ThreadState& st, int w, uint32_t* a)
{
    const int wbase = tid & ~63, lane = tid & 63;
    if (MODE == MODE_SYNCMER || W == -32) {
#if defined(__HIP_DEVICE_COMPILE__) && !defined(BL_CPU_EMU)
        BL_UNROLL
        for (int s = 0; s < S; ++s) sh.half[s][W < 0 ? tid : 0] = SECOND ? st.h2[s] : st.h[s];
#else
        for (int t = wbase; t < wbase + 64; ++t)
            for (int s = 0; s < S; ++s) sh.half[s][W < 0 ? t : 0] = SECOND ? all[t].h2[s] : all[t].h[s];
#endif
        BL_UNROLL
        for (int i = 0; i < NW; ++i) {
            uint64_t best = 0;
            int arg = 0;
            for (int x = 0; x < w; ++x) {
                int pos = 16 * lane + i + x;
                pos = pos < WH ? pos : WH - 1;
                const uint64_t v = sh.half[pos & 15][W < 0 ? wbase + (pos >> 4) : 0];
                if (x == 0 || (LEFT ? v < best : v <= best)) { best = v; arg = i + x; }
            }
            a[i] = (uint32_t)arg;
        }
        return;
    }
    using Mask = typename std::conditional<(W == -8 || W == -16), uint32_t, unsigned long long>::type;
    Mask cand[NW];
    for (int half = 0; half < 2; ++half) {
#if defined(__HIP_DEVICE_COMPILE__) && !defined(BL_CPU_EMU)
        (void)all;
        BL_UNROLL
        for (int s = 0; s < S; ++s) {
            const uint64_t h = SECOND ? st.h2[s] : st.h[s];
            sh.half[s][W < 0 ? tid : 0] = (uint32_t)(half == 0 ? h >> 32 : h);
        }
#else
        (void)st;
        for (int t = wbase; t < wbase + 64; ++t)
            for (int s = 0; s < S; ++s) {
                const uint64_t h = SECOND ? all[t].h2[s] : all[t].h[s];
                sh.half[s][W < 0 ? t : 0] = (uint32_t)(half == 0 ? h >> 32 : h);
            }
#endif
        BL_UNROLL
        for (int i = 0; i < NW; ++i) {
            uint32_t best = 0;
            Mask mask = 0;
            int arg = 0;
            for (int x = 0; x < w; ++x) {
                int pos = 16 * lane + i + x;
                pos = pos < WH ? pos : WH - 1;
                const uint32_t v = (uint32_t)sh.half[pos & 15][W < 0 ? wbase + (pos >> 4) : 0];
                if (half == 0) {
                    if (x == 0 || v < best) { best = v; mask = (Mask)1 << x; }
                    else if (v == best) mask |= (Mask)1 << x;
                } else if ((cand[i] >> x) & 1) {
                    const bool first = ((cand[i] & (((Mask)1 << x) - 1)) == 0);
                    if (first || (LEFT ? v < best : v <= best)) { best = v; arg = i + x; }
                }
            }
            if (half == 0) cand[i] = mask;
            else a[i] = (uint32_t)arg;
        }
    }
}

template <int MODE, int W, int NW, int P, bool LEFT, bool SECOND, bool RAW>
BL_DEV void lane_window_argmin_generic(const ScanParams& p, TileShared<MODE, W>& sh, const ThreadState* all, int tid, ThreadState& st, int w, bool owns,
                                       uint32_t* a)
{
    constexpr int NE = NW + 2 * P - 1, NH = NE - S;
    uint32_t key[NE];
    BL_UNROLL
    for (int s = 0; s < S; ++s) key[s] = packed_key7((uint32_t)((SECOND ? st.h2[s] : st.h[s]) >> 32), LEFT ? s : 127 - s);
#if defined(__HIP_DEVICE_COMPILE__) && !defined(BL_CPU_EMU)
    (void)all;
    {
        uint32_t cur[S];
        BL_UNROLL
        for (int x = 0; x < S; ++x) cur[x] = key[x];
        BL_UNROLL
        for (int hop = 0; hop * S < NH; ++hop) {
            BL_UNROLL
            for (int x = 0; x < S; ++x) {
// ... 813 lines not shown
```

Before: 562.3.

## Precompute packed 2-bit base codes per batch and read them in scan kernels

Adds a per-batch pack_codes kernel that encodes the ASCII bases into 2-bit codes, one 32-bit word per 16 bases, plus a bitmask marking chunks that contain non-ACGT bases. The count and emit kernels then load these packed codes (a quarter of the bytes) instead of re-encoding raw bases. The emit kernel reads codes straight from the packed array rather than from per-tile slot copies written by the count kernel, which drops that write and read traffic. This costs extra device memory and a pack pass at batch creation, and falls back to ASCII decoding when any chunk in a wave is flagged bad.

```diff
diff --git a/biolib_amd/csrc/bl_capi.hip b/biolib_amd/csrc/bl_capi.hip
--- a/biolib_amd/csrc/bl_capi.hip
+++ b/biolib_amd/csrc/bl_capi.hip
@@ -31,6 +31,8 @@
 struct bl_ctx;
 hipStream_t bl_ctx_stream(bl_ctx* ctx);
 int bl_ctx_device(bl_ctx* ctx);
+void* bl_ctx_pool_alloc(bl_ctx* ctx, size_t bytes);
+void bl_ctx_pool_free(bl_ctx* ctx, void* p);
 
 namespace {
 
@@ -90,6 +92,7 @@
     bool timed = false;
     bool exact_windows = false;
     bool position_tiled = false;
+    bool packed_codes = true;
     int jaccard128_path = 0;
     bool count128_tables = true;
     int table_prefix_bits = -1;
@@ -116,6 +119,9 @@
     uint8_t* bases = nullptr;
     bool owns_bases = false;
     uint32_t* start_bits = nullptr;
+    uint32_t* packed = nullptr;
+    uint32_t* codes = nullptr;
+    uint32_t* chunk_bad = nullptr;
     uint64_t n_bases = 0;
     uint64_t n_seqs = 0;
     uint64_t read_len = 0;
@@ -307,6 +313,19 @@
     return BL_OK;
 }
 
+int make_packed_codes(bl_ctx* c, bl_batch* b, hipStream_t s)
+{
+    if (!c->packed_codes) return BL_OK;
+    const uint64_t total = (uint64_t)bl::packed_total((int64_t)b->n_bases);
+    b->packed = static_cast<uint32_t*>(bl_ctx_pool_alloc(c, (total + total / 32) * sizeof(uint32_t)));
+    if (!b->packed) return fail(BL_ERR_OOM, "device allocation of the batch's packed codes failed (bl_ctx_set_option(\"packed_codes\", 0) does without)");
+    b->codes = b->packed + bl::PACK_LEAD;
+    b->chunk_bad = b->packed + total + bl::PACK_LEAD / 32;
+    hipError_t e = bl::launch_pack_codes(b->bases, b->n_bases, b->packed, b->packed + total, s);
+    if (e != hipSuccess) return fail(BL_ERR_HIP, std::string("pack_codes: ") + hipGetErrorString(e));
+    return BL_OK;
+}
+
 int ensure_start_bits(bl_ctx* c, const bl_batch* cb)
 {
     bl_batch* b = const_cast<bl_batch*>(cb);
@@ -562,6 +581,10 @@
         c->position_tiled = value != 0;
         return BL_OK;
     }
+    if (n == "packed_codes" && (value == 0 || value == 1)) {
+        c->packed_codes = value != 0;
+        return BL_OK;
+    }
     if (n == "count128_tables" && (value == 0 || value == 1)) {
         c->count128_tables = value != 0;
         return BL_OK;
@@ -677,6 +700,8 @@
     hipError_t e = hipMemsetAsync(b->bases + (n_bases & ~15ull), 0, 64 + (n_bases & 15ull), c->stream);
     if (e == hipSuccess && n_bases) e = hipMemcpyAsync(b->bases, bases, n_bases, hipMemcpyHostToDevice, c->stream);
     if (e != hipSuccess) { bl_batch_destroy(b); return fail(BL_ERR_HIP, std::string("upload: ") + hipGetErrorString(e)); }
+    rc = make_packed_codes(c, b, c->stream);
+    if (rc != BL_OK) { bl_batch_destroy(b); return rc; }
     uint64_t fixed = 0;
     if (read_len) {
         if (read_len < n_bases) {
@@ -761,6 +786,8 @@
     e = hipMemsetAsync(b->bases + (n_bases & ~15ull), 0, 64 + (n_bases & 15ull), c->stream);
     if (e == hipSuccess) e = bl::launch_synth(b->bases, 0, n_bases, seed, c->stream);
     if (e != hipSuccess) { bl_batch_destroy(b); return fail(BL_ERR_HIP, std::string("synth: ") + hipGetErrorString(e)); }
+    rc = make_packed_codes(c, b, c->stream);
+    if (rc != BL_OK) { bl_batch_destroy(b); return rc; }
     if (read_len > 0 && read_len < n_bases) {
         b->read_len = read_len;
         b->n_seqs = (n_bases + read_len - 1) / read_len;
@@ -783,13 +810,16 @@
     b->bases = static_cast<uint8_t*>(d_bases);
     b->owns_bases = true;
     b->n_seqs = n_seqs;
+    hipStream_t s = bl_ctx_stream(c);
+    rc = make_packed_codes(c, b, s);
+    if (rc != BL_OK) { bl_ctx_pool_free(c, d_offsets); bl_batch_destroy(b); return rc; }
     if (fixed_len && n_seqs > 1 && fixed_len < n_bases) {
         b->read_len = fixed_len;
         bl_ctx_pool_free(c, d_offsets);
+        if (b->codes && hipStreamSynchronize(s) != hipSuccess) { bl_batch_destroy(b); return fail(BL_ERR_HIP, "adopt: pack_codes failed"); }
         *out = b;
         return BL_OK;
     }
-    hipStream_t s = bl_ctx_stream(c);
     const uint64_t n_words = (n_bases + 31) / 32 + 4;
     b->start_bits = static_cast<uint32_t*>(bl_ctx_pool_alloc(c, n_words * sizeof(uint32_t)));
     hipError_t e = b->start_bits ? hipSuccess : hipErrorOutOfMemory;
@@ -813,6 +843,10 @@
     b->n_seqs = like->n_seqs;
     b->read_len = like->read_len;
     b->origin = like->origin;
+    hipStream_t s = bl_ctx_stream(c);
+    rc = make_packed_codes(c, b, s);
+    if (rc == BL_OK && b->codes && hipStreamSynchronize(s) != hipSuccess) rc = fail(BL_ERR_HIP, "adopt: pack_codes failed");
+    if (rc != BL_OK) { bl_batch_destroy(b); return rc; }
     *out = b;
     return BL_OK;
 }
@@ -833,6 +867,7 @@
     }
     if (b->owns_bases && b->bases) bl_ctx_pool_free(b->ctx, b->bases);
     if (b->start_bits) bl_ctx_pool_free(b->ctx, b->start_bits);
+    if (b->packed) bl_ctx_pool_free(b->ctx, b->packed);
     delete b;
     return BL_OK;
 }
@@ -1132,6 +1167,10 @@
         if (rc != BL_OK) return rc;
     }
     p.start_bits = b->start_bits;
+    if (c->packed_codes && b->codes && bl::packed_covers(p) && (p.frl || bl::packed_scan_shape(mode, (int)w))) {
+        p.codes_packed = b->codes;
+        p.chunk_bad = b->chunk_bad;
+    }
     p.unit = (int32_t)unit;
     p.w = (int32_t)w;
     p.seed = (uint32_t)seed;
@@ -1146,7 +1185,8 @@
     const size_t n_lists = mode == bl::MODE_SUPERKMER ? 3 : 1;
     const size_t slot_entries = nt * (size_t)p.stride;
     const size_t list_bytes = n_lists * slot_entries * sizeof(uint16_t);
-    rc = grow(c, reinterpret_cast<void**>(&c->cur->slot_buf), &c->cur->slot_buf_bytes, list_bytes + nt * (size_t)p.slot_chunks * sizeof(uint32_t));
+    const size_t code_bytes = p.codes_packed ? 0 : nt * (size_t)p.slot_chunks * sizeof(uint32_t);
+    rc = grow(c, reinterpret_cast<void**>(&c->cur->slot_buf), &c->cur->slot_buf_bytes, list_bytes + code_bytes);
     if (rc != BL_OK) return rc;
     unsigned long long* tb = reinterpret_cast<unsigned long long*>(c->cur->tile_buf);
     p.tile_counts = tb;
@@ -1158,7 +1198,7 @@
     p.slots_a = c->cur->slot_buf;
     p.slots_j = mode == bl::MODE_SUPERKMER ? c->cur->slot_buf + slot_entries : nullptr;
     p.slots_e = mode == bl::MODE_SUPERKMER ? c->cur->slot_buf + 2 * slot_entries : nullptr;
-    p.slots_c = reinterpret_cast<uint32_t*>(reinterpret_cast<unsigned char*>(c->cur->slot_buf) + list_bytes);
+    p.slots_c = p.codes_packed ? nullptr : reinterpret_cast<uint32_t*>(reinterpret_cast<unsigned char*>(c->cur->slot_buf) + list_bytes);
     p.shards = c->shards();
     const bl::GroupRange all{0, (uint32_t)p.n_tiles};
     unsigned long long* carry = reinterpret_cast<unsigned long long*>(c->cur->ws);
diff --git a/biolib_amd/csrc/bl_kernels.hip b/biolib_amd/csrc/bl_kernels.hip
--- a/biolib_amd/csrc/bl_kernels.hip
+++ b/biolib_amd/csrc/bl_kernels.hip
@@ -128,14 +128,15 @@
     for (uint32_t i = tid; i < (n + 1) / 2; i += TPB) d32[i] = s32[i];
 }
 
-template <int MODE, int W, int SY = 0, int U = 0>
+template <int MODE, int W, int SY = 0, int U = 0, bool PACKED = false>
 __device__ __forceinline__ void count_tile(const ScanParams& p, TileShared<MODE, W>& sh, uint32_t tile, int tid)
 {
     const int64_t q0 = p.origin + (int64_t)tile * p.stride;
-    phase_load<MODE, W>(p, sh, tid, q0);
+    static_assert(!PACKED || SY != 0 || U != 0 || packed_scan_shape(MODE, W), "scan_windows hands no packed copy to this shape: its twin is never launched");
+    phase_load<MODE, W, PACKED>(p, sh, tid, q0);
     constexpr bool CS = SY == 1;
     if (SY != 0 && tid == 0) sh.redo = 0;
-    if (MODE != MODE_SYNCMER) {
+    if (MODE != MODE_SYNCMER && !PACKED) {
         const int needed = staged_chunks(p);
         uint32_t* sc = p.slots_c + (size_t)tile * p.slot_chunks;
         if (tid < needed) sc[tid] = sh.codes[tid];
@@ -194,13 +195,13 @@
     }
 }
 
-template <int MODE, int W, int NS, int LIM_LAST, bool GENERIC, bool APPROX = false, int U = 0>
+template <int MODE, int W, int NS, int LIM_LAST, bool GENERIC, bool APPROX = false, int U = 0, bool PACKED = false>
 __device__ __forceinline__ void count_tile_frl(const ScanParams& p, TileShared<MODE, W>& sh, uint32_t tile, int tid)
 {
     const int64_t q0 = tile_q0(p, tile);
-    phase_load_frl<MODE, W>(p, sh, tid, q0);
+    phase_load_frl<MODE, W, PACKED>(p, sh, tid, q0);
     if (APPROX && tid == 0) sh.redo = 0;
-    {
+    if (!PACKED) {
         uint32_t* sc = p.slots_c + (size_t)tile * p.slot_chunks;
         for (int c = tid; c < p.slot_chunks; c += TPB) sc[c] = sh.codes[c];
     }
@@ -229,7 +230,7 @@
 }
 
 constexpr int C3_RC = NCHUNK + 4;
-template <int MODE, bool LOOPED = false, bool C3 = false, bool WIDE = false>
+template <int MODE, bool LOOPED = false, bool C3 = false, bool WIDE = false, bool PACKED = false>
 __device__ __forceinline__ void emit_tile(const ScanParams& p, uint32_t* codes, uint32_t tile, int tid, Digest& dg)
 {
     const int64_t q0 = tile_q0(p, tile);
@@ -237,7 +238,7 @@
     const unsigned long long cnt = uniform64(p.tile_counts[tile]);
     const unsigned long long base = uniform64(p.tile_base[tile] + p.block_base[tile / SCAN_BLK]);
     const int needed = staged_chunks(p);
-    const uint32_t* sc = p.slots_c + (size_t)tile * p.slot_chunks;
+    const uint32_t* sc = PACKED ? p.codes_packed + (q0 >> 4) : p.slots_c + (size_t)tile * p.slot_chunks;
     const uint32_t c0 = (MODE != MODE_SYNCMER && tid < needed) ? sc[tid] : 0;
     const uint32_t c1 = (MODE != MODE_SYNCMER && TPB + tid < needed) ? sc[TPB + tid] : 0;
     const uint16_t* la = p.slots_a + slot;
@@ -295,7 +296,7 @@
     for (uint32_t r = 2 * TPB + tid; r < n_s; r += TPB) one(r, la[r], MODE == MODE_SUPERKMER ? lj[r] : 0u);
 }
 
-template <int MODE, int W, int U, int C, int SY = 0>
+template <bool PACKED, int MODE, int W, int U, int C, int SY = 0>
 __global__ __launch_bounds__(TPB, (MODE == MODE_MINIMIZER && SY == 2 ? BL_POSAX_WAVES : MODE == MODE_SUPERKMER && SY == 2 ? BL_SKAX_WAVES : SY == 1 && W < 0 ? BL_CSRT_WAVES : SY == 1 ? BL_CS_WAVES : SY == 2 ? BL_SY2_WAVES : (MODE == MODE_SYNCMER && W > 0 ? BL_SY0_WAVES : MODE == MODE_SYNCMER || (MODE == MODE_SUPERKMER && W == -32) ? 2 : (W == -32 || (W < 0 && MODE == MODE_SUPERKMER) ? 3 : (W == -16 ? 5 : (W < 0 ? 4 : (W <= 11 ? 5 : (MODE == MODE_SUPERKMER && W == 17 && U == 15 ? BL_C4_WAVES : 4)))))))) void scan_count_kernel(const ScanParams pin, GroupRange g)
 {
     __shared__ TileShared<MODE, W> sh;
@@ -306,10 +307,10 @@
         p.stride = NWAVE * (64 * S - 16 * ((W + 15) / 16));
     }
     if (C >= 0) p.canonical = C;
-    if (blockIdx.x < g.count) count_tile<MODE, W, SY, U>(p, sh, g.first + blockIdx.x, threadIdx.x);
-}
-
-template <int MODE, int W, int U, int C>
+    if (blockIdx.x < g.count) count_tile<MODE, W, SY, U, PACKED>(p, sh, g.first + blockIdx.x, threadIdx.x);
+}
+
+template <bool PACKED, int MODE, int W, int U, int C>
 __global__ __launch_bounds__(TPB, 2) void scan_redo_kernel(const ScanParams pin)
 {
     __shared__ TileShared<MODE, W> sh;
@@ -322,7 +323,7 @@
     if (C >= 0) p.canonical = C;
     const unsigned long long n = *p.redo_count;
     for (unsigned long long i = blockIdx.x; i < n; i += gridDim.x) {
-        count_tile<MODE, W>(p, sh, p.redo_list[i], threadIdx.x);
+        count_tile<MODE, W, 0, 0, PACKED>(p, sh, p.redo_list[i], threadIdx.x);
         __syncthreads();
     }
 }
@@ -353,24 +354,24 @@
 #ifndef BL_FRL_WAVES
 #define BL_FRL_WAVES 5
 #endif
-template <int MODE, int W, int NS, int U, int L, int C, bool APPROX = false>
+template <bool PACKED, int MODE, int W, int NS, int U, int L, int C, bool APPROX = false>
 __global__ __launch_bounds__(TPB, (W <= 11 ? BL_FRL_WAVES : 4)) void scan_count_frl_kernel(const ScanParams pin, GroupRange g)
 {
     __shared__ TileShared<MODE, W> sh;
     const ScanParams p = frl_params<MODE, W, NS, U, L, C>(pin);
     constexpr int LIM_LAST = frl_lim_last<W, NS, U, L>();
     static_assert(L == 0 || (LIM_LAST >= 1 && LIM_LAST <= NS), "read-tiled geometry: the last lane of a read must own 1..NS windows");
-    if (blockIdx.x < g.count) count_tile_frl<MODE, W, NS, LIM_LAST, U == 0, APPROX, U>(p, sh, g.first + blockIdx.x, threadIdx.x);
-}
-
-template <int MODE, int W, int NS, int U, int L, int C>
+    if (blockIdx.x < g.count) count_tile_frl<MODE, W, NS, LIM_LAST, U == 0, APPROX, U, PACKED>(p, sh, g.first + blockIdx.x, threadIdx.x);
+}
+
+template <bool PACKED, int MODE, int W, int NS, int U, int L, int C>
 __global__ __launch_bounds__(TPB, (W <= 11 ? 5 : 4)) void scan_redo_frl_kernel(const ScanParams pin)
 {
     __shared__ TileShared<MODE, W> sh;
     const ScanParams p = frl_params<MODE, W, NS, U, L, C>(pin);
     const unsigned long long n = *p.redo_count;
     for (unsigned long long i = blockIdx.x; i < n; i += gridDim.x) {
-        count_tile_frl<MODE, W, NS, frl_lim_last<W, NS, U, L>(), U == 0, false, U>(p, sh, p.redo_list[i], threadIdx.x);
+        count_tile_frl<MODE, W, NS, frl_lim_last<W, NS, U, L>(), U == 0, false, U, PACKED>(p, sh, p.redo_list[i], threadIdx.x);
         __syncthreads();
     }
 }
@@ -383,7 +384,7 @@
 
 template <int MODE, int U, int C, int FRL>
 constexpr bool emit_c3() { return MODE == MODE_MINIMIZER && U == 31 && C == 1 && FRL == 1; }
-template <int MODE, int U = 0, int C = -1, int FRL = -1, bool WIDE = false>
+template <int MODE, int U = 0, int C = -1, int FRL = -1, bool WIDE = false, bool PACKED = false>
 __global__ __launch_bounds__(TPB) void scan_emit_kernel(const ScanParams pin, GroupRange g)
 {
     static_assert(!WIDE || (MODE == MODE_SUPERKMER && U == 0), "32-byte records are super-k-mer groups; the unit length comes from the arguments");
@@ -404,7 +405,7 @@
 #pragma unroll 1
         for (uint32_t k = 0; k < (uint32_t)K && t0 + k < g.count; ++k) {
             Digest d1{0, 0, 0};
-            emit_tile<MODE, true, C3>(p, codes[k & 1], g.first + t0 + k, tid, d1);
+            emit_tile<MODE, true, C3, false, PACKED>(p, codes[k & 1], g.first + t0 + k, tid, d1);
             acc[0][tid] ^= (uint32_t)d1.xv; acc[1][tid] ^= (uint32_t)(d1.xv >> 32);
             acc[2][tid] ^= (uint32_t)d1.xh; acc[3][tid] ^= (uint32_t)(d1.xh >> 32);
             acc[4][tid] ^= (uint32_t)d1.xp; acc[5][tid] ^= (uint32_t)(d1.xp >> 32);
@@ -414,7 +415,7 @@
         dg.xp = ((unsigned long long)acc[5][tid] << 32) | acc[4][tid];
     } else {
         if (blockIdx.x >= g.count) return;
-        emit_tile<MODE, false, C3, WIDE>(p, codes[0], g.first + blockIdx.x, tid, dg);
+        emit_tile<MODE, false, C3, WIDE, PACKED>(p, codes[0], g.first + blockIdx.x, tid, dg);
     }
 
     const unsigned long long xv = MODE == MODE_SYNCMER ? 0ull : wave_xor_to_last_u64(dg.xv), xh = MODE == MODE_SYNCMER ? 0ull : wave_xor_to_last_u64(dg.xh);
@@ -599,12 +600,25 @@
     if (p < n_bases && offsets[q + 1] > p) atomicOr(&bits[p >> 5], 1u << (p & 31));
 }
 
+__global__ __launch_bounds__(256) void pack_codes_kernel(const uint8_t* bases, int64_t n_bases, uint32_t* codes, uint32_t* chunk_bad)
+{
+    const int64_t t = (int64_t)blockIdx.x * 256 + threadIdx.x;
+    if (t >= packed_total(n_bases)) return;
+    uint32_t code;
+    const bool bad = pack_chunk(bases, n_bases, t - PACK_LEAD, code);
+    codes[t] = code;
+    const unsigned long long m = __builtin_amdgcn_ballot_w64(bad);
+    if ((threadIdx.x & 31) == 0) chunk_bad[t >> 5] = (uint32_t)(m >> (threadIdx.x & 32));
+}
+
 
 #define BL_LAUNCH(NAME, KERNEL, GRID, BLOCK, LDS, ...)                          \
     do {                                                                       \
         if (log) log->add(NAME);                                               \
         hipLaunchKernelGGL(KERNEL, GRID, BLOCK, LDS, stream, __VA_ARGS__);     \
     } while (0)
+#define BL_PK(KERNEL, ...) (p.codes_packed ? KERNEL<true, __VA_ARGS__> : KERNEL<false, __VA_ARGS__>)
+#define BL_PK_W(KERNEL, MODEV, WV, ...) (p.codes_packed ? KERNEL<packed_scan_shape(MODEV, WV), MODEV, WV, __VA_ARGS__> : KERNEL<false, MODEV, WV, __VA_ARGS__>)
 #define BL_MODE_NAME(HEAD, TAIL) (MODE == MODE_MINIMIZER ? HEAD "MM" TAIL : MODE == MODE_SUPERKMER ? HEAD "SK" TAIL : HEAD "SY" TAIL)
 
 #define BL_W_ALL(X)                                                                                                                      \
@@ -651,10 +665,10 @@
     const dim3 grid(g.count), block(TPB);
     if (mode == MODE_MINIMIZER && p.w == 11 && p.unit == 31 && p.canonical && p.read_len == 150 && p.ns == 15 && p.rpw == 8) {
         if (p.redo_list && g.first == 0 && !p.exact_windows) {
-            BL_LAUNCH("frl<MM,W=11,NS=15,U=31,L=150,approx>", (scan_count_frl_kernel<MODE_MINIMIZER, 11, 15, 31, 150, 1, true>), grid, block, 0, p, g);
-            BL_LAUNCH("frl_redo<MM,W=11,NS=15,U=31,L=150>", (scan_redo_frl_kernel<MODE_MINIMIZER, 11, 15, 31, 150, 1>), dim3(g.count < 512u ? g.count : 512u), block, 0, p);
+            BL_LAUNCH("frl<MM,W=11,NS=15,U=31,L=150,approx>", BL_PK(scan_count_frl_kernel, MODE_MINIMIZER, 11, 15, 31, 150, 1, true), grid, block, 0, p, g);
+            BL_LAUNCH("frl_redo<MM,W=11,NS=15,U=31,L=150>", BL_PK(scan_redo_frl_kernel, MODE_MINIMIZER, 11, 15, 31, 150, 1), dim3(g.count < 512u ? g.count : 512u), block, 0, p);
         } else {
-            BL_LAUNCH("frl<MM,W=11,NS=15,U=31,L=150>", (scan_count_frl_kernel<MODE_MINIMIZER, 11, 15, 31, 150, 1>), grid, block, 0, p, g);
+            BL_LAUNCH("frl<MM,W=11,NS=15,U=31,L=150>", BL_PK(scan_count_frl_kernel, MODE_MINIMIZER, 11, 15, 31, 150, 1), grid, block, 0, p, g);
         }
         return hipGetLastError();
     }
@@ -663,10 +677,10 @@
         const dim3 redo_grid(g.count < 512u ? g.count : 512u);
 #define BL_FRL_SHAPE(NSV)                                                                                                                                    \
     if (approx) {                                                                                                                                            \
-        BL_LAUNCH("frl<MM,W=11,NS=" #NSV ",U=31,approx>", (scan_count_frl_kernel<MODE_MINIMIZER, 11, NSV, 31, 0, 1, true>), grid, block, 0, p, g);            \
-        BL_LAUNCH("frl_redo<MM,W=11,NS=" #NSV ",U=31>", (scan_redo_frl_kernel<MODE_MINIMIZER, 11, NSV, 31, 0, 1>), redo_grid, block, 0, p);                   \
+        BL_LAUNCH("frl<MM,W=11,NS=" #NSV ",U=31,approx>", BL_PK(scan_count_frl_kernel, MODE_MINIMIZER, 11, NSV, 31, 0, 1, true), grid, block, 0, p, g);            \
+        BL_LAUNCH("frl_redo<MM,W=11,NS=" #NSV ",U=31>", BL_PK(scan_redo_frl_kernel, MODE_MINIMIZER, 11, NSV, 31, 0, 1), redo_grid, block, 0, p);                   \
     } else {                                                                                                                                                 \
-        BL_LAUNCH("frl<MM,W=11,NS=" #NSV ",U=31>", (scan_count_frl_kernel<MODE_MINIMIZER, 11, NSV, 31, 0, 1>), grid, block, 0, p, g);                         \
+        BL_LAUNCH("frl<MM,W=11,NS=" #NSV ",U=31>", BL_PK(scan_count_frl_kernel, MODE_MINIMIZER, 11, NSV, 31, 0, 1), grid, block, 0, p, g);                         \
     }
         if (p.ns == 14) { BL_FRL_SHAPE(14) } else if (p.ns == 15) { BL_FRL_SHAPE(15) } else { BL_FRL_SHAPE(16) }
 #undef BL_FRL_SHAPE
@@ -675,14 +689,14 @@
     if (p.ns != S) return hipErrorInvalidValue;
     if (mode == MODE_MINIMIZER) {
         switch (p.w) {
-            case 5: BL_LAUNCH("frl<MM,W=5>", (scan_count_frl_kernel<MODE_MINIMIZER, 5, S, 0, 0, -1>), grid, block, 0, p, g); break;
-            case 10: BL_LAUNCH("frl<MM,W=10>", (scan_count_frl_kernel<MODE_MINIMIZER, 10, S, 0, 0, -1>), grid, block, 0, p, g); break;
-            case 11: BL_LAUNCH("frl<MM,W=11>", (scan_count_frl_kernel<MODE_MINIMIZER, 11, S, 0, 0, -1>), grid, block, 0, p, g); break;
-            case 19: BL_LAUNCH("frl<MM,W=19>", (scan_count_frl_kernel<MODE_MINIMIZER, 19, S, 0, 0, -1>), grid, block, 0, p, g); break;
+            case 5: BL_LAUNCH("frl<MM,W=5>", BL_PK(scan_count_frl_kernel, MODE_MINIMIZER, 5, S, 0, 0, -1), grid, block, 0, p, g); break;
+            case 10: BL_LAUNCH("frl<MM,W=10>", BL_PK(scan_count_frl_kernel, MODE_MINIMIZER, 10, S, 0, 0, -1), grid, block, 0, p, g); break;
+            case 11: BL_LAUNCH("frl<MM,W=11>", BL_PK(scan_count_frl_kernel, MODE_MINIMIZER, 11, S, 0, 0, -1), grid, block, 0, p, g); break;
+            case 19: BL_LAUNCH("frl<MM,W=19>", BL_PK(scan_count_frl_kernel, MODE_MINIMIZER, 19, S, 0, 0, -1), grid, block, 0, p, g); break;
             default: return hipErrorInvalidValue;
         }
     } else if (mode == MODE_SUPERKMER && p.w == 17) {
-        BL_LAUNCH("frl<SK,W=17>", (scan_count_frl_kernel<MODE_SUPERKMER, 17, S, 0, 0, -1>), grid, block, 0, p, g);
+        BL_LAUNCH("frl<SK,W=17>", BL_PK(scan_count_frl_kernel, MODE_SUPERKMER, 17, S, 0, 0, -1), grid, block, 0, p, g);
     } else {
         return hipErrorInvalidValue;
     }
@@ -696,65 +710,65 @@
     if (MODE == MODE_MINIMIZER && p.w == 11 && p.unit == 31 && p.canonical) {
 #ifndef BL_NO_POSAX
         if (p.redo_list && g.first == 0 && !p.exact_windows) {
-            BL_LAUNCH("count<MM,W=11,U=31,C=1,approx>", (scan_count_kernel<MODE_MINIMIZER, 11, 31, 1, 2>), grid, block, 0, p, g);
-            BL_LAUNCH("redo<MM,W=11,U=31,C=1>", (scan_redo_kernel<MODE_MINIMIZER, 11, 31, 1>), dim3(g.count < 512u ? g.count : 512u), block, 0, p);
+            BL_LAUNCH("count<MM,W=11,U=31,C=1,approx>", BL_PK(scan_count_kernel, MODE_MINIMIZER, 11, 31, 1, 2), grid, block, 0, p, g);
+            BL_LAUNCH("redo<MM,W=11,U=31,C=1>", BL_PK(scan_redo_kernel, MODE_MINIMIZER, 11, 31, 1), dim3(g.count < 512u ? g.count : 512u), block, 0, p);
             return hipGetLastError();
         }
 #endif
-        BL_LAUNCH("count<MM,W=11,U=31,C=1>", (scan_count_kernel<MODE, 11, 31, 1>), grid, block, 0, p, g);
+        BL_LAUNCH("count<MM,W=11,U=31,C=1>", BL_PK(scan_count_kernel, MODE, 11, 31, 1), grid, block, 0, p, g);
         return hipGetLastError();
     }
     if (MODE == MODE_SUPERKMER && p.w == 17 && p.unit == 15 && p.canonical) {
 #ifdef BL_SKAX
         if (p.redo_list && g.first == 0 && !p.exact_windows) {
-            BL_LAUNCH("count<SK,W=17,U=15,C=1,approx>", (scan_count_kernel<MODE_SUPERKMER, 17, 15, 1, 2>), grid, block, 0, p, g);
-            BL_LAUNCH("redo<SK,W=17,U=15,C=1>", (scan_redo_kernel<MODE_SUPERKMER, 17, 15, 1>), dim3(g.count < 512u ? g.count : 512u), block, 0, p);
+            BL_LAUNCH("count<SK,W=17,U=15,C=1,approx>", BL_PK(scan_count_kernel, MODE_SUPERKMER, 17, 15, 1, 2), grid, block, 0, p, g);
+            BL_LAUNCH("redo<SK,W=17,U=15,C=1>", BL_PK(scan_redo_kernel, MODE_SUPERKMER, 17, 15, 1), dim3(g.count < 512u ? g.count : 512u), block, 0, p);
             return hipGetLastError();
         }
 #endif
-        BL_LAUNCH("count<SK,W=17,U=15,C=1>", (scan_count_kernel<MODE, 17, 15, 1>), grid, block, 0, p, g);
+        BL_LAUNCH("count<SK,W=17,U=15,C=1>", BL_PK(scan_count_kernel, MODE, 17, 15, 1), grid, block, 0, p, g);
         return hipGetLastError();
     }
     if (MODE == MODE_SYNCMER && p.w == 21 && p.unit == 11 && p.canonical) {
         const bool closed = (p.soff == 0 && p.eoff == 20) || (p.soff == 20 && p.eoff == 0);
         const unsigned redo_grid = g.count < 512u ? g.count : 512u;
         if (closed && !p.exact_windows && p.redo_list && g.first == 0) {
-            BL_LAUNCH("count<SY,W=21,U=11,C=1,closed>", (scan_count_kernel<MODE_SYNCMER, 21, 11, 1, 1>), grid, block, 0, p, g);
-            BL_LAUNCH("redo<SY,W=21,U=11,C=1>", (scan_redo_kernel<MODE_SYNCMER, 21, 11, 1>), dim3(redo_grid), block, 0, p);
+            BL_LAUNCH("count<SY,W=21,U=11,C=1,closed>", BL_PK(scan_count_kernel, MODE_SYNCMER, 21, 11, 1, 1), grid, block, 0, p, g);
+            BL_LAUNCH("redo<SY,W=21,U=11,C=1>", BL_PK(scan_redo_kernel, MODE_SYNCMER, 21, 11, 1), dim3(redo_grid), block, 0, p);
 #ifndef BL_NO_SY2
         } else if (p.redo_list && g.first == 0) {
-            BL_LAUNCH("count<SY,W=21,U=11,C=1,deferred>", (scan_count_kernel<MODE_SYNCMER, 21, 11, 1, 2>), grid, block, 0, p, g);
-            BL_LAUNCH("redo<SY,W=21,U=11,C=1>", (scan_redo_kernel<MODE_SYNCMER, 21, 11, 1>), dim3(redo_grid), block, 0, p);
+            BL_LAUNCH("count<SY,W=21,U=11,C=1,deferred>", BL_PK(scan_count_kernel, MODE_SYNCMER, 21, 11, 1, 2), grid, block, 0, p, g);
+            BL_LAUNCH("redo<SY,W=21,U=11,C=1>", BL_PK(scan_redo_kernel, MODE_SYNCMER, 21, 11, 1), dim3(redo_grid), block, 0, p);
 #endif
         } else {
-            BL_LAUNCH("count<SY,W=21,U=11,C=1>", (scan_count_kernel<MODE, 21, 11, 1>), grid, block, 0, p, g);
+            BL_LAUNCH("count<SY,W=21,U=11,C=1>", BL_PK(scan_count_kernel, MODE, 21, 11, 1), grid, block, 0, p, g);
         }
         return hipGetLastError();
     }
     if (MODE == MODE_SYNCMER && p.w <= 32 && !p.exact_windows && ((p.soff == 0 && p.eoff == p.w - 1) || (p.soff == p.w - 1 && p.eoff == 0))) {
-        if (p.w <= 17) BL_LAUNCH("count<SY,closed,W<=17>", (scan_count_kernel<MODE_SYNCMER, -8, 0, -1, 1>), grid, block, 0, p, g);
-        else BL_LAUNCH("count<SY,closed,W<=32>", (scan_count_kernel<MODE_SYNCMER, -16, 0, -1, 1>), grid, block, 0, p, g);
+        if (p.w <= 17) BL_LAUNCH("count<SY,closed,W<=17>", BL_PK(scan_count_kernel, MODE_SYNCMER, -8, 0, -1, 1), grid, block, 0, p, g);
+        else BL_LAUNCH("count<SY,closed,W<=32>", BL_PK(scan_count_kernel, MODE_SYNCMER, -16, 0, -1, 1), grid, block, 0, p, g);
         return hipGetLastError();
     }
     if (MODE != MODE_SYNCMER && p.w >= 2 && p.w <= 32) {
         constexpr int MM = MODE == MODE_SYNCMER ? MODE_MINIMIZER : MODE;
         switch (p.w) {
-#define BL_W(WV) case WV: BL_LAUNCH(BL_MODE_NAME("count<", ",W=" #WV ">"), (scan_count_kernel<MM, WV, 0, -1>), grid, block, 0, p, g); return hipGetLastError();
+#define BL_W(WV) case WV: BL_LAUNCH(BL_MODE_NAME("count<", ",W=" #WV ">"), BL_PK_W(scan_count_kernel, MM, WV, 0, -1), grid, block, 0, p, g); return hipGetLastError();
             BL_W_ALL(BL_W)
 #undef BL_W
         }
     }
     switch (p.w) {
-        case 1: BL_LAUNCH(BL_MODE_NAME("count<", ",W=1>"), (scan_count_kernel<MODE, 1, 0, -1>), grid, block, 0, p, g); break;
-        case 11: BL_LAUNCH(BL_MODE_NAME("count<", ",W=11>"), (scan_count_kernel<MODE, 11, 0, -1>), grid, block, 0, p, g); break;
-        case 17: BL_LAUNCH(BL_MODE_NAME("count<", ",W=17>"), (scan_count_kernel<MODE, 17, 0, -1>), grid, block, 0, p, g); break;
-        case 21: BL_LAUNCH(BL_MODE_NAME("count<", ",W=21>"), (scan_count_kernel<MODE, 21, 0, -1>), grid, block, 0, p, g); break;
+        case 1: BL_LAUNCH(BL_MODE_NAME("count<", ",W=1>"), BL_PK(scan_count_kernel, MODE, 1, 0, -1), grid, block, 0, p, g); break;
+        case 11: BL_LAUNCH(BL_MODE_NAME("count<", ",W=11>"), BL_PK(scan_count_kernel, MODE, 11, 0, -1), grid, block, 0, p, g); break;
+        case 17: BL_LAUNCH(BL_MODE_NAME("count<", ",W=17>"), BL_PK(scan_count_kernel, MODE, 17, 0, -1), grid, block, 0, p, g); break;
+        case 21: BL_LAUNCH(BL_MODE_NAME("count<", ",W=21>"), BL_PK(scan_count_kernel, MODE, 21, 0, -1), grid, block, 0, p, g); break;
         default:
             if constexpr (MODE == MODE_SYNCMER) {
-                if (p.w <= 16) { BL_LAUNCH("count<SY,W<=16>", (scan_count_kernel<MODE, -8, 0, -1>), grid, block, 0, p, g); break; }
-                if (p.w <= 32) { BL_LAUNCH("count<SY,W<=32>", (scan_count_kernel<MODE, -16, 0, -1>), grid, block, 0, p, g); break; }
+                if (p.w <= 16) { BL_LAUNCH("count<SY,W<=16>", BL_PK(scan_count_kernel, MODE, -8, 0, -1), grid, block, 0, p, g); break; }
+                if (p.w <= 32) { BL_LAUNCH("count<SY,W<=32>", BL_PK(scan_count_kernel, MODE, -16, 0, -1), grid, block, 0, p, g); break; }
             }
-            BL_LAUNCH(BL_MODE_NAME("count<", ",W>32>"), (scan_count_kernel<MODE, -32, 0, -1>), grid, block, 0, p, g);
+            BL_LAUNCH(BL_MODE_NAME("count<", ",W>32>"), BL_PK(scan_count_kernel, MODE, -32, 0, -1), grid, block, 0, p, g);
             break;
     }
     return hipGetLastError();
@@ -781,14 +795,17 @@
     const dim3 grid((g.count + K - 1) / K), block(TPB);
     if (MODE == MODE_MINIMIZER && p.frl && p.unit == 31 && p.canonical) {
         const uint32_t have_c3 = (uint32_t)(((K > 1 ? 2 : 1) * 2 * C3_RC + (K > 1 ? 6 * TPB : 0)) * sizeof(uint32_t));
-        BL_LAUNCH("emit<MM,C3>", (scan_emit_kernel<MODE_MINIMIZER, 31, 1, 1>), grid, block, lds_per_wg > have_c3 ? lds_per_wg - have_c3 : 0, p, g);
+        if (p.codes_packed) BL_LAUNCH("emit<MM,C3>", (scan_emit_kernel<MODE_MINIMIZER, 31, 1, 1, false, true>), grid, block, lds_per_wg > have_c3 ? lds_per_wg - have_c3 : 0, p, g);
+        else BL_LAUNCH("emit<MM,C3>", (scan_emit_kernel<MODE_MINIMIZER, 31, 1, 1>), grid, block, lds_per_wg > have_c3 ? lds_per_wg - have_c3 : 0, p, g);
         return;
     }
     if (MODE == MODE_SUPERKMER && p.records128) {
-        BL_LAUNCH("emit<SK,wide>", (scan_emit_kernel<MODE_SUPERKMER, 0, -1, -1, true>), grid, block, pad, p, g);
+        if (p.codes_packed) BL_LAUNCH("emit<SK,wide>", (scan_emit_kernel<MODE_SUPERKMER, 0, -1, -1, true, true>), grid, block, pad, p, g);
+        else BL_LAUNCH("emit<SK,wide>", (scan_emit_kernel<MODE_SUPERKMER, 0, -1, -1, true>), grid, block, pad, p, g);
         return;
     }
-    BL_LAUNCH(BL_MODE_NAME("emit<", ">"), (scan_emit_kernel<MODE>), grid, block, pad, p, g);
+    if (MODE != MODE_SYNCMER && p.codes_packed) BL_LAUNCH(BL_MODE_NAME("emit<", ">"), (scan_emit_kernel<MODE, 0, -1, -1, false, MODE != MODE_SYNCMER>), grid, block, pad, p, g);
+    else BL_LAUNCH(BL_MODE_NAME("emit<", ">"), (scan_emit_kernel<MODE>), grid, block, pad, p, g);
 }
 
 hipError_t launch_scan_emit(int mode, const ScanParams& p, GroupRange g, hipStream_t stream, uint32_t lds_per_wg, LaunchLog* log)
@@ -803,6 +820,8 @@
     return hipGetLastError();
 }
 #undef BL_LAUNCH
+#undef BL_PK
+#undef BL_PK_W
 #undef BL_MODE_NAME
 #undef BL_W_ALL
 
@@ -851,6 +870,13 @@
     return hipGetLastError();
 }
 
+hipError_t launch_pack_codes(const uint8_t* bases, uint64_t n_bases, uint32_t* codes, uint32_t* chunk_bad, hipStream_t stream)
+{
+    const uint64_t total = (uint64_t)packed_total((int64_t)n_bases);
+    hipLaunchKernelGGL(pack_codes_kernel, dim3((unsigned)((total + 255) / 256)), dim3(256), 0, stream, bases, (int64_t)n_bases, codes, chunk_bad);
+    return hipGetLastError();
+}
+
 }
 
 #ifdef BL_EXPERIMENT_COUNT_FALLBACK
diff --git a/biolib_amd/csrc/bl_launch.hpp b/biolib_amd/csrc/bl_launch.hpp
--- a/biolib_amd/csrc/bl_launch.hpp
+++ b/biolib_amd/csrc/bl_launch.hpp
@@ -18,4 +18,5 @@
 hipError_t launch_synth(uint8_t* bases, uint64_t first, uint64_t n, uint64_t seed, hipStream_t stream);
 hipError_t launch_start_bits_fixed(uint32_t* bits, uint64_t n_words, uint64_t n_bases, uint64_t read_len, hipStream_t stream);
 hipError_t launch_start_bits_offsets(uint32_t* bits, const uint64_t* offsets, uint64_t n_seqs, uint64_t n_bases, hipStream_t stream);
+hipError_t launch_pack_codes(const uint8_t* bases, uint64_t n_bases, uint32_t* codes, uint32_t* chunk_bad, hipStream_t stream);
 }
diff --git a/biolib_amd/csrc/bl_scan_core.hpp b/biolib_amd/csrc/bl_scan_core.hpp
--- a/biolib_amd/csrc/bl_scan_core.hpp
+++ b/biolib_amd/csrc/bl_scan_core.hpp
@@ -79,7 +79,17 @@
     uint32_t lpr_inv;
     int64_t n_reads;
     int32_t records128;
+    const uint32_t* codes_packed;
+    const uint32_t* chunk_bad;
 };
+
+constexpr int PACK_LEAD = 32, PACK_TAIL = NCHUNK;
+BL_DEV int64_t packed_total(int64_t n_bases) { return (PACK_LEAD + ((n_bases + 15) >> 4) + PACK_TAIL + 63) & ~63LL; }
+constexpr bool packed_scan_shape(int mode, int w) { return !(mode == MODE_MINIMIZER && w == 25); }
+BL_DEV bool packed_covers(const ScanParams& p)
+{
+    return p.n_tiles > 0 && p.origin >= -16 * (int64_t)PACK_LEAD && p.origin + (int64_t)(p.n_tiles - 1) * p.stride < p.n_bases + 16;
+}
 
 BL_DEV bool frl_width_built(int mode, int w)
 {
diff --git a/biolib_amd/csrc/bl_scan_frl.hpp b/biolib_amd/csrc/bl_scan_frl.hpp
--- a/biolib_amd/csrc/bl_scan_frl.hpp
+++ b/biolib_amd/csrc/bl_scan_frl.hpp
@@ -9,31 +9,39 @@
     return p.frl ? (g & ~15LL) : g;
 }
 
+template <bool PACKED = false>
 BL_DEV bool stage_chunk_frl(const ScanParams& p, uint32_t* codes, uint32_t* flags, int c, int64_t q0)
 {
     const int64_t g = q0 + 16 * (int64_t)c;
-    uint32_t d[4] = {0, 0, 0, 0};
-    if (g + 16 <= p.n_bases) {
-        const Vec16 v = *reinterpret_cast<const Vec16*>(p.bases + g);
-        d[0] = v.x; d[1] = v.y; d[2] = v.z; d[3] = v.w;
-    } else if (BL_COLD(g < p.n_bases)) {
-        for (int b = 0; b < 16; ++b) {
-            const int64_t q = g + b;
-            if (q < p.n_bases) d[b >> 2] |= (uint32_t)p.bases[q] << (8 * (b & 3));
-        }
-    }
-    uint32_t code, bad;
-    encode16(d, code, bad);
+    uint32_t code = 0, bad = 0;
+    bool ascii = true;
+    if (PACKED) {
+        const bool pbad = packed_chunk(p, g, code);
+        ascii = BL_COLD(wave_any(pbad));
+    }
+    if (ascii) {
+        uint32_t d[4] = {0, 0, 0, 0};
+        if (g + 16 <= p.n_bases) {
+            const Vec16 v = *reinterpret_cast<const Vec16*>(p.bases + g);
+            d[0] = v.x; d[1] = v.y; d[2] = v.z; d[3] = v.w;
+        } else if (BL_COLD(g < p.n_bases)) {
+            for (int b = 0; b < 16; ++b) {
+                const int64_t q = g + b;
+                if (q < p.n_bases) d[b >> 2] |= (uint32_t)p.bases[q] << (8 * (b & 3));
+            }
+        }
+        encode16(d, code, bad);
+    }
     codes[c] = code;
     flags[c] = ~bad & 0xffffu;
     return bad != 0;
 }
 
-template <int MODE, int W>
+template <int MODE, int W, bool PACKED = false>
 BL_DEV void phase_load_frl(const ScanParams& p, TileShared<MODE, W>& sh, int tid, int64_t q0)
 {
     bool bad = false;
-    for (int c = tid; c < p.slot_chunks; c += TPB) bad |= stage_chunk_frl(p, sh.codes, sh.flags, c, q0);
+    for (int c = tid; c < p.slot_chunks; c += TPB) bad |= stage_chunk_frl<PACKED>(p, sh.codes, sh.flags, c, q0);
     const int wv = wave_index(tid);
 #if defined(__HIP_DEVICE_COMPILE__) && !defined(BL_CPU_EMU)
     const bool any = wave_any(bad);
diff --git a/biolib_amd/csrc/bl_scan_phases.hpp b/biolib_amd/csrc/bl_scan_phases.hpp
--- a/biolib_amd/csrc/bl_scan_phases.hpp
+++ b/biolib_amd/csrc/bl_scan_phases.hpp
@@ -44,21 +44,36 @@
     uint32_t x, y, z, w;
 };
 
+BL_DEV bool packed_chunk(const ScanParams& p, int64_t g, uint32_t& code)
+{
+    const int64_t ci = g >> 4;
+    code = p.codes_packed[ci];
+    return ((p.chunk_bad[ci >> 5] >> (ci & 31)) & 1u) != 0;
+}
+
+template <bool PACKED = false>
 BL_DEV void stage_chunk(const ScanParams& p, uint32_t* codes, uint32_t* flags, int c, int64_t q0)
 {
     const int64_t g = q0 + 16 * (int64_t)c;
-    uint32_t d[4] = {0, 0, 0, 0};
-    if (g >= 0 && g + 16 <= p.n_bases) {
-        const Vec16 v = *reinterpret_cast<const Vec16*>(p.bases + g);
-        d[0] = v.x; d[1] = v.y; d[2] = v.z; d[3] = v.w;
-    } else if (BL_COLD(g + 16 > 0 && g < p.n_bases)) {
-        for (int b = 0; b < 16; ++b) {
-            const int64_t q = g + b;
-            if (q >= 0 && q < p.n_bases) d[b >> 2] |= (uint32_t)p.bases[q] << (8 * (b & 3));
-        }
-    }
-    uint32_t code, bad;
-    encode16(d, code, bad);
+    uint32_t code = 0, bad = 0;
+    bool ascii = true;
+    if (PACKED) {
+        const bool pbad = packed_chunk(p, g, code);
+        ascii = BL_COLD(wave_any(pbad));
+    }
+    if (ascii) {
+        uint32_t d[4] = {0, 0, 0, 0};
+        if (g >= 0 && g + 16 <= p.n_bases) {
+            const Vec16 v = *reinterpret_cast<const Vec16*>(p.bases + g);
+            d[0] = v.x; d[1] = v.y; d[2] = v.z; d[3] = v.w;
+        } else if (BL_COLD(g + 16 > 0 && g < p.n_bases)) {
+            for (int b = 0; b < 16; ++b) {
+                const int64_t q = g + b;
+                if (q >= 0 && q < p.n_bases) d[b >> 2] |= (uint32_t)p.bases[q] << (8 * (b & 3));
+            }
+        }
+        encode16(d, code, bad);
+    }
     uint32_t start = 0;
     if (p.start_bits) {
         if (g >= 0 && g < p.n_bases) start = (p.start_bits[g >> 5] >> (g & 31)) & 0xffffu;
@@ -99,6 +114,18 @@
     return code;
 }
 
+BL_DEV bool pack_chunk(const uint8_t* bases, int64_t n_bases, int64_t ci, uint32_t& code)
+{
+    ScanParams lp{};
+    lp.bases = bases;
+    lp.n_bases = n_bases;
+    const Vec16 v = load_chunk(lp, 0, 16 * ci);
+    const uint32_t d[4] = {v.x, v.y, v.z, v.w};
+    uint32_t bad;
+    encode16(d, code, bad);
+    return bad != 0 || 16 * ci + 16 > n_bases;
+}
+
 BL_DEV int wave_index(int tid)
 {
 #if defined(__HIP_DEVICE_COMPILE__) && !defined(BL_CPU_EMU)
@@ -123,12 +150,12 @@
 }
 static_assert(3 * 63 + WCHUNK <= NCHUNK_POS && NCHUNK_POS <= 2 * TPB && NCHUNK_POS <= NCHUNK, "a tile's staged chunks fit its slot, two staging rounds and the LDS array");
 
-template <int MODE, int W>
+template <int MODE, int W, bool PACKED = false>
 BL_DEV void phase_load(const ScanParams& p, TileShared<MODE, W>& sh, int tid, int64_t q0)
 {
     const int needed = staged_chunks(p);
-    if (tid < needed) stage_chunk(p, sh.codes, sh.flags, tid, q0);
-    if (TPB + tid < needed) stage_chunk(p, sh.codes, sh.flags, TPB + tid, q0);
+    if (tid < needed) stage_chunk<PACKED>(p, sh.codes, sh.flags, tid, q0);
+    if (TPB + tid < needed) stage_chunk<PACKED>(p, sh.codes, sh.flags, TPB + tid, q0);
 }
 
 BL_DEV void gather_flags(const uint32_t* flags, int lane, Bits128& good, Bits128& start)
```

New measurement: 599.5 (median of 6 runs). 1.07x the previous value.
